# MilchRatchet/Luminary

Hardware: AMD Instinct MI355X
Metric: Mrays/s at 1920x1080, 8 bounces (higher is better)
Workload: dtype f32

## Files before the change

include/lum_core.h:

```cpp
#ifndef LUM_CORE_H
#define LUM_CORE_H

#include <stdint.h>

#ifdef __cplusplus
extern "C" {
#endif

typedef struct LumContext LumContext;

typedef struct LumDeviceSceneView {
  uint32_t num_meshes;
  uint32_t num_instances;
  uint32_t num_materials;
  uint32_t num_lights;
  const uint32_t* mesh_tri_offset;
  const float* vertices;
  const uint32_t* tri_tex;
  const uint32_t* instance_mesh_ids;
  const float* instance_transforms;
  const uint16_t* materials;
  const uint8_t* light_tree_root;
  const uint8_t* light_tree_nodes;
  const uint32_t* light_tri_handles;
// ... 135 lines not shown

int lumc_generate_result(LumContext* ctx, uint32_t mode, uint32_t local_error_minimization, uint32_t uniform_samples, float exposure,
                         const LumOutputParams* tone, float* d_result, void* stream);
int lumc_generate_result_host(LumContext* ctx, uint32_t mode, uint32_t local_error_minimization, uint32_t uniform_samples, float exposure,
                              const LumOutputParams* tone, float* result);
int lumc_render_undersampled(LumContext* ctx, uint32_t stage, uint32_t iteration, void* stream);
int lumc_generate_result_undersampled(LumContext* ctx, uint32_t stage, uint32_t iteration, float* d_result, void* stream);
int lumc_generate_result_undersampled_host(LumContext* ctx, uint32_t stage, uint32_t iteration, float* result);
int lumc_adaptive_note_first_sample(LumContext* ctx, void* stream);
int lumc_post_bloom(LumContext* ctx, float* d_image, uint32_t full_width, uint32_t full_height, uint32_t undersampling_stage, float blend, void* stream);
int lumc_post_bloom_host(LumContext* ctx, float* image, uint32_t full_width, uint32_t full_height, uint32_t undersampling_stage, float blend);
typedef struct LumDenoiseParams {
  uint32_t iterations;
  float sigma_luminance;
  float sigma_normal;
  float sigma_depth;
  uint32_t uniform_samples;
} LumDenoiseParams;
void lumc_denoise_default_params(LumDenoiseParams* params);
int lumc_render_guides(LumContext* ctx, uint32_t num_samples, void* stream);
int lumc_download_guides(LumContext* ctx, float* albedo, float* normal, float* depth);
int lumc_has_guides(const LumContext* ctx);
int lumc_denoise(LumContext* ctx, const LumDenoiseParams* params, float* d_image, void* stream);
int lumc_denoise_host(LumContext* ctx, const LumDenoiseParams* params, float* image);
int lumc_set_denoise_form(LumContext* ctx, int lds);
int lumc_download_result_image(LumContext* ctx, float* result);
const float* lumc_result_image(LumContext* ctx);

int lumc_trace_closest(LumContext* ctx, uint32_t num_rays, const float* d_origins, const float* d_dirs, const uint32_t* d_ignore, uint32_t* d_out, void* stream);
int lumc_pixel_query(LumContext* ctx, uint32_t x, uint32_t y, uint32_t sample_id, uint32_t out[6]);
int lumc_trace_closest_host(LumContext* ctx, uint32_t num_rays, const float* origins, const float* dirs, const uint32_t* ignore, uint32_t* out);

int lumc_trace_visibility(LumContext* ctx, uint32_t num_rays, const float* d_origins, const float* d_dirs, const float* d_dist, const uint32_t* d_ids, const uint32_t* d_order,
                          float* d_out, void* stream);
int lumc_trace_visibility_host(LumContext* ctx, uint32_t num_rays, const float* origins, const float* dirs, const float* dist, const uint32_t* ids, const uint32_t* order, float* out);
int lumc_light_query_host(LumContext* ctx, uint32_t num_rays, const float* origins, const float* dirs, const uint32_t* self, const float* randoms, uint32_t* out_ids,
                          uint32_t* out_num_hits);

#define LUMC_LENS_MAX_INTERFACES 24
typedef struct LumLensInterface { float radius, vertex, cylindrical_radius; } LumLensInterface;
typedef struct LumLensMedium { float design_ior, abbe, cylindrical_radius; } LumLensMedium;
typedef struct LumPhysicalCamera {
  float aperture_point, aperture_radius, exit_pupil_point, exit_pupil_radius, image_plane_distance, sensor_width;
  uint32_t allow_reflections;
  uint32_t num_interfaces;
  LumLensInterface interfaces[LUMC_LENS_MAX_INTERFACES];
  LumLensMedium media[LUMC_LENS_MAX_INTERFACES + 1];
} LumPhysicalCamera;
int lumc_set_physical_camera(LumContext* ctx, const LumPhysicalCamera* camera);
int lumc_camera_rays(LumContext* ctx, const uint32_t* pixels, uint32_t n, uint32_t first_sample, uint32_t samples, float* out_origin, float* out_dir, float* out_weight);

int lumc_set_bvh_builder(LumContext* ctx, int builder);

unsigned int lumc_lds_stack_bytes(void);

#define LUMC_COMM_ID_BYTES 128
int lumc_device_count(void);
uint32_t lumc_tile_lattice_step(uint32_t world);
uint32_t lumc_tile_owner(uint32_t tile_x, uint32_t tile_y, uint32_t tiles_x, uint32_t world);
int lumc_tile_pixels(uint32_t width, uint32_t height, uint32_t rank, uint32_t world, uint32_t tile, uint32_t* out, uint32_t* count);
int lumc_comm_unique_id(uint8_t id[LUMC_COMM_ID_BYTES]);
int lumc_comm_init_rank(LumContext* ctx, int world, int rank, const uint8_t id[LUMC_COMM_ID_BYTES]);
int lumc_comm_init_all(LumContext** ctxs, int n);
void lumc_comm_destroy(LumContext* ctx);
int lumc_frame_assemble(LumContext* ctx, uint32_t frame_pixels, int root, void* stream, float** d_frame_out);
int lumc_frame_assemble_all(LumContext** ctxs, int n, uint32_t frame_pixels, int root, float** d_frame_root);
int lumc_frame_gather(LumContext* ctx, uint32_t width, uint32_t height, int root, void* stream, float** d_frame_out);
int lumc_frame_gather_all(LumContext** ctxs, int n, uint32_t width, uint32_t height, int root, float** d_frame_root);
int lumc_frame_download(LumContext* ctx, uint32_t frame_pixels, float* first_moment, float* second_moment);
uint32_t lumc_frame_plane_stride(const LumContext* ctx);
int lumc_use_assembled_frame(LumContext* ctx, int on);
int lumc_accumulators_from_frame(LumContext* dst, LumContext* src);
int lumc_comm_count(const LumContext* ctx);
int lumc_device_name(int ordinal, char* out, size_t size);

int lumc_set_ray_sorting(LumContext* ctx, int mode);
int lumc_get_ray_sorting(const LumContext* ctx);

enum { LUMC_FLAVOUR_EXACT = 0, LUMC_FLAVOUR_FAST = 1 };
int lumc_set_flavour(LumContext* ctx, int flavour);
int lumc_get_flavour(const LumContext* ctx);
int lumc_set_ambient_reuse(LumContext* ctx, int mode);
int lumc_get_ambient_reuse(const LumContext* ctx);
int lumc_set_fused_resolve(LumContext* ctx, int on);
int lumc_set_sobol_table(LumContext* ctx, int on);
double lumc_bvh_build_seconds(const LumContext* ctx);
int lumc_bvh_meshes_by_builder(const LumContext* ctx, uint32_t out[2]);
int lumc_bvh_stats(LumContext* ctx, uint64_t out[4]);
uint32_t lumc_scene_view_sizeof(void);
int lumc_host_bvh_probe(const float* boxes, uint32_t count, uint32_t max_leaf, uint64_t out[6], double inner_area[3]);
uint32_t lumc_leaf_max_triangles(void);
typedef struct LumMeshRefitStats {
  uint64_t refits, rebuilds;
  uint32_t last_refits, last_rebuilds;
  double max_cost_growth;
  double seconds;
  double seconds_upload, seconds_refit, seconds_rebuild, seconds_assemble;
  double seconds_hash, seconds_download, seconds_lights;
} LumMeshRefitStats;
int lumc_set_mesh_refit(LumContext* ctx, uint32_t mode, float max_cost_growth);
int lumc_mesh_refit_stats(const LumContext* ctx, LumMeshRefitStats* out);
int lumc_bvh_refit_probe(const float* built_boxes, const float* refit_boxes, uint32_t count, uint32_t refit_count, int builder, int on_gpu, uint64_t sizes[3],
                         void* built_nodes, void* refit_nodes, void* host_refit_nodes, uint32_t* prims, double cost[3], uint64_t* valid);
int lumc_scene_tree_probe(const LumDeviceSceneView* scene, uint64_t sizes[4], void* nodes, void* tris, void* leaves, void* rows, uint32_t* mesh_root, float bounds[6]);
typedef struct LumInstanceUpdateStats {
  uint64_t device_updates, fallbacks, relayouts;
  uint32_t tlas_nodes, tlas_depth, tlas_capacity, hittable;
  double seconds;
  double seconds_relayout, seconds_upload, seconds_boxes, seconds_build, seconds_leaves;
} LumInstanceUpdateStats;
int lumc_set_instance_update(LumContext* ctx, uint32_t mode);
int lumc_instance_update_stats(const LumContext* ctx, LumInstanceUpdateStats* out);
int lumc_instance_boxes_probe(const LumDeviceSceneView* scene, const float* mesh_boxes, int on_gpu, void* rows, float* boxes, uint32_t* hittable);
int lumc_resident_tree_probe(LumContext* ctx, uint64_t sizes[5], void* top_nodes, void* leaves, uint32_t* mesh_root, uint64_t* mesh_hash);
int lumc_set_mesh_refit_in_place(LumContext* ctx, uint32_t on);
typedef struct LumResidentRefitStats {
  uint64_t updates, fallbacks;
  uint32_t last_meshes, last_launches;
  uint64_t last_bytes_downloaded;
  double seconds;
  double seconds_upload, seconds_hash, seconds_refit, seconds_cost, seconds_top_level;
} LumResidentRefitStats;
int lumc_resident_refit_stats(const LumContext* ctx, LumResidentRefitStats* out);
int lumc_resident_mesh_nodes_probe(LumContext* ctx, void* nodes);
int lumc_host_bvh_nodes_probe(const float* boxes, uint32_t count, uint32_t max_leaf, uint32_t max_depth, uint64_t sizes[3], void* nodes, uint32_t* prims);

#ifdef __cplusplus
}
#endif

#endif
```

luminary_amd/core.py:

```python
import ctypes as C

import numpy as np

from . import DeviceSceneView, _lib

DIRTY_CONSTANTS, DIRTY_MATERIALS, DIRTY_INSTANCES, DIRTY_LIGHTS, DIRTY_MESHES, DIRTY_TEXTURES, DIRTY_PARTICLES, DIRTY_ALL = 1, 2, 4, 8, 16, 32, 64, 127
DIRTY_MESH_POSITIONS = 128
DIRTY_INSTANCE_TRANSFORMS = 256
BVH_BUILDERS = {"sah": 0, "lbvh": 1, "ploc": 2, "sah_gpu": 3}
CNT_TRACE, CNT_SHADOW, CNT_LIGHT_BVH, CNT_VERTICES, CNT_NODES, CNT_TRIS, CNT_NODES_SHADOW, CNT_TRIS_SHADOW, CNT_NODES_LIGHT, CNT_TRIS_LIGHT, CNT_NODES_LDS, CNT_NODES_LDS_SHADOW, CNT_AMBIENT_DEFERRED, CNT_AMBIENT_FALLBACK = range(14)
CNT_COUNT = 16
KERNELS = ("generate", "trace", "shade", "shadow", "accumulate", "light_query", "resolve", "output", "sky", "sort", "volume")


class CoreError(RuntimeError):
    pass


class OutputParams(C.Structure):
    _fields_ = [("src_width", C.c_uint32), ("src_height", C.c_uint32), ("dst_width", C.c_uint32), ("dst_height", C.c_uint32),
                ("inv_sample_count", C.c_float), ("exposure", C.c_float), ("tonemap", C.c_uint32), ("filter", C.c_uint32), ("dithering", C.c_uint32),
                ("purkinje", C.c_uint32), ("use_color_correction", C.c_uint32), ("passthrough", C.c_uint32), ("purkinje_kappa1", C.c_float),
                ("purkinje_kappa2", C.c_float), ("cc_h", C.c_float), ("cc_s", C.c_float), ("cc_v", C.c_float), ("film_grain", C.c_float),
                ("agx_slope", C.c_float), ("agx_power", C.c_float), ("agx_saturation", C.c_float), ("supersampling", C.c_uint32),
# ... 127 lines not shown
        self._lib.lumc_context_create.restype = C.c_int
        rc = self._lib.lumc_context_create(C.c_int(device), C.byref(self._ctx))
        if rc != 0:
            msg = self._lib.lumc_last_error(self._ctx).decode() if self._ctx else "context allocation failed"
            if self._ctx:
                self._lib.lumc_context_destroy(self._ctx)
                self._ctx = C.c_void_p()
            raise CoreError("lumc_context_create failed (no CPU fallback exists): " + msg)
        self.num_pixels = 0

    @property
    def flavour(self):
        fn = getattr(self._lib, "lumc_get_flavour", None)
        if fn is None:
            return "exact"
        fn.restype = C.c_int
        return "fast" if fn(self._ctx) == 1 else "exact"

    @staticmethod
    def device_count():
        return int(_lib().lumc_device_count())

    @staticmethod
    def tile_pixels(width, height, rank, world, tile=32):
        lib = _lib()
        n = C.c_uint32()
        if lib.lumc_tile_pixels(C.c_uint32(width), C.c_uint32(height), C.c_uint32(rank), C.c_uint32(world), C.c_uint32(tile), C.c_void_p(0), C.byref(n)):
            raise CoreError("lumc_tile_pixels: bad arguments")
        out = np.zeros(max(n.value, 1), dtype=np.uint32)
        lib.lumc_tile_pixels(C.c_uint32(width), C.c_uint32(height), C.c_uint32(rank), C.c_uint32(world), C.c_uint32(tile), out.ctypes.data_as(C.c_void_p), C.byref(n))
        return out[:n.value]

    @staticmethod
    def comm_unique_id():
        buf = (C.c_uint8 * 128)()
        if _lib().lumc_comm_unique_id(buf):
            raise CoreError("lumc_comm_unique_id failed")
        return bytes(buf)

    def comm_init_rank(self, world, rank, unique_id):
        buf = (C.c_uint8 * 128).from_buffer_copy(unique_id)
        self._call("lumc_comm_init_rank", C.c_int(world), C.c_int(rank), buf)

    def frame_assemble(self, frame_pixels, root=0, stream=0):
        ptr = C.c_void_p()
        self._call("lumc_frame_assemble", C.c_uint32(frame_pixels), C.c_int(root), C.c_void_p(stream), C.byref(ptr))
        return ptr.value

    def frame_gather(self, width, height, root=0, stream=0):
        ptr = C.c_void_p()
        self._call("lumc_frame_gather", C.c_uint32(width), C.c_uint32(height), C.c_int(root), C.c_void_p(stream), C.byref(ptr))
        return ptr.value

    def frame_download(self, frame_pixels):
        fm = np.zeros(3 * frame_pixels, dtype=np.float32)
        sm = np.zeros(frame_pixels, dtype=np.float32)
        self._call("lumc_frame_download", C.c_uint32(frame_pixels), fm.ctypes.data_as(C.c_void_p), sm.ctypes.data_as(C.c_void_p))
        return fm.reshape(3, -1), sm

    @property
    def ray_sorting(self):
        fn = self._lib.lumc_get_ray_sorting
        fn.restype = C.c_int
        return int(fn(self._ctx))

    def set_ray_sorting(self, mode):
        self._call("lumc_set_ray_sorting", C.c_int(mode))

    def set_fused_resolve(self, on):
        self._call("lumc_set_fused_resolve", C.c_int(int(on)))

    def set_sobol_table(self, on):
        self._call("lumc_set_sobol_table", C.c_int(1 if on else 0))

    def set_ambient_reuse(self, mode):
        self._call("lumc_set_ambient_reuse", C.c_int(mode))

    @property
    def ambient_reuse(self):
        fn = self._lib.lumc_get_ambient_reuse
        fn.restype = C.c_int
        return bool(fn(self._ctx))

    def set_physical_camera(self, camera):
        self._call("lumc_set_physical_camera", C.byref(camera) if camera is not None else C.c_void_p(0))

    def camera_rays(self, pixels, first_sample, samples):
        px = np.ascontiguousarray(pixels, dtype=np.uint32)
        n = px.size * samples
        o = np.zeros((n, 3), dtype=np.float32)
        d = np.zeros((n, 3), dtype=np.float32)
        w = np.zeros(n, dtype=np.float32)
        self._call("lumc_camera_rays", px.ctypes.data_as(C.c_void_p), C.c_uint32(px.size), C.c_uint32(first_sample), C.c_uint32(samples),
                   o.ctypes.data_as(C.c_void_p), d.ctypes.data_as(C.c_void_p), w.ctypes.data_as(C.c_void_p))
        return o, d, w

    def pixel_query(self, x, y, sample_id=0):
        out = (C.c_uint32 * 6)()
        self._call("lumc_pixel_query", C.c_uint32(x), C.c_uint32(y), C.c_uint32(sample_id), out)
        a = np.array(list(out), dtype=np.uint32)
        return int(a[0]), int(a[1]), float(a[2:3].view(np.float32)[0]), a[3:6].view(np.float32).copy()

    def set_flavour(self, name):
        self._call("lumc_set_flavour", C.c_int({"exact": 0, "fast": 1}[name]))

    def _call(self, name, *args):
        fn = getattr(self._lib, name)
        fn.restype = C.c_int
        if fn(self._ctx, *args) != 0:
            raise CoreError("%s failed: %s" % (name, self._lib.lumc_last_error(self._ctx).decode()))

    def close(self):
        if self._ctx:
            self._lib.lumc_context_destroy(self._ctx)
            self._ctx = C.c_void_p()

    def __del__(self):
        try:
            self.close()
        except Exception:
            pass

    def upload(self, view):
        self._view_keepalive = view
        self._call("lumc_scene_upload", C.byref(view))
        self.width, self.height = view.width, view.height

    def update(self, view, dirty):
        self._view_keepalive = view
        self._call("lumc_scene_update", C.byref(view), C.c_uint(dirty))
        self.width, self.height = view.width, view.height

    def generate_output(self, params, first_moment=None, want_float=False):
        out = np.zeros((params.dst_height, params.dst_width), dtype=np.uint32)
        planes = np.zeros(params.output_planes_shape(), dtype=np.float32) if want_float else None
        pl = planes.ctypes.data_as(C.c_void_p) if want_float else C.c_void_p(0)
        if isinstance(first_moment, np.ndarray):
            fm = np.ascontiguousarray(first_moment, dtype=np.float32)
            self._call("lumc_generate_output_from_host", C.byref(params), fm.ctypes.data_as(C.c_void_p), out.ctypes.data_as(C.c_void_p), pl)
        else:
            ptr = C.c_void_p(0) if first_moment is None else C.c_void_p(int(first_moment))
            self._call("lumc_generate_output_host", C.byref(params), ptr, out.ctypes.data_as(C.c_void_p), pl)
        return (out, planes) if want_float else out

    def download_luts(self):
        out = {"conductor": np.zeros(1024, np.uint16), "glossy": np.zeros(1024, np.uint16), "dielectric": np.zeros(32768, np.uint16),
               "dielectric_inv": np.zeros(32768, np.uint16)}
        self._call("lumc_download_luts", *[out[k].ctypes.data_as(C.c_void_p) for k in ("conductor", "glossy", "dielectric", "dielectric_inv")])
        return out

    def download_sky_luts(self):
        tm = np.zeros(2 * 64 * 256 * 4, dtype=np.float32)
        ms = np.zeros(2 * 32 * 32 * 4, dtype=np.float32)
        self._call("lumc_download_sky_luts", tm.ctypes.data_as(C.c_void_p), ms.ctypes.data_as(C.c_void_p))
        return tm, ms

    def cloud_noise_generate(self, seed):
        shape, detail, weather = np.zeros(128 ** 3, np.uint32), np.zeros(32 ** 3, np.uint32), np.zeros(1024 ** 2, np.uint32)
        self._call("lumc_cloud_noise_generate", C.c_uint32(seed), shape.ctypes.data_as(C.c_void_p), detail.ctypes.data_as(C.c_void_p),
                   weather.ctypes.data_as(C.c_void_p))
        return shape, detail, weather

    def sky_hdri_build(self, origin, dim, samples):
        o = (C.c_float * 3)(*[float(x) for x in origin])
        self._call("lumc_sky_hdri_build", o, C.c_uint32(dim), C.c_uint32(samples))
        out = np.zeros((dim, dim, 4), dtype=np.float32)
# ... 278 lines not shown
```

luminary_amd/csrc/device/dev_trace.h:

```cpp
#pragma once

#include "dev_light.h"

LUM_NS_BEGIN

#ifndef LUM_TRACE_BLOCK
#define LUM_TRACE_BLOCK 1024
#endif
constexpr int kTraceBlock = LUM_TRACE_BLOCK;

constexpr uint32_t kHitSky        = 0xFFFFFFFEu;
constexpr uint32_t kLeaveInstance = 0xFFFFFFFDu;
constexpr uint32_t kTraversalDone = 0xFFFFFFFCu;
constexpr uint32_t kNoInstance    = 0xFFFFFFFFu;
constexpr int kStackSize = 128;
#ifndef LUM_CHUNK_MAX
#define LUM_CHUNK_MAX 256u
#endif
#ifndef LUM_VOTE_TRIS
#define LUM_VOTE_TRIS 1u
#define LUM_VOTE_NODES 2u
#endif
#ifndef LUM_REFILL
#define LUM_REFILL 40
// ... 87 lines not shown
  static LUM_DEV W pack(uint32_t e) { return e; }
  static LUM_DEV uint32_t unpack(W w) { return w; }
};
template <> struct StackWord<uint2> {
  typedef unsigned long long W;
  static LUM_DEV W pack(uint2 e) { return (W) e.x | ((W) e.y << 32); }
  static LUM_DEV uint2 unpack(W w) { return make_uint2((uint32_t) w, (uint32_t) (w >> 32)); }
};
template <typename E> struct TraversalStack {
  typedef typename StackWord<E>::W W;
  typedef __attribute__((address_space(5))) W* ScratchPtr;
  typedef __attribute__((address_space(3))) W* LdsPtr;
  ScratchPtr scratch; LdsPtr lds; int lds_entries;
  LUM_DEV void store(int i, E e) { if (i < lds_entries) lds[(uint32_t) i * (uint32_t) kTraceBlock] = StackWord<E>::pack(e); else scratch[i] = StackWord<E>::pack(e); }
  LUM_DEV E load(int i) const { if (i < lds_entries) return StackWord<E>::unpack(lds[(uint32_t) i * (uint32_t) kTraceBlock]); return StackWord<E>::unpack(scratch[i]); }
};
template <bool kOrdered, bool kCull, int kFarFirst = 0, typename S>
LUM_DEV uint32_t visit_node(const NodeSource& src, uint32_t cur, const TRay& r, float tmax, S& stk, int& sp,
                            typename StackEntry<kCull>::E& top, RayStats& st) {
  static_assert(!(kFarFirst && kCull), "the negated keys are not distances: only for queries that do not cull by them");
  using SE = StackEntry<kCull>;
  const uint32_t b = cur << 7;
  float4 nx, ny, nz, fx, fy, fz;
  uint4 ch;
  if (cur < src.lds_count) {
    const char* p = src.lds + b;
    nx = *reinterpret_cast<const float4*>(p + r.nx); ny = *reinterpret_cast<const float4*>(p + r.ny); nz = *reinterpret_cast<const float4*>(p + r.nz);
    fx = *reinterpret_cast<const float4*>(p + r.fx); fy = *reinterpret_cast<const float4*>(p + r.fy); fz = *reinterpret_cast<const float4*>(p + r.fz);
    ch = *reinterpret_cast<const uint4*>(p + 96u);
    st.lds_nodes++;
  }
  else {
    const Bvh4Node* __restrict__ nodes = src.global;
    nx = node_f4(nodes, b + r.nx); ny = node_f4(nodes, b + r.ny); nz = node_f4(nodes, b + r.nz);
    fx = node_f4(nodes, b + r.fx); fy = node_f4(nodes, b + r.fy); fz = node_f4(nodes, b + r.fz);
    ch = node_u4(nodes, b + 96u);
  }
  float k0 = child_entry<kFarFirst>(nx.x, ny.x, nz.x, fx.x, fy.x, fz.x, r, tmax);
  float k1 = child_entry<kFarFirst>(nx.y, ny.y, nz.y, fx.y, fy.y, fz.y, r, tmax);
  float k2 = child_entry<kFarFirst>(nx.z, ny.z, nz.z, fx.z, fy.z, fz.z, r, tmax);
  float k3 = child_entry<kFarFirst>(nx.w, ny.w, nz.w, fx.w, fy.w, fz.w, r, tmax);
  uint32_t c0 = ch.x, c1 = ch.y, c2 = ch.z, c3 = ch.w;
  if (kOrdered) {
    cswap(k0, c0, k1, c1); cswap(k2, c2, k3, c3); cswap(k0, c0, k2, c2); cswap(k1, c1, k3, c3); cswap(k1, c1, k2, c2);
  }
  const float inf = __builtin_inff();
  if (k1 < inf) {
    if (k2 < inf) {
      if (k3 < inf) { stk.store(sp, top); sp++; top = SE::make(c3, k3); }
      stk.store(sp, top); sp++; top = SE::make(c2, k2);
    }
    stk.store(sp, top); sp++; top = SE::make(c1, k1);
  }
  return (k0 < inf) ? c0 : kBvhEmpty;
}

template <typename S>
LUM_DEV uint2 stack_pop(const S& stk, int& sp, uint2& top) {
  const uint2 e = top;
  if (sp > 0) { sp--; top = stk.load(sp); }
  else top = make_uint2(kTraversalDone, 0u);
  return e;
}
template <typename S, typename E>
LUM_DEV void stack_push(S& stk, int& sp, E& top, E e) { stk.store(sp, top); sp++; top = e; }

LUM_DEV float4 tri_f4(const BvhTri* tris, uint32_t index, uint32_t word) { return reinterpret_cast<const float4*>(tris + index)[word]; }

struct LeafTris {
  float4 a[kBvhLeafMaxTri], b[kBvhLeafMaxTri], c[kBvhLeafMaxTri];
  template <bool kAllSlots>
  LUM_DEV void load(const BvhTri* __restrict__ tris, uint32_t first, uint32_t count) {
#pragma unroll
    for (uint32_t j = 0; j < kBvhLeafMaxTri; j++) {
      if (kAllSlots) {
        const uint32_t t = first + min(j, count - 1u);
        a[j] = tri_f4(tris, t, 0); b[j] = tri_f4(tris, t, 1); c[j] = tri_f4(tris, t, 2);
      }
      else if (j < count) { a[j] = tri_f4(tris, first + j, 0); b[j] = tri_f4(tris, first + j, 1); c[j] = tri_f4(tris, first + j, 2); }
    }
  }
};

template <class Q>
LUM_DEV void trace_items(const DeviceScene& sc, uint32_t n, uint32_t* __restrict__ cursor, Q& q, RayStats& st, uint32_t& rays, uint32_t lds_count) {
  if (n == 0u) return;
  using SE = StackEntry<Q::kCull>;
  using E = typename SE::E;
  E stack_in_scratch[kStackSize];
  int sp = 0;
  TRay r;
  V3 wo = v3(0.0f, 0.0f, 0.0f), wd = v3(0.0f, 0.0f, 1.0f);
  float tmax = 0.0f;
  uint32_t cur = kTraversalDone, inst = kNoInstance, idx = 0;
  r.set(wo, wd);
  bool more = true;
  const uint32_t lane = threadIdx.x & 63u;
  const unsigned long long below = (1ull << lane) - 1ull;
  extern __shared__ float4 lds_top[];
  {
    const float4* __restrict__ g = reinterpret_cast<const float4*>(sc.bvh_nodes);
    for (uint32_t i = threadIdx.x; i < lds_count * (kNodeBytes / 16u); i += blockDim.x) lds_top[i] = g[i];
    __syncthreads();
  }
  __shared__ float4 lds_leaves[4u * LUM_LDS_INSTANCES];
  const uint32_t staged_leaves = min(sc.tlas_num_leaves, (uint32_t) LUM_LDS_INSTANCES);
  for (uint32_t i = threadIdx.x; i < 4u * staged_leaves; i += blockDim.x) lds_leaves[i] = sc.tlas_leaves[i];
  __syncthreads();
  const NodeSource nodes{sc.bvh_nodes, reinterpret_cast<const char*>(lds_top), lds_count};
  typedef typename TraversalStack<E>::W StackW;
  static_assert(sizeof(StackW) == sizeof(E), "a stack entry is one machine word");
  TraversalStack<E> stk{(typename TraversalStack<E>::ScratchPtr) reinterpret_cast<StackW*>(stack_in_scratch),
                        (typename TraversalStack<E>::LdsPtr) (reinterpret_cast<StackW*>(reinterpret_cast<char*>(lds_top) + lds_count * kNodeBytes) + threadIdx.x),
                        (int) (LUM_LDS_STACK_BYTES / (kRayBlockMax * (uint32_t) sizeof(E)))};

  E top = SE::make(kTraversalDone, 0.0f);
#ifdef LUM_PHASE_STATS
  uint32_t phase_[8] = {0, 0, 0, 0, 0, 0, 0, 0};
  unsigned long long ptime_[12] = {0, 0, 0, 0, 0, 0, 0, 0, 0, 0, 0, 0};
  const unsigned long long t_kernel_ = __builtin_readcyclecounter();
#endif
  auto pop = [&]() {
    LUM_PHASE(6); LUM_PHASE_LANES(7);
    bool left_instance = false, again;
    E e;
    do {
      e = top;
      const bool done = SE::node(e) == kTraversalDone, leave = SE::node(e) == kLeaveInstance;
      if (!done) { sp--; top = stk.load(sp); }
      left_instance |= leave;
      again = !done && (leave || !SE::reachable(e, tmax));
    } while (again);
    cur = SE::node(e);
    if (left_instance) { inst = kNoInstance; r.set(wo, wd); }
  };

  const uint32_t waves = gridDim.x * (blockDim.x / 64u);
  uint32_t chunk = n / (waves * 2u);
  chunk = (min(max(chunk, 64u), LUM_CHUNK_MAX) + 63u) & ~63u;
  uint32_t chunk_next = 0, chunk_end = 0;

  while (true) {
    const unsigned long long idle = __ballot(cur == kTraversalDone);
#ifdef LUM_PHASE_STATS
    const unsigned long long t_refill_ = __builtin_readcyclecounter();
    const bool refilling_ = idle != 0ull && more;
#endif
    if (idle != 0ull && more) {
      if (chunk_next >= chunk_end) {
        uint32_t base = 0;
        if (lane == 0) base = atomicAdd(cursor, chunk);
        base = __builtin_amdgcn_readfirstlane(base);
        chunk_next = base;
        chunk_end = min(base + chunk, n);
        more = base < n;
      }
      if (more) {
        const uint32_t avail = chunk_end - chunk_next, want = (uint32_t) __popcll(idle);
        const uint32_t rank = (uint32_t) __popcll(idle & below);
        if (cur == kTraversalDone && rank < avail) {
          idx = chunk_next + rank;
          if (q.load(sc, idx, wo, wd, tmax)) {
            rays++;
            const uint32_t e = 0x7F800000u;
            const bool finite = (fbits(wo.x) & e) != e && (fbits(wo.y) & e) != e && (fbits(wo.z) & e) != e && (fbits(wd.x) & e) != e && (fbits(wd.y) & e) != e &&
                                (fbits(wd.z) & e) != e;
            if (finite) { r.set(wo, wd); cur = 0; sp = 0; top = SE::make(kTraversalDone, 0.0f); inst = kNoInstance; }
            else q.finish(sc, idx);
          }
        }
        chunk_next += min(want, avail);
      }
    }
#ifdef LUM_PHASE_STATS
    if (refilling_) { ptime_[8] += __builtin_readcyclecounter() - t_refill_; ptime_[9]++; }
#endif
    if (__ballot(cur != kTraversalDone) == 0ull) break;
    LUM_PHASE(5);

    while (true) {
      const bool live = cur != kTraversalDone;
      const bool at_leaf = live && (cur & kBvhLeafBit);
      const bool want_tris = at_leaf && inst != kNoInstance, want_enter = at_leaf && inst == kNoInstance;
      const uint32_t n_live = (uint32_t) __popcll(__ballot(live)), n_tris = (uint32_t) __popcll(__ballot(want_tris)), n_enter = (uint32_t) __popcll(__ballot(want_enter));
      if (n_live == 0u) break;
      const uint32_t n_nodes = n_live - n_tris - n_enter;
      const bool run_tris = n_tris * LUM_VOTE_TRIS >= max(n_nodes, n_enter) * LUM_VOTE_NODES;
      const bool run_enter = !run_tris && n_enter >= n_nodes;
      const bool do_tris = run_tris && want_tris, do_enter = run_enter && want_enter, do_node = !run_tris && !run_enter && live && !at_leaf;
      LUM_TIME_BEGIN();
#ifdef LUM_PHASE_STATS
      const bool memory_node_ = __ballot(do_node && cur >= lds_count) != 0ull;
#endif
      {
        if (do_tris) {
          LUM_PHASE(3); LUM_PHASE_LANES(4);
          if (q.on_tris(sc, inst, cur & 0x0FFFFFFFu, ((cur >> 28) & 0x7u) + 1u, r.o, r.d, tmax, st)) cur = kTraversalDone;
          else pop();
          if (cur == kTraversalDone) q.finish(sc, idx);
        }
      }
      {
        if (do_enter) {
          LUM_PHASE(1); LUM_PHASE_LANES(2);
          const uint32_t leaf_index = cur & 0x0FFFFFFFu;
          float4 r0, r1, r2, meta;
          if (leaf_index < staged_leaves) { const float4* leaf = lds_leaves + 4u * leaf_index; r0 = leaf[0]; r1 = leaf[1]; r2 = leaf[2]; meta = leaf[3]; }
          else { const float4* __restrict__ leaf = sc.tlas_leaves + 4u * leaf_index; r0 = leaf[0]; r1 = leaf[1]; r2 = leaf[2]; meta = leaf[3]; }
          inst = fbits(meta.x);
          const float px = wo.x - r0.w, py = wo.y - r1.w, pz = wo.z - r2.w;
          const V3 oo = v3(mat_row_apply(r0.x, r0.y, r0.z, px, py, pz), mat_row_apply(r1.x, r1.y, r1.z, px, py, pz), mat_row_apply(r2.x, r2.y, r2.z, px, py, pz));
          const V3 od = v3(mat_row_apply(r0.x, r0.y, r0.z, wd.x, wd.y, wd.z), mat_row_apply(r1.x, r1.y, r1.z, wd.x, wd.y, wd.z),
                           mat_row_apply(r2.x, r2.y, r2.z, wd.x, wd.y, wd.z));
          r.set(oo, od);
          stack_push(stk, sp, top, SE::make(kLeaveInstance, 0.0f));
          cur = fbits(meta.y);
        }
      }
      {
        if (do_node) {
          LUM_PHASE(0);
          st.nodes++;
          cur = visit_node<Q::kOrdered, Q::kCull, Q::kFarFirst>(nodes, cur, r, tmax, stk, sp, top, st);
          if (cur == kBvhEmpty) {
            pop();
            if (cur == kTraversalDone) q.finish(sc, idx);
          }
        }
      }
#ifdef LUM_PHASE_STATS
      {
        asm volatile("s_waitcnt vmcnt(0) lgkmcnt(0)" ::: "memory");
        const int kind = run_tris ? 4 : (run_enter ? 6 : (memory_node_ ? 0 : 2));
        LUM_TIME_END(kind);
      }
#endif
      if (more && n_live < LUM_REFILL) break;
    }
  }
#ifdef LUM_PHASE_STATS
  ptime_[10] = __builtin_readcyclecounter() - t_kernel_; ptime_[11] = 1;
  for (int k = 0; k < 8; k++) if (phase_[k]) atomicAdd(&g_phase[k], (unsigned long long) phase_[k]);
  if ((threadIdx.x & 63u) == 0u) for (int k = 0; k < 12; k++) if (ptime_[k]) atomicAdd(&g_phase_time[k], ptime_[k]);
#endif
}

struct Hit { uint32_t instance_id, tri_id; float t; uint32_t scene_tri; };

struct ClosestState {
  static constexpr bool kOrdered = true;
  static constexpr int kFarFirst = 0;
  static constexpr bool kCull = true;
  static constexpr uint32_t kOpaqueBit = 0x80000000u;
  bool use_ignore, cutout;
  uint32_t ign_inst, ign_tri;
  Hit best;
  LUM_DEV void begin(bool ignore, uint32_t inst, uint32_t tri) { use_ignore = ignore; cutout = false; ign_inst = inst; ign_tri = tri; best = Hit{kHitSky, 0u, kFltMax, 0u}; }
  LUM_DEV bool on_tris(const DeviceScene& sc, uint32_t inst, uint32_t first, uint32_t count, V3 o, V3 d, float& tmax, RayStats& st) {
    LeafTris lt;
    lt.load<false>(sc.blas_tris, first, count);
#pragma unroll
    for (uint32_t j = 0; j < kBvhLeafMaxTri; j++) {
      if (j >= count) break;
      const float4 a = lt.a[j], b = lt.b[j], c = lt.c[j];
      const uint32_t id = fbits(a.w);
      st.tris++;
      if (use_ignore && inst == ign_inst && id == ign_tri) continue;
      F2 uv;
      const float t = intersect_triangle(v3(a.x, a.y, a.z), v3(b.x, b.y, b.z), v3(c.x, c.y, c.z), o, d, uv);
      if (t < best.t || (t == best.t && t != kFltMax && (inst < best.instance_id || (inst == best.instance_id && id < best.tri_id)))) {
        if (fbits(c.w) < sc.num_textures &&
            texture_load(sc, fbits(c.w), triangle_uv(sc.tri_tex[fbits(b.w)], uv), true, make_float4(0.0f, 0.0f, 0.0f, 1.0f)).w == 0.0f) {
          cutout = true;
          continue;
        }
        best.instance_id = inst; best.tri_id = id; best.t = t; best.scene_tri = fbits(b.w) | (fbits(c.w) == kBvhTriOpaque ? kOpaqueBit : 0u); tmax = t;
      }
    }
    return false;
  }
  LUM_DEV Hit result() const { return (best.t == kFltMax) ? Hit{kHitSky, 0u, kFltMax, 0u} : Hit{best.instance_id, best.tri_id, best.t, best.scene_tri & ~kOpaqueBit}; }
};

struct ShadowState {
  static constexpr bool kOrdered = true;
// ... 140 lines not shown
```

luminary_amd/csrc/device/kernel_shadow.h:

```cpp
#pragma once

#include "dev_trace.h"

#ifndef LUM_SHADOW_KERNEL_EXTERN
#define LUM_SHADOW_KERNEL_EXTERN 0
#endif

LUM_NS_BEGIN

struct ShadowQuery : ShadowState {
  ShadowQueue sq;
  const uint32_t* order;
  uint32_t out;
  LUM_DEV bool load(const DeviceScene&, uint32_t slot, V3& o, V3& d, float& tmax) {
    const uint32_t j = order ? order[slot] : slot;
    const float4 o4 = ld_stream(&sq.origin_dist[j]), d4 = ld_stream(&sq.dir_out[j]);
    begin(ld_stream(&sq.ids[j]), o4.w);
    out = fbits(d4.w);
    o = v3(o4.x, o4.y, o4.z); d = v3(d4.x, d4.y, d4.z); tmax = o4.w;
    return true;
  }
  LUM_DEV void finish(const DeviceScene&, uint32_t) {
    const Col v = result();
#ifdef LUM_PHASE_STATS
    { const uint32_t kind = min(out / sq.capacity, 3u); atomicAdd(&g_vis_stat[2u * kind], 1ull); if (blocked) atomicAdd(&g_vis_stat[2u * kind + 1u], 1ull); }
#endif
    st_stream(&sq.vis[out], make_float4(v.r, v.g, v.b, 0.0f));
  }
};

#if LUM_SHADOW_KERNEL_EXTERN
__global__ LUM_TRACE_BOUNDS void k_shadow_rays(DeviceScene sc, ShadowQueue sq, const uint32_t* order, uint32_t* ctrl, uint64_t* counters, uint32_t lds_nodes);
#else
__global__ LUM_TRACE_BOUNDS void k_shadow_rays(DeviceScene sc, ShadowQueue sq, const uint32_t* order, uint32_t* ctrl, uint64_t* counters, uint32_t lds_nodes) {
  RayStats st{0, 0, 0};
  uint32_t rays = 0;
  ShadowQuery q;
  q.sq = sq;
  q.order = order;
  trace_items(sc, ctrl[kCtlShadowItems], ctrl + kCtlShadowCursor, q, st, rays, lds_nodes);
  flush_stats(counters, st, rays, kCntShadow, kCntNodesShadow, kCntTrisShadow, kCntNodesLdsShadow);
}
#endif

LUM_NS_END
```

luminary_amd/csrc/device/kernels.h:

```cpp
#pragma once

#include "kernel_shadow.h"
#include "dev_sky.h"
#include "dev_volume.h"
#include "dev_particle.h"
#include "dev_water.h"
#include "dev_cloud_march.h"
#include "dev_adaptive.h"
#include "dev_camera.h"
#include "dev_wave.h"

LUM_NS_BEGIN

#ifndef LUM_SHADE_WAVES
#define LUM_SHADE_WAVES 3
#endif
#ifndef LUM_CLOUD_WAVES
#define LUM_CLOUD_WAVES 4
#endif
#ifndef LUM_FEATURE_WAVES
#define LUM_FEATURE_WAVES 3
#endif
#ifndef LUM_VOLUME_WAVES
#define LUM_VOLUME_WAVES 4
// ... 94 lines not shown
  const uint32_t rounds = (pass_tasks + gridDim.x * 256u - 1u) / (gridDim.x * 256u);
  for (uint32_t round = 0; round < rounds; round++) {
    const uint32_t slot = (round * gridDim.x + blockIdx.x) * 256u + threadIdx.x;
    const uint32_t t = pass.task_begin + slot;
    bool valid = false;
    uint32_t x = 0, y = 0, sample_id = 0;
    if (slot < pass_tasks) {
      uint32_t lo = pass.block_begin, hi = pass.block_end - 1u;
      while (lo < hi) {
        const uint32_t mid = (lo + hi) >> 1;
        if (t < a.block_task_end[mid] * pass.executions) hi = mid; else lo = mid + 1u;
      }
      const uint32_t block = lo;
      const uint32_t base = block ? a.block_task_end[block - 1u] * pass.executions : 0u;
      const uint32_t packed = a.stage_counts[block];
      const uint32_t per_pixel = adaptive_stage_count(packed, a.stage_id) * pass.executions;
      const uint32_t local = t - base;
      const uint32_t local_pixel = local / per_pixel, local_sample = local - local_pixel * per_pixel;
      const uint32_t by = block / a.blocks_x, bx = block - by * a.blocks_x;
      x = (bx << kAdaptiveBlockLog) + (local_pixel & 3u);
      y = (by << kAdaptiveBlockLog) + (local_pixel >> kAdaptiveBlockLog);
      sample_id = adaptive_pixel_samples(a, packed) + local_sample;
      valid = x < sc.width && y < sc.height && sample_id < kMaxGlobalSamples;
      results[slot] = make_float4(0.0f, 0.0f, 0.0f, 0.0f);
    }
    generate_path<kCam>(sc, lens, q, count, valid, x, y, sample_id, slot);
  }
}

template <int kCam>
__global__ __launch_bounds__(kBlock) void k_camera_rays(DeviceScene sc, DeviceLens lens_arg, const uint32_t* pixels, uint32_t n, uint32_t first_sample, uint32_t samples,
                                                        float* out_origin, float* out_dir, float* out_weight) {
  __shared__ DeviceLens lds_lens;
  const DeviceLens& lens = stage_lens<kCam>(lens_arg, &lds_lens);
  const uint32_t total = n * samples;
  for (uint32_t i = blockIdx.x * kBlock + threadIdx.x; i < total; i += gridDim.x * kBlock) {
    const uint32_t b = i / n, index = pixels[i - b * n];
    const uint32_t y = index / sc.width, x = index - y * sc.width;
    const Sampler smp{sc.bluenoise_2d, x, y, first_sample + b, 0};
    V3 o, d;
    const float w = camera_sample<kCam>(sc, lens, smp, o, d);
    out_origin[3 * i] = o.x; out_origin[3 * i + 1] = o.y; out_origin[3 * i + 2] = o.z;
    out_dir[3 * i] = d.x; out_dir[3 * i + 1] = d.y; out_dir[3 * i + 2] = d.z;
    out_weight[i] = w;
  }
}

constexpr uint32_t kNoAmbientPath = 0xFFFFFFFFu;
constexpr bool kReuseProves = !LUM_FAST;
constexpr uint32_t kHitTriOpaque = 0x80000000u, kHitTriCutout = 0x40000000u, kHitTriBeyondEps = 0x20000000u, kHitTriHit = 0x10000000u, kHitTriMask = 0x0FFFFFFFu;

struct TraceQuery : ClosestState {
  PathQueue q;
  const uint32_t* order;
  uint32_t item;
  LUM_DEV bool load(const DeviceScene&, uint32_t j, V3& o, V3& d, float& tmax) {
    const uint32_t i = order ? order[j] : j;
    item = i;
    const float4 o4 = ld_stream(&q.origin_t[i]), d4 = ld_stream(&q.dir_slot[i]);
    const uint32_t state = q.aux[i].w;
    const uint2 ign = *reinterpret_cast<const uint2*>(&q.hit_id[i]);
    begin((state & kStUseIgnoreHandle) != 0, ign.x, ign.y);
    o = v3(o4.x, o4.y, o4.z); d = v3(d4.x, d4.y, d4.z); tmax = kFltMax;
    return true;
  }
  LUM_DEV void finish(const DeviceScene&, uint32_t) {
    const uint32_t i = item;
    const Hit h = result();
    reinterpret_cast<float*>(&q.origin_t[i])[3] = h.t;
    *reinterpret_cast<uint2*>(&q.hit_id[i]) = make_uint2(h.instance_id, h.tri_id);
    static_assert(kOpaqueBit == kHitTriOpaque, "the opaque bit is stored where ClosestState keeps it");
    q.hit_scene_tri[i] = ((best.t == kFltMax) ? 0u : (best.scene_tri | kHitTriHit | (best.t > kEps ? kHitTriBeyondEps : 0u))) | (cutout ? kHitTriCutout : 0u);
  }
};

__global__ LUM_TRACE_BOUNDS void k_trace(DeviceScene sc, PathQueue q, const uint32_t* order, uint32_t* ctrl, uint64_t* counters, uint32_t lds_nodes) {
  RayStats st{0, 0, 0};
  uint32_t rays = 0;
  TraceQuery tq;
  tq.q = q;
  tq.order = order;
  tq.item = 0;
  trace_items(sc, ctrl[kCtlPaths], ctrl + kCtlTraceCursor, tq, st, rays, lds_nodes);
  flush_stats(counters, st, rays, kCntTrace, kCntNodes, kCntTris, kCntNodesLds);
}

LUM_DEV GeoContext build_context(const DeviceScene& sc, V3 hit_origin, V3 ray_world, uint32_t state, uint32_t inst, uint32_t tri, uint32_t tbase, uint32_t medium) {
  const Transform tf = load_transform(sc, inst);
  const float4 a = sc.vertices[3 * tbase], b = sc.vertices[3 * tbase + 1], c = sc.vertices[3 * tbase + 2];
  const uint4 tt = sc.tri_tex[tbase];
  V3 position = xf_point_inv(tf, hit_origin);
  const V3 ray = xf_rot_inv(tf, ray_world);
  const V3 p0 = v3(a.x, a.y, a.z);
  const V3 e1 = v3(b.x, b.y, b.z) - p0, e2 = v3(c.x, c.y, c.z) - p0;
  V3 face = normalize(cross(e1, e2));
  const F2 co = barycentric_in_triangle(p0, e1, e2, position);
  position = p0 + (e1 * co.x + e2 * co.y);
  position = xf_point(tf, position);
  const Material mat = load_material(sc, tt.w & 0xFFFFu);
  const F2 tex_coords = triangle_uv(tt, co);
  const V3 n0 = normal_unpack(fbits(a.w)), n1 = normal_unpack(fbits(b.w)), n2 = normal_unpack(fbits(c.w));
  const bool inside = dot(face, ray) > 0.0f;
  if (inside) face = face * -1.0f;
  V3 normal = lerp_normals(n0, n1 - n0, n2 - n0, co, face);
  if (mat.normal_tex != kTextureNone) {
    const bool valid = mat.normal_tex < sc.num_textures;
    const float4 nf = texture_load(sc, mat.normal_tex, tex_coords, false, make_float4(0.0f, 0.0f, 1.0f, 0.0f));
    V3 mn = v3(nf.x, nf.y, nf.z);
    if ((mat.flags & kDMatNormalMapCompressed) && valid) mn = mn * 2.0f - v3(1.0f, 1.0f, 1.0f);
    mn = normalize(mn);
    normal = qapply(qinv(rotation_to_z(normal)), mn);
  }
  normal = adapt_normal(ray * -1.0f, normal, face);
  Col albedo = mat.albedo;
  float alpha = mat.alpha;
  if (mat.albedo_tex != kTextureNone) {
    const float4 af = texture_load(sc, mat.albedo_tex, tex_coords, true, make_float4(0.9f, 0.9f, 0.9f, 1.0f));
    albedo = col(af.x, af.y, af.z);
    alpha = af.w;
  }
  const bool emissive_side = !inside || (mat.flags & kDMatBidirectionalEmission);
  const bool emits = (mat.flags & kDMatEmission) && emissive_side && ((state & kStAllowEmission) != 0);
  Col emission = emits ? mat.emission : col(0.0f, 0.0f, 0.0f);
  if (emits && mat.luminance_tex != kTextureNone) {
    const float4 lf = texture_load(sc, mat.luminance_tex, tex_coords, true, make_float4(0.0f, 0.0f, 0.0f, 0.0f));
    emission = col(lf.x, lf.y, lf.z) * (alpha * mat.emission_scale);
  }
  float roughness = mat.roughness;
  if (mat.roughness_tex != kTextureNone) roughness = texture_load(sc, mat.roughness_tex, tex_coords, true, make_float4(0.5f, 0.0f, 0.0f, 0.0f)).x;
  if (mat.flags & kDMatRoughnessAsSmoothness) roughness = 1.0f - roughness;
  roughness = fmaxf(roughness, 2e-2f);
  if ((state & kStDeltaPath) == 0) roughness = fmaxf(roughness, mat.roughness_clamp);
  uint32_t flags = mat.flags & kDMatSubstrateMask;
  if (mat.metallic_tex == kTextureNone && (mat.flags & kDMatMetallic)) flags |= kMatMetallic;
  if (mat.flags & kDMatColoredTransparency) flags |= kMatColoredTransparency;
  if (inside) flags |= kMatRefractionInside;
  const float other_ior = medium_ior_peek(medium, inside);
  const float ior_in = inside ? mat.refraction_index : other_ior;
  const float ior_out = inside ? other_ior : mat.refraction_index;
  if (((flags & kMatSubstrateMask) == kMatTranslucent) && (fabsf(1.0f - ior_in / ior_out) < 1e-4f)) {
    if ((flags & kMatColoredTransparency) == 0) albedo = col(lerpf(1.0f, albedo.r, alpha), lerpf(1.0f, albedo.g, alpha), lerpf(1.0f, albedo.b, alpha));
    alpha = 0.0f;
    flags |= kMatColoredTransparency;
  }
  GeoContext g;
  g.instance_id = inst; g.tri_id = tri;
  g.normal = xf_rot(tf, normal);
  g.face_normal_packed = normal_pack(face);
  g.position = position;
  g.V = ray_world * -1.0f;
  g.state = state;
  g.params.flags = flags;
  g.params.set(albedo, alpha, roughness, emission, ior_in / ior_out);
  return g;
}

LUM_DEV void add_to_result(float4* results, uint32_t slot, Col v) {
  if (!any_positive(v)) return;
  float4 r = results[slot];
  r.x += v.r; r.y += v.g; r.z += v.b;
  results[slot] = r;
}

struct ResolveRecords { uint4 aux; uint32_t slot; float4 cl, lc; uint4 amb; };
LUM_DEV ResolveRecords load_resolve_records(const PathQueue& in, const NeeQueue& nee, uint32_t i) {
  ResolveRecords r;
// ... 1430 lines not shown
#pragma unroll
        for (uint32_t r = 0; r < kListRounds; r++) {
          if ((scattered_mask >> r) & 1u) vq.items[base + w.rank(b[r])] = ((group_start + r) * gridDim.x + blockIdx.x) * kBlock + threadIdx.x;
          base += Wave::count(b[r]);
        }
      }
      scattered_mask = 0;
    }
  }
}

__global__ __launch_bounds__(kBlock) void k_volume_bounce(DeviceScene sc, PathQueue in, PathQueue out, VolumeQueue vq, uint32_t* ctrl, uint32_t depth_const) {
  const uint32_t n = ctrl[kCtlVolumeItems];
  uint32_t* count_out = ctrl + kCtlStride + kCtlPaths;
  const uint32_t lane = threadIdx.x & 63;
  const unsigned long long below = (1ull << lane) - 1ull;
  const uint32_t rounds = (n + gridDim.x * kBlock - 1) / (gridDim.x * kBlock);
  constexpr uint32_t kReserveRounds = 8;
  uint32_t reserved_base = 0;
  for (uint32_t round = 0; round < rounds; round++) {
    const uint32_t k = (round * gridDim.x + blockIdx.x) * kBlock + threadIdx.x;
    const bool valid = k < n;
    if (round % kReserveRounds == 0) {
      uint32_t count = 0;
      const uint32_t first = (round * gridDim.x + blockIdx.x) * kBlock + (threadIdx.x & ~63u);
      for (uint32_t r = 0; r < kReserveRounds && round + r < rounds; r++) {
        const uint32_t lo = first + r * gridDim.x * kBlock;
        count += (lo < n) ? min(64u, n - lo) : 0u;
      }
      uint32_t base = 0;
      if (lane == 0 && count) base = atomicAdd(count_out, count);
      reserved_base = __builtin_amdgcn_readfirstlane(base);
    }
    float4 n_o, n_d; uint4 n_aux, n_hid;
    if (valid) {
      const uint32_t i = vq.items[k];
      const float4 o4 = in.origin_t[i], d4 = in.dir_slot[i];
      const uint4 aux = in.aux[i], hid = in.hit_id[i];
      const Sampler smp{sc.bluenoise_2d, hid.z & 0xFFFFu, hid.z >> 16, path_sample_id(hid.w), depth_const};
      const V3 ray = v3(d4.x, d4.y, d4.z);
      const V3 origin = v3(o4.x, o4.y, o4.z) + ray * o4.w;
      const VolContext ctx = volume_context(sc, volume_stack_peek(hid.w, false), origin, ray, aux.w, 0.0f);
      const V3 bounce = volume_bsdf_sample(sc, ctx, smp, kRndVolGiResampling, kRndVolGiDiffuse);
      uint32_t state = aux.w & ~(kStDeltaPath | kStCameraDirection | kStAllowEmission | kStUseIgnoreHandle);
      if (sc.sky_mode != kSkyDefault) state &= ~kStAllowAmbient; else state |= kStAllowAmbient;
      state |= kStVolumeScattered;
      n_o = make_float4(origin.x, origin.y, origin.z, kFltMax);
      n_d = make_float4(bounce.x, bounce.y, bounce.z, d4.w);
      n_aux = make_uint4(aux.x, aux.y, aux.z, state);
      n_hid = make_uint4(0u, 0u, hid.z, hid.w);
    }
    const unsigned long long b = __ballot(valid);
    if (valid) {
      const uint32_t j = reserved_base + (uint32_t) __popcll(b & below);
      out.origin_t[j] = n_o; out.dir_slot[j] = n_d; out.aux[j] = n_aux; out.hit_id[j] = n_hid;
    }
    reserved_base += (uint32_t) __popcll(b);
  }
}

struct RaysQuery : ClosestState {
  const float* origins; const float* dirs; const uint32_t* ignore; uint32_t* out;
  LUM_DEV bool load(const DeviceScene&, uint32_t i, V3& o, V3& d, float& tmax) {
    const bool ign = ignore != nullptr && ignore[2 * i] != 0xFFFFFFFFu;
    begin(ign, ign ? ignore[2 * i] : 0u, ign ? ignore[2 * i + 1] : 0u);
    o = v3(origins[3 * i], origins[3 * i + 1], origins[3 * i + 2]); d = v3(dirs[3 * i], dirs[3 * i + 1], dirs[3 * i + 2]); tmax = kFltMax;
    return true;
  }
  LUM_DEV void finish(const DeviceScene&, uint32_t i) {
    const Hit h = result();
    out[3 * i] = h.instance_id; out[3 * i + 1] = h.tri_id; out[3 * i + 2] = fbits(h.t);
  }
};

__global__ LUM_TRACE_BOUNDS void k_trace_rays(DeviceScene sc, uint32_t n, const float* origins, const float* dirs, const uint32_t* ignore,
                                                           uint32_t* out, uint32_t* cursor, uint64_t* counters, uint32_t lds_nodes) {
  RayStats st{0, 0, 0};
  uint32_t rays = 0;
  RaysQuery q;
  q.origins = origins; q.dirs = dirs; q.ignore = ignore; q.out = out;
  trace_items(sc, n, cursor, q, st, rays, lds_nodes);
  flush_stats(counters, st, rays, kCntTrace, kCntNodes, kCntTris, kCntNodesLds);
}

__global__ __launch_bounds__(kBlock) void k_light_query_probe(DeviceScene sc, uint32_t n, const float* origins, const float* dirs, const uint32_t* self, const float* randoms,
                                                              uint32_t* out_ids, uint32_t* out_num_hits) {
  const uint32_t i = blockIdx.x * kBlock + threadIdx.x;
  if (i >= n) return;
  RayStats st{0, 0, 0};
  uint32_t num_hits = 0;
  const uint32_t id = light_query(sc, v3(origins[3 * i], origins[3 * i + 1], origins[3 * i + 2]), v3(dirs[3 * i], dirs[3 * i + 1], dirs[3 * i + 2]), self[2 * i], self[2 * i + 1],
                                  randoms[i], num_hits, st);
  out_ids[i] = id; out_num_hits[i] = num_hits;
}

__global__ __launch_bounds__(256) void k_sobol_table(uint2* __restrict__ table, uint32_t first_sample, uint32_t count, uint32_t stride, uint32_t dims) {
  const uint32_t t = blockIdx.x * 256u + threadIdx.x;
  const uint32_t dim = t / stride, s = t - dim * stride;
  if (dim >= dims || s >= count) return;
  const U2 q = sobol_owen(first_sample + s, dim);
  table[t] = make_uint2(q.x, q.y);
}

LUM_NS_END
```

luminary_amd/csrc/device/wavefront_table.h:

```cpp
#pragma once

#include <hip/hip_runtime.h>

#include "dev_scene.h"

namespace lum {

struct WavefrontKernels {
  const char* flavour;
  uint32_t trace_block;
  int (*set_ray_kernel_lds)(size_t bytes);
  int (*init_sampler_seeds)();
  void (*sobol_table)(hipStream_t s, uint2* table, uint32_t first_sample, uint32_t count, uint32_t stride, uint32_t dims);
  void (*generate)(uint32_t grid, hipStream_t s, const DeviceScene& sc, const PassParams& pp, const PathQueue& q, float4* results, uint32_t* count, const DeviceLens& lens,
                   int cam);
  void (*generate_adaptive)(uint32_t grid, hipStream_t s, const DeviceScene& sc, const AdaptiveView& a, const AdaptivePass& pass, const PathQueue& q, float4* results,
                            uint32_t* count, const DeviceLens& lens, int cam);
  void (*trace)(uint32_t grid, size_t lds, hipStream_t s, const DeviceScene& sc, const PathQueue& q, const uint32_t* order, uint32_t* ctrl, uint64_t* counters,
                uint32_t lds_nodes);
  void (*sky_inscattering)(uint32_t grid, hipStream_t s, const DeviceScene& sc, const PathQueue& in, float4* results, const uint32_t* ctrl, uint32_t depth_const);
  void (*shade)(uint32_t grid, hipStream_t s, const DeviceScene& sc, const PathQueue& in, const PathQueue& out, const NeeQueue& nee, const ShadowQueue& sq, float4* results,
                uint32_t* ctrl, uint32_t depth_const, uint64_t* counters, uint32_t ambient_reuse, const FusedResolve* fused_dev, uint32_t fused_flags);
  void (*shade_debug)(uint32_t grid, hipStream_t s, const DeviceScene& sc, const PathQueue& in, float4* results, const uint32_t* ctrl);
  void (*sky)(uint32_t grid, hipStream_t s, const DeviceScene& sc, const PathQueue& in, const ShadowQueue& sq, float4* results, const uint32_t* ctrl, uint32_t depth_const);
  void (*light_query)(uint32_t grid, hipStream_t s, const DeviceScene& sc, const PathQueue& in, const NeeQueue& nee, const ShadowQueue& sq, uint32_t* ctrl, uint32_t depth_const,
                      uint64_t* counters);
  void (*shadow_rays)(uint32_t grid, size_t lds, hipStream_t s, const DeviceScene& sc, const ShadowQueue& sq, const uint32_t* order, uint32_t* ctrl, uint64_t* counters,
                      uint32_t lds_nodes);
  void (*resolve)(uint32_t grid, hipStream_t s, const DeviceScene& sc, const PathQueue& in, const NeeQueue& nee, const ShadowQueue& sq, float4* results, const uint32_t* ctrl);
  void (*resolve_reuse)(uint32_t grid, hipStream_t s, const DeviceScene& sc, const PathQueue& in, const PathQueue& next, const NeeQueue& nee, const ShadowQueue& sq, float4* results,
                        uint32_t* ctrl, uint64_t* counters);
  void (*resolve_listed)(uint32_t grid, hipStream_t s, const DeviceScene& sc, const PathQueue& in, const NeeQueue& nee, const ShadowQueue& sq, float4* results, const uint32_t* ctrl);
  void (*resolve_ended)(uint32_t grid, hipStream_t s, const DeviceScene& sc, const PathQueue& in, const NeeQueue& nee, const ShadowQueue& sq, float4* results, const uint32_t* ctrl,
                        const uint32_t* list);
  bool fused_resolve;
  void (*volume_inscatter)(uint32_t grid, hipStream_t s, const DeviceScene& sc, const PathQueue& in, const VolumeQueue& vq, const ShadowQueue& sq, uint32_t* ctrl,
                           uint32_t depth_const);
  void (*volume_resolve)(uint32_t grid, hipStream_t s, const DeviceScene& sc, const PathQueue& in, const VolumeQueue& vq, const ShadowQueue& sq, float4* results,
                         const uint32_t* ctrl);
  void (*volume_events)(uint32_t grid, hipStream_t s, const DeviceScene& sc, const PathQueue& in, const VolumeQueue& vq, float4* results, uint32_t* ctrl, uint32_t depth_const);
  void (*volume_bounce)(uint32_t grid, hipStream_t s, const DeviceScene& sc, const PathQueue& in, const PathQueue& out, const VolumeQueue& vq, uint32_t* ctrl,
                        uint32_t depth_const);
  void (*trace_particles)(uint32_t grid, size_t lds, hipStream_t s, const DeviceScene& particle_tree, const PathQueue& q, uint32_t* ctrl, uint32_t lds_nodes);
  void (*particle_shade)(uint32_t grid, hipStream_t s, const DeviceScene& sc, const PathQueue& in, const PathQueue& out, const NeeQueue& nee, const ShadowQueue& sq,
                         uint32_t* ctrl, uint32_t depth_const);
  void (*trace_ocean)(uint32_t grid, hipStream_t s, const DeviceScene& sc, const PathQueue& q, const uint32_t* ctrl);
  void (*ocean_shade)(uint32_t grid, hipStream_t s, const DeviceScene& sc, const PathQueue& in, const PathQueue& out, const NeeQueue& nee, const ShadowQueue& sq, uint32_t* ctrl,
                      uint32_t depth_const);
  void (*clouds_list)(uint32_t grid, hipStream_t s, const DeviceScene& sc, const PathQueue& in, const CloudQueue& cq, uint32_t* ctrl);
  void (*clouds_march)(uint32_t grid, hipStream_t s, const DeviceScene& sc, const PathQueue& in, const CloudQueue& cq, uint32_t* ctrl, uint32_t depth_const);
  void (*clouds)(uint32_t grid, hipStream_t s, const DeviceScene& sc, const PathQueue& in, const CloudQueue& cq, float4* results, const uint32_t* ctrl, uint32_t depth_const);
  void (*trace_rays)(uint32_t grid, size_t lds, hipStream_t s, const DeviceScene& sc, uint32_t n, const float* origins, const float* dirs, const uint32_t* ignore, uint32_t* out,
                     uint32_t* cursor, uint64_t* counters, uint32_t lds_nodes);
  void (*camera_rays)(uint32_t grid, hipStream_t s, const DeviceScene& sc, const DeviceLens& lens, int cam, const uint32_t* pixels, uint32_t n, uint32_t first_sample,
                      uint32_t samples, float* origin, float* dir, float* weight);
  void (*guide)(uint32_t grid, hipStream_t s, const DeviceScene& sc, const PathQueue& in, const uint32_t* ctrl, float* planes, uint32_t n);
  void (*guide_normalise)(uint32_t grid, hipStream_t s, float* planes, uint32_t n, uint32_t samples);
  void (*denoise_prepare)(uint32_t grid, hipStream_t s, const AdaptiveView& a, const DenoiseArgs& p, const float* fm, const float* sm, const float* image, const float* guides,
                          float4* rec_a, uint4* rec_b);
  void (*denoise_atrous)(hipStream_t s, const DenoiseArgs& p, const float4* a_in, const uint4* rec_b, float4* a_out, bool lds);
  void (*denoise_finish)(uint32_t grid, hipStream_t s, const DenoiseArgs& p, const float4* rec_a, const float* guides, float* image);
  void (*light_query_probe)(hipStream_t s, const DeviceScene& sc, uint32_t n, const float* origins, const float* dirs, const uint32_t* self, const float* randoms, uint32_t* out_ids,
                            uint32_t* out_num_hits);
};

const WavefrontKernels* wavefront_kernels_exact();
const WavefrontKernels* wavefront_kernels_fast();

}
```

luminary_amd/csrc/device/wavefront_table_impl.h:

```cpp
#pragma once

#include "dev_adaptive.h"
#include "dev_denoise.h"
#include "wavefront_table.h"

LUM_NS_BEGIN
namespace table {

static int set_ray_kernel_lds(size_t bytes) {
  hipError_t e = hipFuncSetAttribute((const void*) k_trace, hipFuncAttributeMaxDynamicSharedMemorySize, (int) bytes);
  if (e == hipSuccess) e = hipFuncSetAttribute((const void*) k_shadow_rays, hipFuncAttributeMaxDynamicSharedMemorySize, (int) bytes);
  if (e == hipSuccess) e = hipFuncSetAttribute((const void*) k_trace_rays, hipFuncAttributeMaxDynamicSharedMemorySize, (int) bytes);
  if (e == hipSuccess) e = hipFuncSetAttribute((const void*) k_trace_particles, hipFuncAttributeMaxDynamicSharedMemorySize, (int) bytes);
  return (int) e;
}
static int init_sampler_seeds() { return upload_sampler_seeds(); }
static void sobol_table(hipStream_t s, uint2* table, uint32_t first_sample, uint32_t count, uint32_t stride, uint32_t dims) {
  hipLaunchKernelGGL(k_sobol_table, dim3((dims * stride + 255u) / 256u), dim3(256), 0, s, table, first_sample, count, stride, dims);
}
static void generate(uint32_t grid, hipStream_t s, const DeviceScene& sc, const PassParams& pp, const PathQueue& q, float4* results, uint32_t* count, const DeviceLens& lens,
                     int cam) {
  auto* k = cam == kCamPhysical ? k_generate<kCamPhysical> : cam == kCamPhysicalReflections ? k_generate<kCamPhysicalReflections> : k_generate<kCamThinLens>;
  hipLaunchKernelGGL(k, dim3(grid), dim3(kBlock), 0, s, sc, pp, q, results, count, lens);
}
static void generate_adaptive(uint32_t grid, hipStream_t s, const DeviceScene& sc, const AdaptiveView& a, const AdaptivePass& pass, const PathQueue& q, float4* results,
                              uint32_t* count, const DeviceLens& lens, int cam) {
  auto* k = cam == kCamPhysical ? k_generate_adaptive<kCamPhysical> : cam == kCamPhysicalReflections ? k_generate_adaptive<kCamPhysicalReflections>
                                                                                                     : k_generate_adaptive<kCamThinLens>;
  hipLaunchKernelGGL(k, dim3(grid), dim3(kBlock), 0, s, sc, a, pass, q, results, count, lens);
}
static void camera_rays(uint32_t grid, hipStream_t s, const DeviceScene& sc, const DeviceLens& lens, int cam, const uint32_t* pixels, uint32_t n, uint32_t first_sample,
                        uint32_t samples, float* origin, float* dir, float* weight) {
  auto* k = cam == kCamPhysical ? k_camera_rays<kCamPhysical> : cam == kCamPhysicalReflections ? k_camera_rays<kCamPhysicalReflections> : k_camera_rays<kCamThinLens>;
  hipLaunchKernelGGL(k, dim3(grid), dim3(kBlock), 0, s, sc, lens, pixels, n, first_sample, samples, origin, dir, weight);
}
static void trace(uint32_t grid, size_t lds, hipStream_t s, const DeviceScene& sc, const PathQueue& q, const uint32_t* order, uint32_t* ctrl, uint64_t* counters,
                  uint32_t lds_nodes) {
  hipLaunchKernelGGL(k_trace, dim3(grid), dim3(kTraceBlock), lds, s, sc, q, order, ctrl, counters, lds_nodes);
}
static void sky_inscattering(uint32_t grid, hipStream_t s, const DeviceScene& sc, const PathQueue& in, float4* results, const uint32_t* ctrl, uint32_t depth_const) {
  hipLaunchKernelGGL(k_sky_inscattering, dim3(grid), dim3(kBlock), 0, s, sc, in, results, ctrl, depth_const);
}
static void shade(uint32_t grid, hipStream_t s, const DeviceScene& sc, const PathQueue& in, const PathQueue& out, const NeeQueue& nee, const ShadowQueue& sq, float4* results,
                  uint32_t* ctrl, uint32_t depth_const, uint64_t* counters, uint32_t ambient_reuse, const FusedResolve* fused_dev, uint32_t fused_flags) {
  auto* k = sc.sky_mode == kSkyDefault ? k_shade<kSkyDefault, false> : sc.sky_mode == kSkyHdri ? k_shade<kSkyHdri, false> : k_shade<kSkyConstantColor, false>;
  if (sc.ocean_active) k = sc.sky_mode == kSkyDefault ? k_shade<kSkyDefault, true> : sc.sky_mode == kSkyHdri ? k_shade<kSkyHdri, true> : k_shade<kSkyConstantColor, true>;
  if (sc.sobol_table) {
    k = sc.sky_mode == kSkyDefault ? k_shade<kSkyDefault, false, true> : sc.sky_mode == kSkyHdri ? k_shade<kSkyHdri, false, true> : k_shade<kSkyConstantColor, false, true>;
    if (sc.ocean_active) k = sc.sky_mode == kSkyDefault ? k_shade<kSkyDefault, true, true> : sc.sky_mode == kSkyHdri ? k_shade<kSkyHdri, true, true> : k_shade<kSkyConstantColor, true, true>;
  }
  hipLaunchKernelGGL(k, dim3(grid), dim3(kBlock), 0, s, sc, in, out, nee, sq, results, ctrl, depth_const, counters, ambient_reuse, fused_dev, fused_flags);
}
static void shade_debug(uint32_t grid, hipStream_t s, const DeviceScene& sc, const PathQueue& in, float4* results, const uint32_t* ctrl) {
  hipLaunchKernelGGL(k_shade_debug, dim3(grid), dim3(kBlock), 0, s, sc, in, results, ctrl);
}
static void sky(uint32_t grid, hipStream_t s, const DeviceScene& sc, const PathQueue& in, const ShadowQueue& sq, float4* results, const uint32_t* ctrl, uint32_t depth_const) {
  hipLaunchKernelGGL(k_sky, dim3(grid), dim3(kBlock), 0, s, sc, in, sq, results, ctrl, depth_const);
}
static void light_query(uint32_t grid, hipStream_t s, const DeviceScene& sc, const PathQueue& in, const NeeQueue& nee, const ShadowQueue& sq, uint32_t* ctrl, uint32_t depth_const,
                        uint64_t* counters) {
  hipLaunchKernelGGL(k_light_query, dim3(grid), dim3(kBlock), 0, s, sc, in, nee, sq, ctrl, depth_const, counters);
}
static void shadow_rays(uint32_t grid, size_t lds, hipStream_t s, const DeviceScene& sc, const ShadowQueue& sq, const uint32_t* order, uint32_t* ctrl, uint64_t* counters,
                        uint32_t lds_nodes) {
  hipLaunchKernelGGL(k_shadow_rays, dim3(grid), dim3(kTraceBlock), lds, s, sc, sq, order, ctrl, counters, lds_nodes);
}
static void resolve(uint32_t grid, hipStream_t s, const DeviceScene& sc, const PathQueue& in, const NeeQueue& nee, const ShadowQueue& sq, float4* results, const uint32_t* ctrl) {
  hipLaunchKernelGGL(k_resolve, dim3(grid), dim3(kBlock), 0, s, sc, in, nee, sq, results, ctrl);
}
static void resolve_reuse(uint32_t grid, hipStream_t s, const DeviceScene& sc, const PathQueue& in, const PathQueue& next, const NeeQueue& nee, const ShadowQueue& sq, float4* results,
                          uint32_t* ctrl, uint64_t* counters) {
  hipLaunchKernelGGL(k_resolve_reuse, dim3(grid), dim3(kBlock), 0, s, sc, in, next, nee, sq, results, ctrl, counters);
}
static void resolve_listed(uint32_t grid, hipStream_t s, const DeviceScene& sc, const PathQueue& in, const NeeQueue& nee, const ShadowQueue& sq, float4* results, const uint32_t* ctrl) {
  hipLaunchKernelGGL(k_resolve_listed, dim3(grid), dim3(kBlock), 0, s, sc, in, nee, sq, results, ctrl);
}
static void resolve_ended(uint32_t grid, hipStream_t s, const DeviceScene& sc, const PathQueue& in, const NeeQueue& nee, const ShadowQueue& sq, float4* results, const uint32_t* ctrl,
                          const uint32_t* list) {
  hipLaunchKernelGGL(k_resolve_ended, dim3(grid), dim3(kBlock), 0, s, sc, in, nee, sq, results, ctrl, list);
}
static void volume_inscatter(uint32_t grid, hipStream_t s, const DeviceScene& sc, const PathQueue& in, const VolumeQueue& vq, const ShadowQueue& sq, uint32_t* ctrl,
                             uint32_t depth_const) {
  hipLaunchKernelGGL(k_volume_inscatter, dim3(grid), dim3(kBlock), 0, s, sc, in, vq, sq, ctrl, depth_const);
}
static void volume_resolve(uint32_t grid, hipStream_t s, const DeviceScene& sc, const PathQueue& in, const VolumeQueue& vq, const ShadowQueue& sq, float4* results,
                           const uint32_t* ctrl) {
  hipLaunchKernelGGL(k_volume_resolve, dim3(grid), dim3(kBlock), 0, s, sc, in, vq, sq, results, ctrl);
}
static void volume_events(uint32_t grid, hipStream_t s, const DeviceScene& sc, const PathQueue& in, const VolumeQueue& vq, float4* results, uint32_t* ctrl,
                          uint32_t depth_const) {
  hipLaunchKernelGGL(k_volume_events, dim3(grid), dim3(kBlock), 0, s, sc, in, vq, results, ctrl, depth_const);
}
static void volume_bounce(uint32_t grid, hipStream_t s, const DeviceScene& sc, const PathQueue& in, const PathQueue& out, const VolumeQueue& vq, uint32_t* ctrl,
                          uint32_t depth_const) {
  hipLaunchKernelGGL(k_volume_bounce, dim3(grid), dim3(kBlock), 0, s, sc, in, out, vq, ctrl, depth_const);
}
static void trace_particles(uint32_t grid, size_t lds, hipStream_t s, const DeviceScene& particle_tree, const PathQueue& q, uint32_t* ctrl, uint32_t lds_nodes) {
  hipLaunchKernelGGL(k_trace_particles, dim3(grid), dim3(kTraceBlock), lds, s, particle_tree, q, ctrl, lds_nodes);
}
static void particle_shade(uint32_t grid, hipStream_t s, const DeviceScene& sc, const PathQueue& in, const PathQueue& out, const NeeQueue& nee, const ShadowQueue& sq,
                           uint32_t* ctrl, uint32_t depth_const) {
  hipLaunchKernelGGL(k_particle_shade, dim3(grid), dim3(kBlock), 0, s, sc, in, out, nee, sq, ctrl, depth_const);
}
static void trace_ocean(uint32_t grid, hipStream_t s, const DeviceScene& sc, const PathQueue& q, const uint32_t* ctrl) {
  hipLaunchKernelGGL(k_trace_ocean, dim3(grid), dim3(kBlock), 0, s, sc, q, ctrl);
}
static void ocean_shade(uint32_t grid, hipStream_t s, const DeviceScene& sc, const PathQueue& in, const PathQueue& out, const NeeQueue& nee, const ShadowQueue& sq,
                        uint32_t* ctrl, uint32_t depth_const) {
  hipLaunchKernelGGL(k_ocean_shade, dim3(grid), dim3(kBlock), 0, s, sc, in, out, nee, sq, ctrl, depth_const);
}
static void clouds_list(uint32_t grid, hipStream_t s, const DeviceScene& sc, const PathQueue& in, const CloudQueue& cq, uint32_t* ctrl) {
  hipLaunchKernelGGL(k_clouds_list, dim3(grid), dim3(kBlock), 0, s, sc, in, cq, ctrl);
}
static void clouds_march(uint32_t grid, hipStream_t s, const DeviceScene& sc, const PathQueue& in, const CloudQueue& cq, uint32_t* ctrl, uint32_t depth_const) {
  hipLaunchKernelGGL(k_clouds_march, dim3(grid), dim3(kBlock), 0, s, sc, in, cq, ctrl, depth_const);
}
static void clouds(uint32_t grid, hipStream_t s, const DeviceScene& sc, const PathQueue& in, const CloudQueue& cq, float4* results, const uint32_t* ctrl, uint32_t depth_const) {
  hipLaunchKernelGGL(k_clouds, dim3(grid), dim3(kBlock), 0, s, sc, in, cq, results, ctrl, depth_const);
}
static void trace_rays(uint32_t grid, size_t lds, hipStream_t s, const DeviceScene& sc, uint32_t n, const float* origins, const float* dirs, const uint32_t* ignore, uint32_t* out,
                       uint32_t* cursor, uint64_t* counters, uint32_t lds_nodes) {
  hipLaunchKernelGGL(k_trace_rays, dim3(grid), dim3(kTraceBlock), lds, s, sc, n, origins, dirs, ignore, out, cursor, counters, lds_nodes);
}
static void guide(uint32_t grid, hipStream_t s, const DeviceScene& sc, const PathQueue& in, const uint32_t* ctrl, float* planes, uint32_t n) {
  hipLaunchKernelGGL(k_guide, dim3(grid), dim3(kBlock), 0, s, sc, in, ctrl, planes, n);
}
static void guide_normalise(uint32_t grid, hipStream_t s, float* planes, uint32_t n, uint32_t samples) {
  hipLaunchKernelGGL(k_guide_normalise, dim3(grid), dim3(256), 0, s, planes, n, samples);
}
static void denoise_prepare(uint32_t grid, hipStream_t s, const AdaptiveView& a, const DenoiseArgs& p, const float* fm, const float* sm, const float* image, const float* guides,
                            float4* rec_a, uint4* rec_b) {
  hipLaunchKernelGGL(k_denoise_prepare, dim3(grid), dim3(256), 0, s, a, p, fm, sm, image, guides, rec_a, rec_b);
}
static void denoise_atrous(hipStream_t s, const DenoiseArgs& p, const float4* a_in, const uint4* rec_b, float4* a_out, bool lds) {
  const dim3 grid((p.width + kDenoiseTileX - 1u) / kDenoiseTileX, (p.height + kDenoiseTileY - 1u) / kDenoiseTileY);
  if (lds && p.step <= kDenoiseMaxLdsStep) hipLaunchKernelGGL(k_denoise_atrous<true>, grid, dim3(256), 0, s, p, a_in, rec_b, a_out);
  else hipLaunchKernelGGL(k_denoise_atrous<false>, grid, dim3(256), 0, s, p, a_in, rec_b, a_out);
}
static void denoise_finish(uint32_t grid, hipStream_t s, const DenoiseArgs& p, const float4* rec_a, const float* guides, float* image) {
  hipLaunchKernelGGL(k_denoise_finish, dim3(grid), dim3(256), 0, s, p, rec_a, guides, image);
}
static void light_query_probe(hipStream_t s, const DeviceScene& sc, uint32_t n, const float* origins, const float* dirs, const uint32_t* self, const float* randoms, uint32_t* out_ids,
                              uint32_t* out_num_hits) {
  hipLaunchKernelGGL(k_light_query_probe, dim3((n + kBlock - 1) / kBlock), dim3(kBlock), 0, s, sc, n, origins, dirs, self, randoms, out_ids, out_num_hits);
}

static constexpr WavefrontKernels make_table() {
  WavefrontKernels t{};
  t.flavour = LUM_FLAVOUR_NAME; t.trace_block = (uint32_t) kTraceBlock; t.set_ray_kernel_lds = set_ray_kernel_lds; t.init_sampler_seeds = init_sampler_seeds;
  t.sobol_table = sobol_table; t.generate = generate; t.generate_adaptive = generate_adaptive; t.trace = trace; t.sky_inscattering = sky_inscattering;
  t.shade = shade; t.shade_debug = shade_debug; t.sky = sky; t.light_query = light_query;
  t.shadow_rays = shadow_rays; t.resolve = resolve; t.resolve_reuse = resolve_reuse; t.resolve_listed = resolve_listed; t.resolve_ended = resolve_ended; t.fused_resolve = LUM_FAST != 0;
  t.volume_inscatter = volume_inscatter; t.volume_resolve = volume_resolve; t.volume_events = volume_events; t.volume_bounce = volume_bounce;
  t.trace_particles = trace_particles; t.particle_shade = particle_shade; t.trace_ocean = trace_ocean; t.ocean_shade = ocean_shade;
  t.clouds_list = clouds_list; t.clouds_march = clouds_march; t.clouds = clouds; t.trace_rays = trace_rays;
  t.camera_rays = camera_rays; t.guide = guide;
  t.guide_normalise = guide_normalise; t.denoise_prepare = denoise_prepare; t.denoise_atrous = denoise_atrous; t.denoise_finish = denoise_finish; t.light_query_probe = light_query_probe;
  return t;
}
static constexpr WavefrontKernels kTable = make_table();

}
LUM_NS_END

#ifdef LUM_PHASE_STATS
#if LUM_FAST
extern "C" int lumc_debug_phase_stats_fast(uint64_t out[16], int reset) {
  if (hipMemcpyFromSymbol(out, HIP_SYMBOL(g_phase), sizeof(uint64_t) * 16) != hipSuccess) return 1;
  if (reset) { const uint64_t zero[16] = {0}; if (hipMemcpyToSymbol(HIP_SYMBOL(g_phase), zero, sizeof(zero)) != hipSuccess) return 1; }
  return 0;
}
extern "C" int lumc_debug_phase_times_fast(uint64_t out[16], int reset) {
  if (hipMemcpyFromSymbol(out, HIP_SYMBOL(g_phase_time), sizeof(uint64_t) * 16) != hipSuccess) return 1;
  if (reset) { const uint64_t zero[16] = {0}; if (hipMemcpyToSymbol(HIP_SYMBOL(g_phase_time), zero, sizeof(zero)) != hipSuccess) return 1; }
  return 0;
}
extern "C" int lumc_debug_vis_stats_fast(uint64_t out[8], int reset) {
  if (hipMemcpyFromSymbol(out, HIP_SYMBOL(g_vis_stat), sizeof(uint64_t) * 8) != hipSuccess) return 1;
  if (reset) { const uint64_t zero[8] = {0}; if (hipMemcpyToSymbol(HIP_SYMBOL(g_vis_stat), zero, sizeof(zero)) != hipSuccess) return 1; }
  return 0;
}
extern "C" int lumc_debug_shade_times_fast(uint64_t out[16], int reset) {
  if (hipMemcpyFromSymbol(out, HIP_SYMBOL(g_shade_time), sizeof(uint64_t) * 16) != hipSuccess) return 1;
  if (reset) { const uint64_t zero[16] = {0}; if (hipMemcpyToSymbol(HIP_SYMBOL(g_shade_time), zero, sizeof(zero)) != hipSuccess) return 1; }
  return 0;
}
#else
extern "C" int lumc_debug_phase_stats(uint64_t out[16], int reset) {
  if (hipMemcpyFromSymbol(out, HIP_SYMBOL(g_phase), sizeof(uint64_t) * 16) != hipSuccess) return 1;
  if (reset) { const uint64_t zero[16] = {0}; if (hipMemcpyToSymbol(HIP_SYMBOL(g_phase), zero, sizeof(zero)) != hipSuccess) return 1; }
  return 0;
}
#endif
#endif

namespace lum {
#if LUM_FAST
const WavefrontKernels* wavefront_kernels_fast() { return &fast::table::kTable; }
#else
const WavefrontKernels* wavefront_kernels_exact() { return &exact::table::kTable; }
#endif
}
```

luminary_amd/csrc/host/context.h:

```cpp
#pragma once

#include <hip/hip_runtime.h>

#include <cstdio>
#include <memory>
#include <string>
#include <vector>

#include "../../../include/lum_core.h"
#include "../device/dev_scene.h"
#include "../device/wavefront_table.h"
#include "bvh_build.h"
#include "bvh_refit.h"
#include "device_buffer.h"
#include "instance_update.h"
#include "scene_arrays.h"
#include "work_layout.h"

using namespace lum;

typedef struct ncclComm* ncclComm_t;

struct MeshTree { Bvh4 bvh; bool built_on_gpu = false; };

struct MeshRefit {
  RefitPlan plan;
  std::shared_ptr<MeshTree> own;
  uint64_t fit_hash[2] = {0, 0};
  double built_cost = 0.0;
  bool stale = false;
};

struct LumContext {
  int device = 0;
  std::string error;
  const WavefrontKernels* wf = wavefront_kernels_fast();
  int camera = kCamThinLens;
  DeviceLens lens{};
  SceneArrays arrays;
  std::vector<std::shared_ptr<const MeshTree>> mesh_bvh;
  std::vector<Aabb> mesh_box;
  std::vector<MeshRefit> mesh_refit;
  std::vector<uint32_t> mesh_tri_offset;
  uint32_t refit_mode = 0;
  float refit_max_cost_growth = 0.0f;
  LumMeshRefitStats refit_stats{};
  InstanceUpdate instance_update;
  std::vector<uint32_t> instance_mesh_ids;
  uint32_t instance_update_mode = 0;
  LumInstanceUpdateStats instance_stats{};
  uint32_t refit_in_place = 0;
  ResidentRefit resident_refit;
  uint32_t stale_meshes = 0;
  LumResidentRefitStats resident_stats{};
  std::vector<uint32_t> sky_lut_key;
  DeviceBuffer<float> d_bridge_lut;
  std::vector<float> bridge_lut_host;
  DeviceBuffer<float4> d_sky_lut[2];
  DeviceScene scene{};
  bool has_scene = false;
  uint64_t bvh_stats[4] = {0, 0, 0, 0};
  int ambient_reuse = -1;
  uint32_t shade_grid_rounds = 2;
  int fused_resolve = 1;
  struct Fused : FusedBuffers {
    DeviceBuffer<char> block;
    bool records_stale = false;
    uint32_t refused_capacity = 0;
  } fused;
  DeviceBuffer<uint2> d_sobol;
  int sobol_table = 1;
  int fused_ended = 1;
  int fused_ended_default = 1;
  int bvh_builder = 3;
  double bvh_build_seconds = 0.0;
  uint32_t bvh_meshes_by_builder[2] = {0, 0};
  uint32_t lds_nodes = 0;
  uint32_t trace_blocks = 256;
  DeviceBuffer<uint16_t> d_luts[4];
  DeviceBuffer<uint32_t> d_pixels;
  uint32_t num_pixels = 0;
  uint64_t pixels_hash = 0;
  DeviceBuffer<float> d_first_moment, d_second_moment;
  struct Work : WorkBuffers { DeviceBuffer<char> block; } work;
  uint32_t particle_lds_nodes = 0;
  DeviceBuffer<float> d_frame_output;
  DeviceBuffer<uint16_t> d_bluenoise_1d;
  DeviceBuffer<uint32_t> d_argb8;
  struct Adaptive {
    bool active = false;
    LumAdaptiveParams params{};
    uint32_t blocks_x = 0, blocks_y = 0, num_blocks = 0;
    uint32_t stage_id = 0;
    uint32_t executions[kAdaptiveStages + 1] = {0, 0, 0, 0, 0};
    DeviceBuffer<uint32_t> d_stage_counts, d_block_tasks, d_block_task_end;
    DeviceBuffer<float> d_block_variance;
    DeviceBuffer<float> d_partial;
    DeviceBuffer<char> d_scan_temp;
    size_t scan_temp_bytes = 0;
    std::vector<uint32_t> task_end;
    float variance_total = 0.0f;
    DeviceBuffer<uint8_t> d_block_mask;
    bool build_pending = false;
  } adaptive;
  DeviceBuffer<uint32_t> d_cloud_noise[3];
  bool cloud_noise_static = false;
  uint32_t cloud_noise_seed = 0;
  bool cloud_noise_weather_valid = false;
  DeviceBuffer<float4> d_sky_hdri;
  uint32_t sky_hdri_dim = 0;
  std::vector<DeviceBuffer<float>> bloom_mips;
  uint32_t bloom_width = 0, bloom_height = 0;
  DeviceBuffer<uint32_t> d_undersampling_pixels;
  std::vector<uint32_t> sky_hdri_key;
  DeviceBuffer<float> d_frame_result;
  DeviceBuffer<float> d_guides;
  bool guides_valid = false;
  DeviceBuffer<float4> d_denoise_rec[3];
  int denoise_lds = 1;
  struct RaySort {
    int mode = 0;
    PathQueue queue{};
    DeviceBuffer<float4> planes[4];
    int key = 0;
    DeviceBuffer<uint32_t> d_keys[2], d_vals[2];
    DeviceBuffer<char> d_temp;
    size_t temp_bytes = 0;
    float world_lo[3] = {0, 0, 0}, world_hi[3] = {1, 1, 1};
  } sort;
  bool sync_debug = false;
  struct Exchange {
    ncclComm_t comm = nullptr;
    int comm_rank = 0, comm_world = 1;
    DeviceBuffer<float> d_frame;
    uint32_t frame_pixels() const { return (uint32_t) (d_frame.count() / 4); }
    DeviceBuffer<float> d_gather_send, d_gather_recv;
    DeviceBuffer<uint32_t> d_gather_pixels;
    uint32_t gather_stride = 0, gather_key[3] = {0, 0, 0};
    bool use_frame = false;
  } exchange;
  DeviceBuffer<uint32_t> d_ctrl;
  DeviceBuffer<uint64_t> d_counters;
  bool profiling = false;
  struct Stamp { hipEvent_t a, b; int kernel; };
  std::vector<Stamp> stamps;
  double kernel_ms[LUMC_KERNEL_COUNT] = {};
  uint32_t kernel_launches[LUMC_KERNEL_COUNT] = {};
};

#define HIP_TRY(ctx, expr)                                                                                          \
  do {                                                                                                              \
    const hipError_t e__ = (expr);                                                                                  \
    if (e__ != hipSuccess) {                                                                                        \
      (ctx)->error = std::string(#expr) + " failed: " + hipGetErrorString(e__);                                     \
      return 1;                                                                                                     \
    }                                                                                                               \
  } while (0)

#pragma GCC visibility push(hidden)

constexpr uint32_t kLaunchBlock = 256;
inline uint32_t grid_for(uint32_t n) {
  const uint32_t blocks = (n + kLaunchBlock - 1) / kLaunchBlock;
  return blocks < 1 ? 1 : (blocks > 2048 ? 2048 : blocks);
}

inline uint32_t grid_persistent(const LumContext* ctx, uint32_t n) {
  const uint32_t tb = ctx->wf->trace_block;
  const uint32_t blocks = (n + tb - 1) / tb;
  return blocks < 1 ? 1 : (blocks > ctx->trace_blocks ? ctx->trace_blocks : blocks);
}

struct Launch {
  LumContext* ctx;
  hipStream_t stream;
  int kernel;
  size_t idx = (size_t) -1;
  Launch(LumContext* c, hipStream_t s, int k) : ctx(c), stream(s), kernel(k) {
    if (!ctx->profiling) return;
    LumContext::Stamp st;
    st.kernel = k;
    if (hipEventCreate(&st.a) != hipSuccess || hipEventCreate(&st.b) != hipSuccess) return;
    (void) hipEventRecord(st.a, stream);
    ctx->stamps.push_back(st);
    idx = ctx->stamps.size() - 1;
  }
  ~Launch() {
    if (idx != (size_t) -1) (void) hipEventRecord(ctx->stamps[idx].b, stream);
    if (ctx->sync_debug) {
      const hipError_t e = hipStreamSynchronize(stream);
      std::fprintf(stderr, "[lum] launch group %d: %s\n", kernel, hipGetErrorString(e));
    }
  }
};

const uint32_t* sort_rays(LumContext* ctx, hipStream_t stream, const float4* origin, const float4* dir, const uint32_t* count, uint32_t capacity);
int sort_closest_rays(LumContext* ctx, hipStream_t stream, PathQueue& queue, uint32_t* ctrl, uint32_t N, const uint32_t** order);
void free_sort(LumContext* ctx);
void free_exchange(LumContext* ctx);
int scene_device_init();
extern "C" uint64_t pixel_list_hash(const uint32_t* pixels, uint32_t n);

#pragma GCC visibility pop
extern "C" int adaptive_compute_variance(LumContext* ctx, hipStream_t stream);
extern "C" int adaptive_finish_build(LumContext* ctx, hipStream_t stream);
```

luminary_amd/csrc/host/core.hip:

```cpp
#include <hip/hip_runtime.h>

#include <algorithm>
#include <cmath>
#include <cstdio>
#include <cstdlib>
#include <cstring>
#include <string>
#include <vector>

#include "../../../include/lum_core.h"
#include "../device/kernels_shared.h"
#include <hipcub/hipcub.hpp>
#include "context.h"
#include "tiles.h"

static_assert(kLaunchBlock == (uint32_t) kBlock, "grid_for (context.h) counts the kernels' workgroups");

namespace {

void free_work(LumContext* ctx) {
  ctx->work = LumContext::Work{};
  ctx->fused = LumContext::Fused{};
  free_sort(ctx);
  ctx->d_sobol.reset();
// ... 4 lines not shown
  const uint32_t kinds = volumes ? kVolumeShadowKinds : 4u;
  const bool clouds = ctx->scene.cloud_active && ctx->scene.sky_mode == kSkyDefault;
  if (clouds && paths >= (1u << 30)) { ctx->error = "pass too large for the cloud march list (2^30 paths)"; return 1; }
  if (paths <= ctx->work.capacity && kinds <= ctx->work.shadow_kinds && (!clouds || ctx->work.cloud.items)) return 0;
  if (paths < ctx->work.capacity) paths = ctx->work.capacity;
  free_work(ctx);
  WorkBuffers sized;
  ArenaCarver size(nullptr);
  lay_out_work(size, paths, kinds, clouds, sized);
  HIP_TRY(ctx, ctx->work.block.resize(size.used));
  ArenaCarver arena(ctx->work.block.get());
  lay_out_work(arena, paths, kinds, clouds, ctx->work);
  return 0;
}

int upload_fused_records(LumContext* ctx, hipStream_t stream) {
  FusedResolve by_depth[6];
  for (int d = 0; d < 6; d++) {
    by_depth[d].prev = ctx->work.queue[(d + 2) % 3];
    by_depth[d].nee_prev = (d & 1) ? ctx->work.nee : ctx->fused.nee;
    by_depth[d].fallback = ctx->fused.fallback;
    by_depth[d].ended = ctx->fused.ended[d & 1];
    by_depth[d].ended_prev = ctx->fused.ended[(d & 1) ^ 1];
  }
  HIP_TRY(ctx, hipStreamSynchronize(stream));
  HIP_TRY(ctx, hipMemcpy(ctx->fused.records, by_depth, sizeof(by_depth), hipMemcpyHostToDevice));
  ctx->fused.records_stale = false;
  return 0;
}
int ensure_fused(LumContext* ctx, hipStream_t stream) {
  LumContext::Fused& f = ctx->fused;
  const uint32_t paths = ctx->work.capacity;
  if (f.block && f.capacity == paths) return f.records_stale ? upload_fused_records(ctx, stream) : 0;
  if (f.refused_capacity == paths) return 1;
  FusedBuffers sized;
  ArenaCarver size(nullptr);
  lay_out_fused(size, paths, ctx->work, sized);
  if (f.block.resize(size.used) != hipSuccess) { f.refused_capacity = paths; return 1; }
  ArenaCarver arena(f.block.get());
  lay_out_fused(arena, paths, ctx->work, f);
  ctx->work.queue[2] = f.queue;
  for (int k = 0; k < 3; k++) ctx->work.queue[k].parent = f.parent[k];
  return upload_fused_records(ctx, stream);
}

constexpr uint32_t kCtrlRows = 68;

inline uint32_t shade_grid(const LumContext* ctx, uint32_t n) {
  const uint32_t blocks = (n + kBlock - 1) / kBlock;
  const uint32_t resident = ctx->trace_blocks * 3u;
  const uint32_t rounds = ctx->shade_grid_rounds;
  const uint32_t cap = resident * (rounds ? rounds : 1u);
  return blocks < 1 ? 1 : std::min(blocks, cap);
}

int resolve_stamps(LumContext* ctx) {
  for (auto& st : ctx->stamps) {
    float ms = 0.0f;
    if (hipEventSynchronize(st.b) == hipSuccess && hipEventElapsedTime(&ms, st.a, st.b) == hipSuccess) {
      ctx->kernel_ms[st.kernel] += ms;
      ctx->kernel_launches[st.kernel]++;
    }
    (void) hipEventDestroy(st.a);
    (void) hipEventDestroy(st.b);
  }
  ctx->stamps.clear();
  return 0;
}

}

extern "C" {

int lumc_context_create(int device_ordinal, LumContext** out) {
  if (!out) return 1;
  *out = nullptr;
  LumContext* ctx = new LumContext();
  ctx->device = device_ordinal;
  if (const char* b = getenv("LUM_BVH_BUILDER")) ctx->bvh_builder = (std::strcmp(b, "lbvh") == 0) ? 1 : (std::strcmp(b, "ploc") == 0) ? 2 : (std::strcmp(b, "sah") == 0 || std::strcmp(b, "host") == 0) ? 0 : 3;
  if (const char* e = getenv("LUM_SORT")) ctx->sort.mode = atoi(e);
  if (const char* e = getenv("LUM_SYNC_DEBUG")) ctx->sync_debug = atoi(e) != 0;
  if (const char* e = getenv("LUM_SORT_KEY")) ctx->sort.key = atoi(e);
  if (const char* e = getenv("LUM_AMBIENT_REUSE")) ctx->ambient_reuse = atoi(e) != 0 ? 1 : 0;
  if (const char* e = getenv("LUM_FUSED_RESOLVE")) ctx->fused_resolve = atoi(e) != 0 ? 1 : 0;
  if (const char* e = getenv("LUM_SHADE_GRID")) ctx->shade_grid_rounds = (uint32_t) atoi(e);
  if (const char* e = getenv("LUM_SOBOL_TABLE_RT")) ctx->sobol_table = atoi(e) != 0 ? 1 : 0;
  if (const char* e = getenv("LUM_FUSED_ENDED")) ctx->fused_ended = ctx->fused_ended_default = atoi(e) != 0 ? 1 : 0;
  if (const char* e = getenv("LUM_DENOISE_LDS")) ctx->denoise_lds = atoi(e) != 0 ? 1 : 0;
  if (const char* f = getenv("LUM_FLAVOUR")) ctx->wf = (std::strcmp(f, "exact") == 0) ? wavefront_kernels_exact() : wavefront_kernels_fast();
  *out = ctx;
  int count = 0;
  HIP_TRY(ctx, hipGetDeviceCount(&count));
  if (device_ordinal < 0 || device_ordinal >= count) { ctx->error = "no such HIP device"; return 1; }
  HIP_TRY(ctx, hipSetDevice(device_ordinal));
  HIP_TRY(ctx, (hipError_t) wavefront_kernels_exact()->init_sampler_seeds());
  HIP_TRY(ctx, (hipError_t) wavefront_kernels_fast()->init_sampler_seeds());
  HIP_TRY(ctx, (hipError_t) exact::upload_sampler_seeds());
  HIP_TRY(ctx, (hipError_t) scene_device_init());
  HIP_TRY(ctx, ctx->d_ctrl.resize(kCtlStride * kCtrlRows));
  HIP_TRY(ctx, hipMemset(ctx->d_ctrl.get(), 0, sizeof(uint32_t) * kCtlStride * kCtrlRows));
  HIP_TRY(ctx, ctx->d_counters.resize(LUMC_CNT_COUNT));
  HIP_TRY(ctx, hipMemset(ctx->d_counters.get(), 0, sizeof(uint64_t) * LUMC_CNT_COUNT));
  return 0;
}

void lumc_context_destroy(LumContext* ctx) {
  if (!ctx) return;
  (void) hipSetDevice(ctx->device);
  (void) hipDeviceSynchronize();
  resolve_stamps(ctx);
  free_exchange(ctx);
  delete ctx;
}

const char* lumc_last_error(const LumContext* ctx) { return ctx ? ctx->error.c_str() : "null context"; }
uint32_t lumc_scene_view_sizeof(void) { return (uint32_t) sizeof(LumDeviceSceneView); }

uint64_t pixel_list_hash(const uint32_t* pixels, uint32_t n) {
  uint64_t h = 1469598103934665603ull;
  for (uint32_t i = 0; i < n; i++) { h ^= pixels ? pixels[i] : i; h *= 1099511628211ull; }
  return h;
}

int lumc_set_pixels(LumContext* ctx, const uint32_t* pixels, uint32_t num_pixels) {
  if (!ctx || !ctx->has_scene) { if (ctx) ctx->error = "lumc_set_pixels: no scene"; return 1; }
  HIP_TRY(ctx, hipSetDevice(ctx->device));
  if (!pixels) num_pixels = ctx->scene.width * ctx->scene.height;
  ctx->adaptive = LumContext::Adaptive();
  ctx->d_pixels.reset(); ctx->d_first_moment.reset(); ctx->d_second_moment.reset();
  ctx->num_pixels = num_pixels;
  ctx->pixels_hash = pixel_list_hash(pixels, num_pixels);
  if (num_pixels == 0) return 0;
  HIP_TRY(ctx, ctx->d_pixels.assign(pixels, num_pixels));
  HIP_TRY(ctx, ctx->d_first_moment.resize(3 * (size_t) num_pixels));
  HIP_TRY(ctx, ctx->d_second_moment.resize(num_pixels));
  return lumc_clear_accumulators(ctx);
}

int lumc_clear_accumulators(LumContext* ctx) {
  if (!ctx || !ctx->d_first_moment) return 1;
  HIP_TRY(ctx, hipMemset(ctx->d_first_moment.get(), 0, sizeof(float) * 3 * (size_t) ctx->num_pixels));
  HIP_TRY(ctx, hipMemset(ctx->d_second_moment.get(), 0, sizeof(float) * (size_t) ctx->num_pixels));
  return 0;
}

static void trace_particles(LumContext* ctx, hipStream_t stream, const PathQueue& q, uint32_t* ctrl, uint32_t N) {
  DeviceScene tree = ctx->scene;
  tree.bvh_nodes = tree.particle_bvh_nodes; tree.blas_tris = tree.particle_tris; tree.tlas_leaves = tree.particle_leaves; tree.tlas_num_nodes = tree.particle_tlas_num_nodes; tree.tlas_num_leaves = tree.particle_num_leaves;
  Launch l(ctx, stream, LUMC_KERNEL_TRACE);
  ctx->wf->trace_particles(grid_persistent(ctx, N), (size_t) ctx->particle_lds_nodes * kNodeBytes + LUM_LDS_STACK_BYTES, stream, tree, q, ctrl, ctx->particle_lds_nodes);
}

static bool ambient_reuse_active(const LumContext* ctx) {
  const DeviceScene& sc = ctx->scene;
  const bool wanted = ctx->ambient_reuse < 0 ? (ctx->wf == wavefront_kernels_fast()) : ctx->ambient_reuse != 0;
  return wanted && ctx->has_scene && sc.sky_mode != kSkyDefault && !sc.fog_active && !sc.ocean_active && !sc.particles_active && !sc.cloud_active &&
         !sc.sky_aerial_perspective && ctx->sort.mode == 0 && sc.shading_mode == 0u;
}

static void prepare_sobol_table(LumContext* ctx, hipStream_t stream, DeviceScene& sc, uint32_t first_sample, uint32_t sample_count) {
  sc.sobol_table = nullptr;
  if (!(ctx->sobol_table && sample_count > 0 && sample_count <= kSobolTableMaxSamples && sc.shading_mode == 0u)) return;
  const uint32_t stride = (sample_count + 15u) & ~15u, dims = (sc.max_ray_depth + 1u) * kRndTargetCount;
  const size_t entries = (size_t) stride * dims;
  if (ctx->d_sobol.count() < entries && ctx->d_sobol.resize(entries) != hipSuccess) (void) hipGetLastError();
  if (ctx->d_sobol) {
    ctx->wf->sobol_table(stream, ctx->d_sobol.get(), first_sample, sample_count, stride, dims);
    sc.sobol_table = ctx->d_sobol.get(); sc.sobol_first = first_sample; sc.sobol_count = sample_count; sc.sobol_stride = stride;
  }
}

static size_t ray_kernel_lds(const LumContext* ctx) { return (size_t) ctx->lds_nodes * kNodeBytes + LUM_LDS_STACK_BYTES; }
static bool render_volumes(const DeviceScene& sc) { return sc.fog_active || sc.ocean_active; }

static void first_hits(LumContext* ctx, hipStream_t stream, const DeviceScene& sc, uint32_t N) {
  const WavefrontKernels& wf = *ctx->wf;
  {
    Launch l(ctx, stream, LUMC_KERNEL_TRACE);
    wf.trace(grid_persistent(ctx, N), ray_kernel_lds(ctx), stream, sc, ctx->work.queue[0], nullptr, ctx->d_ctrl.get(), ctx->d_counters.get(), ctx->lds_nodes);
  }
  if (sc.particles_active) trace_particles(ctx, stream, ctx->work.queue[0], ctx->d_ctrl.get(), N);
  if (sc.ocean_active) {
    Launch l(ctx, stream, LUMC_KERNEL_TRACE);
    wf.trace_ocean(grid_for(N), stream, sc, ctx->work.queue[0], (const uint32_t*) ctx->d_ctrl.get());
  }
}

static void debug_pass(LumContext* ctx, hipStream_t stream, const DeviceScene& sc, uint32_t N) {
  const WavefrontKernels& wf = *ctx->wf;
  first_hits(ctx, stream, sc, N);
  if (render_volumes(sc)) {
    Launch l(ctx, stream, LUMC_KERNEL_VOLUME);
    wf.volume_events(grid_for(N), stream, sc, ctx->work.queue[0], ctx->work.volume, ctx->work.results, ctx->d_ctrl.get(), 0u);
  }
  if (sc.sky_aerial_perspective && sc.sky_mode != kSkyConstantColor) {
    Launch l(ctx, stream, LUMC_KERNEL_SKY);
    wf.sky_inscattering(grid_for(N), stream, sc, ctx->work.queue[0], ctx->work.results, (const uint32_t*) ctx->d_ctrl.get(), 0u);
  }
  Launch l(ctx, stream, LUMC_KERNEL_SHADE);
  wf.shade_debug(grid_for(N), stream, sc, ctx->work.queue[0], ctx->work.results, (const uint32_t*) ctx->d_ctrl.get());
}

enum ResolveScheme { kResolvePlain, kResolveReuse, kResolveFused };

struct DepthBuffers {
  PathQueue& cur;
  PathQueue& next;
  PathQueue& prev;
  NeeQueue& nee;
  NeeQueue& nee_before;
  uint32_t* ctrl;
  const FusedResolve* fused_records;
  uint32_t* ended;
  uint32_t depth, depth_const;
  bool last;
};

static DepthBuffers depth_buffers(LumContext* ctx, ResolveScheme scheme, uint32_t depth, uint32_t max_depth) {
  const bool fused = scheme == kResolveFused;
  const int cur = fused ? (int) (depth % 3u) : (int) (depth & 1u);
  const int next_q = fused ? (cur + 1) % 3 : (cur ^ 1), prev_q = fused ? (cur + 2) % 3 : (cur ^ 1);
  const bool second_set = fused && (depth & 1u);
  const uint32_t depth_const = (depth == max_depth && depth > 0) ? depth - 1 : depth;
  return DepthBuffers{ctx->work.queue[cur], ctx->work.queue[next_q], ctx->work.queue[prev_q], second_set ? ctx->fused.nee : ctx->work.nee, second_set ? ctx->work.nee : ctx->fused.nee,
                      ctx->d_ctrl.get() + kCtlStride * depth, fused ? ctx->fused.records + depth % 6u : nullptr, fused ? ctx->fused.ended[depth & 1u] : nullptr, depth, depth_const,
                      depth == max_depth};
}

static int closest_hits(LumContext* ctx, hipStream_t stream, const DeviceScene& sc, ResolveScheme scheme, const DepthBuffers& d, uint32_t N) {
  const WavefrontKernels& wf = *ctx->wf;
  const uint32_t* order = nullptr;
  if (ctx->sort.mode >= 1 && d.depth >= 1 && sort_closest_rays(ctx, stream, d.cur, d.ctrl, N, &order)) return 1;
  {
    Launch l(ctx, stream, LUMC_KERNEL_TRACE);
    wf.trace(grid_persistent(ctx, N), ray_kernel_lds(ctx), stream, sc, d.cur, order, d.ctrl, ctx->d_counters.get(), ctx->lds_nodes);
  }
  if (scheme == kResolveReuse && d.depth > 0) {
    uint32_t* prev = d.ctrl - kCtlStride;
    {
      Launch l(ctx, stream, LUMC_KERNEL_RESOLVE);
      wf.resolve_reuse(grid_for(N), stream, sc, d.prev, d.cur, d.nee, ctx->work.shadow, ctx->work.results, prev, ctx->d_counters.get());
    }
    {
      Launch l(ctx, stream, LUMC_KERNEL_SHADOW);
      wf.shadow_rays(ctx->trace_blocks, ray_kernel_lds(ctx), stream, sc, ctx->work.shadow, nullptr, prev + kCtlVolumeShift, ctx->d_counters.get(), ctx->lds_nodes);
    }
    Launch l(ctx, stream, LUMC_KERNEL_RESOLVE);
    wf.resolve_listed(std::min<uint32_t>(grid_for(N), 1024u), stream, sc, d.prev, d.nee, ctx->work.shadow, ctx->work.results, (const uint32_t*) prev);
  }
  return 0;
}

static void media_passes(LumContext* ctx, hipStream_t stream, const DeviceScene& sc, const DepthBuffers& d, uint32_t N) {
  const WavefrontKernels& wf = *ctx->wf;
  if (sc.particles_active) trace_particles(ctx, stream, d.cur, d.ctrl, N);
  if (sc.ocean_active) {
    Launch l(ctx, stream, LUMC_KERNEL_TRACE);
    wf.trace_ocean(grid_for(N), stream, sc, d.cur, (const uint32_t*) d.ctrl);
  }
  if (render_volumes(sc)) {
    {
      Launch l(ctx, stream, LUMC_KERNEL_VOLUME);
      wf.volume_inscatter(grid_for(N), stream, sc, d.cur, ctx->work.volume, ctx->work.shadow, d.ctrl, d.depth_const);
    }
    {
      Launch l(ctx, stream, LUMC_KERNEL_SHADOW);
      wf.shadow_rays(grid_persistent(ctx, N), ray_kernel_lds(ctx), stream, sc, ctx->work.shadow, nullptr, d.ctrl + kCtlVolumeShift, ctx->d_counters.get(), ctx->lds_nodes);
    }
    Launch l(ctx, stream, LUMC_KERNEL_VOLUME);
    wf.volume_resolve(grid_for(N), stream, sc, d.cur, ctx->work.volume, ctx->work.shadow, ctx->work.results, (const uint32_t*) d.ctrl);
    wf.volume_events(grid_for(N), stream, sc, d.cur, ctx->work.volume, ctx->work.results, d.ctrl, d.depth_const);
  }
  if (sc.cloud_active && sc.sky_mode == kSkyDefault && sc.cloud_noise_shape) {
    Launch l(ctx, stream, LUMC_KERNEL_SKY);
    wf.clouds_list(grid_for(N), stream, sc, d.cur, ctx->work.cloud, d.ctrl);
    wf.clouds_march(ctx->trace_blocks * 4u, stream, sc, d.cur, ctx->work.cloud, d.ctrl, d.depth_const);
    wf.clouds(grid_for(N), stream, sc, d.cur, ctx->work.cloud, ctx->work.results, (const uint32_t*) d.ctrl, d.depth_const);
  }
  if (sc.sky_aerial_perspective && sc.sky_mode != kSkyConstantColor) {
    Launch l(ctx, stream, LUMC_KERNEL_SKY);
    wf.sky_inscattering(grid_for(N), stream, sc, d.cur, ctx->work.results, (const uint32_t*) d.ctrl, d.depth_const);
  }
}

static void shade_depth(LumContext* ctx, hipStream_t stream, const DeviceScene& sc, ResolveScheme scheme, const DepthBuffers& d, uint32_t N) {
  const WavefrontKernels& wf = *ctx->wf;
  const bool fused = scheme == kResolveFused;
  {
    Launch l(ctx, stream, LUMC_KERNEL_SHADE);
    wf.shade(shade_grid(ctx, N), stream, sc, d.cur, d.next, d.nee, ctx->work.shadow, ctx->work.results, d.ctrl, d.depth_const, ctx->d_counters.get(),
             (scheme != kResolvePlain && !d.last) ? 1u : 0u, d.fused_records,
             fused ? ((d.depth > 0 ? 1u : 0u) | (!d.last ? 2u : 0u) | (ctx->fused_ended ? 4u : 0u)) : 0u);
  }
  if (fused && d.depth > 0) {
    {
      Launch l(ctx, stream, LUMC_KERNEL_SHADOW);
      wf.shadow_rays(ctx->trace_blocks, ray_kernel_lds(ctx), stream, sc, ctx->fused.fallback, nullptr, d.ctrl + kCtlVolumeShift, ctx->d_counters.get(), ctx->lds_nodes);
    }
    Launch l(ctx, stream, LUMC_KERNEL_RESOLVE);
    wf.resolve_listed(std::min<uint32_t>(grid_for(N), 1024u), stream, sc, d.prev, d.nee_before, ctx->fused.fallback, ctx->work.results, (const uint32_t*) d.ctrl);
  }
}

static void feature_shading(LumContext* ctx, hipStream_t stream, const DeviceScene& sc, const DepthBuffers& d, uint32_t N) {
  const WavefrontKernels& wf = *ctx->wf;
  if (sc.particles_active) {
    Launch l(ctx, stream, LUMC_KERNEL_SHADE);
    wf.particle_shade(grid_for(N), stream, sc, d.cur, d.next, d.nee, ctx->work.shadow, d.ctrl, d.depth_const);
  }
  if (sc.ocean_active) {
    Launch l(ctx, stream, LUMC_KERNEL_SHADE);
    wf.ocean_shade(grid_for(N), stream, sc, d.cur, d.next, d.nee, ctx->work.shadow, d.ctrl, d.depth_const);
  }
  if (sc.sky_mode == kSkyDefault) {
    Launch l(ctx, stream, LUMC_KERNEL_SKY);
    wf.sky(grid_for(N), stream, sc, d.cur, ctx->work.shadow, ctx->work.results, (const uint32_t*) d.ctrl, d.depth_const);
  }
}

static int visibility_and_resolve(LumContext* ctx, hipStream_t stream, const DeviceScene& sc, ResolveScheme scheme, const DepthBuffers& d, uint32_t N) {
  const WavefrontKernels& wf = *ctx->wf;
  {
    Launch l(ctx, stream, LUMC_KERNEL_LIGHT_QUERY);
    wf.light_query(std::min<uint32_t>(grid_for(N), ctx->trace_blocks * 4u), stream, sc, d.cur, d.nee, ctx->work.shadow, d.ctrl, d.depth_const, ctx->d_counters.get());
  }
  const uint32_t* shadow_order = nullptr;
  if (ctx->sort.mode == 2) {
    shadow_order = sort_rays(ctx, stream, ctx->work.shadow.origin_dist, ctx->work.shadow.dir_out, d.ctrl + kCtlShadowItems,
                             (sc.ocean_active ? kSurfaceShadowKindsWater : 4u) * (ctx->work.shadow.capacity < N ? ctx->work.shadow.capacity : N));
    if (!shadow_order) { ctx->error = "ray sorting failed"; return 1; }
  }
  {
    Launch l(ctx, stream, LUMC_KERNEL_SHADOW);
    wf.shadow_rays(grid_persistent(ctx, N), ray_kernel_lds(ctx), stream, sc, ctx->work.shadow, shadow_order, d.ctrl, ctx->d_counters.get(), ctx->lds_nodes);
  }
  if (d.last || scheme == kResolvePlain) {
    Launch l(ctx, stream, LUMC_KERNEL_RESOLVE);
    wf.resolve(grid_for(N), stream, sc, d.cur, d.nee, ctx->work.shadow, ctx->work.results, (const uint32_t*) d.ctrl);
  }
  else if (scheme == kResolveFused) {
    if (!ctx->fused_ended) {
      Launch l(ctx, stream, LUMC_KERNEL_RESOLVE);
      wf.resolve_ended(std::min<uint32_t>(grid_for(N), 4096u), stream, sc, d.cur, d.nee, ctx->work.shadow, ctx->work.results, (const uint32_t*) d.ctrl, d.ended);
    }
  }
  return 0;
}

static void volume_bounce(LumContext* ctx, hipStream_t stream, const DeviceScene& sc, const DepthBuffers& d, uint32_t N) {
  if (render_volumes(sc) && !d.last) {
    Launch l(ctx, stream, LUMC_KERNEL_VOLUME);
    ctx->wf->volume_bounce(grid_for(N), stream, sc, d.cur, d.next, ctx->work.volume, d.ctrl, d.depth_const);
  }
}

static int wavefront_depths(LumContext* ctx, hipStream_t stream, uint32_t N, uint32_t first_sample = 0, uint32_t sample_count = 0) {
  DeviceScene sc = ctx->scene;
  const uint32_t max_depth = sc.max_ray_depth;
  prepare_sobol_table(ctx, stream, sc, first_sample, sample_count);
  if (sc.shading_mode != 0u) { debug_pass(ctx, stream, sc, N); return 0; }
  ResolveScheme scheme = ambient_reuse_active(ctx) ? kResolveReuse : kResolvePlain;
  if (scheme == kResolveReuse && ctx->wf->fused_resolve && ctx->fused_resolve != 0 && ctx->wf == wavefront_kernels_fast() && max_depth > 0) {
    if (ensure_fused(ctx, stream) == 0) scheme = kResolveFused;
    else {
      (void) hipGetLastError();
      ctx->error.clear();
    }
  }
  for (uint32_t depth = 0; depth <= max_depth; depth++) {
    const DepthBuffers d = depth_buffers(ctx, scheme, depth, max_depth);
    if (closest_hits(ctx, stream, sc, scheme, d, N)) return 1;
    media_passes(ctx, stream, sc, d, N);
    shade_depth(ctx, stream, sc, scheme, d, N);
    feature_shading(ctx, stream, sc, d, N);
    if (visibility_and_resolve(ctx, stream, sc, scheme, d, N)) return 1;
    volume_bounce(ctx, stream, sc, d, N);
  }
  return 0;
}

int lumc_render(LumContext* ctx, uint32_t first_sample, uint32_t num_samples, uint32_t samples_per_pass, float* d_fm, float* d_sm, void* stream_) {
  if (!ctx || !ctx->has_scene) { if (ctx) ctx->error = "lumc_render: no scene"; return 1; }
  if (ctx->num_pixels == 0) return 0;
  hipStream_t stream = (hipStream_t) stream_;
  HIP_TRY(ctx, hipSetDevice(ctx->device));
  if (!d_fm) { d_fm = ctx->d_first_moment.get(); d_sm = ctx->d_second_moment.get(); }
  if (samples_per_pass == 0) samples_per_pass = 1;
  if (first_sample >= kMaxGlobalSamples) return 0;
  if (first_sample + (uint64_t) num_samples > kMaxGlobalSamples) num_samples = kMaxGlobalSamples - first_sample;
  const uint32_t P = ctx->num_pixels;
  const uint64_t want = (uint64_t) P * samples_per_pass;
  if (want > 0x7FFFFFFFull) { ctx->error = "pass too large"; return 1; }
  if (ensure_work(ctx, (uint32_t) want)) return 1;
  const DeviceScene& sc = ctx->scene;
  const uint32_t max_depth = sc.max_ray_depth;

  for (uint32_t done = 0; done < num_samples; done += samples_per_pass) {
    const uint32_t batch = std::min(samples_per_pass, num_samples - done);
    const uint32_t N = P * batch;
    PassParams pp{ctx->d_pixels.get(), P, batch, first_sample + done};
    HIP_TRY(ctx, hipMemsetAsync(ctx->d_ctrl.get(), 0, sizeof(uint32_t) * kCtlStride * (max_depth + 2), stream));
    {
      Launch l(ctx, stream, LUMC_KERNEL_GENERATE);
      ctx->wf->generate(grid_for(N), stream, sc, pp, ctx->work.queue[0], ctx->work.results, ctx->d_ctrl.get() + kCtlPaths, ctx->lens, ctx->camera);
    }
    if (wavefront_depths(ctx, stream, N, first_sample + done, batch)) return 1;
    {
      Launch l(ctx, stream, LUMC_KERNEL_ACCUMULATE);
      hipLaunchKernelGGL(k_accumulate, dim3(grid_for(P)), dim3(kBlock), 0, stream, (const float4*) ctx->work.results, P, batch, d_fm, d_sm);
    }
    HIP_TRY(ctx, hipGetLastError());
  }
  return 0;
}

int lumc_render_undersampled(LumContext* ctx, uint32_t stage, uint32_t iteration, void* stream_) {
  if (!ctx || !ctx->has_scene || !ctx->d_first_moment || ctx->d_pixels || ctx->num_pixels != ctx->scene.width * ctx->scene.height) {
// ... 537 lines not shown
  return 0;
}
int lumc_set_profiling(LumContext* ctx, int enabled) {
  if (!ctx) return 1;
  ctx->profiling = enabled != 0;
  for (int k = 0; k < LUMC_KERNEL_COUNT; k++) { ctx->kernel_ms[k] = 0.0; ctx->kernel_launches[k] = 0; }
  return 0;
}
int lumc_kernel_times(LumContext* ctx, double total_ms[LUMC_KERNEL_COUNT], uint32_t launches[LUMC_KERNEL_COUNT]) {
  if (!ctx) return 1;
  if (lumc_synchronize(ctx)) return 1;
  for (int k = 0; k < LUMC_KERNEL_COUNT; k++) { total_ms[k] = ctx->kernel_ms[k]; launches[k] = ctx->kernel_launches[k]; }
  return 0;
}

extern "C" const unsigned char lum_embedded_bluenoise_1d[];
extern "C" const unsigned char lum_embedded_bluenoise_1d_end[];

int lumc_generate_output(LumContext* ctx, const LumOutputParams* params, const float* d_first_moment, uint32_t* d_argb8, void* stream_) {
  if (!ctx || !params || !d_argb8) { if (ctx) ctx->error = "lumc_generate_output: null argument"; return 1; }
  static_assert(sizeof(LumOutputParams) == sizeof(OutputParams), "output parameter structs must match");
  HIP_TRY(ctx, hipSetDevice(ctx->device));
  hipStream_t stream = (hipStream_t) stream_;
  OutputParams p;
  std::memcpy(&p, params, sizeof(p));
  if (p.src_width == 0 || p.src_height == 0 || p.dst_width < 2 || p.dst_height < 2) { ctx->error = "lumc_generate_output: image sizes must be at least 2x2"; return 1; }
  if (p.supersampling > 3 || p.undersampling_stage > 15) { ctx->error = "lumc_generate_output: supersampling at most 3, undersampling stage at most 15"; return 1; }
  const uint32_t ns = p.src_width * p.src_height;
  const uint32_t uo = std::max(p.undersampling_stage, p.supersampling);
  const uint32_t n_out = (p.src_width >> uo) * (p.src_height >> uo);
  if (n_out == 0) { ctx->error = "lumc_generate_output: the frame is smaller than one output pixel"; return 1; }
  if (!d_first_moment) {
    if (p.undersampling_stage) { ctx->error = "lumc_generate_output: an undersampled image must be passed explicitly (lumc_result_image)"; return 1; }
    if (!ctx->d_first_moment || ctx->d_pixels || ctx->num_pixels != ns) { ctx->error = "lumc_generate_output: the context does not hold a full frame of this size"; return 1; }
    d_first_moment = ctx->d_first_moment.get();
  }
  if (!ctx->d_bluenoise_1d) {
    const size_t bytes = (size_t) (lum_embedded_bluenoise_1d_end - lum_embedded_bluenoise_1d);
    if (bytes != 65536 * sizeof(uint16_t)) { ctx->error = "embedded 1D blue-noise mask has the wrong size"; return 1; }
    HIP_TRY(ctx, ctx->d_bluenoise_1d.assign((const uint16_t*) lum_embedded_bluenoise_1d, 65536));
  }
  if (ctx->d_frame_output.count() < 3 * (size_t) ns) HIP_TRY(ctx, ctx->d_frame_output.resize(3 * (size_t) ns));
  {
    Launch l(ctx, stream, LUMC_KERNEL_OUTPUT);
    hipLaunchKernelGGL(k_final_image, dim3(grid_for(n_out)), dim3(256), 0, stream, p, d_first_moment, ctx->d_frame_output.get());
    hipLaunchKernelGGL(k_to_argb8, dim3(grid_for(p.dst_width * p.dst_height)), dim3(256), 0, stream, p, (const float*) ctx->d_frame_output.get(),
                       (const uint16_t*) ctx->d_bluenoise_1d.get(), d_argb8);
  }
  HIP_TRY(ctx, hipGetLastError());
  return 0;
}

int lumc_generate_output_host(LumContext* ctx, const LumOutputParams* params, const float* d_first_moment, uint32_t* argb8, float* frame_output) {
  if (!ctx || !params || !argb8) { if (ctx) ctx->error = "lumc_generate_output_host: null argument"; return 1; }
  HIP_TRY(ctx, hipSetDevice(ctx->device));
  const uint32_t n = params->dst_width * params->dst_height;
  if (ctx->d_argb8.count() < n) HIP_TRY(ctx, ctx->d_argb8.resize(n));
  if (lumc_generate_output(ctx, params, d_first_moment, ctx->d_argb8.get(), nullptr)) return 1;
  HIP_TRY(ctx, hipDeviceSynchronize());
  HIP_TRY(ctx, hipMemcpy(argb8, ctx->d_argb8.get(), sizeof(uint32_t) * (size_t) n, hipMemcpyDeviceToHost));
  if (frame_output) {
    const uint32_t uo = std::max(params->undersampling_stage, params->supersampling);
    HIP_TRY(ctx, hipMemcpy(frame_output, ctx->d_frame_output.get(), sizeof(float) * 3 * (size_t) (params->src_width >> uo) * (params->src_height >> uo), hipMemcpyDeviceToHost));
  }
  return 0;
}

int lumc_generate_output_from_host(LumContext* ctx, const LumOutputParams* params, const float* first_moment, uint32_t* argb8, float* frame_output) {
  if (!ctx || !params || !first_moment || !argb8) { if (ctx) ctx->error = "lumc_generate_output_from_host: null argument"; return 1; }
  HIP_TRY(ctx, hipSetDevice(ctx->device));
  DeviceBuffer<float> d;
  HIP_TRY(ctx, d.assign(first_moment, 3 * (size_t) (params->src_width >> params->undersampling_stage) * (params->src_height >> params->undersampling_stage)));
  return lumc_generate_output_host(ctx, params, d.get(), argb8, frame_output);
}

int lumc_trace_closest(LumContext* ctx, uint32_t n, const float* d_origins, const float* d_dirs, const uint32_t* d_ignore, uint32_t* d_out, void* stream_) {
  if (!ctx || !ctx->has_scene) { if (ctx) ctx->error = "lumc_trace_closest: no scene"; return 1; }
  if (n == 0) return 0;
  hipStream_t stream = (hipStream_t) stream_;
  uint32_t* cursor = ctx->d_ctrl.get() + kCtlStride * (kCtrlRows - 1);
  HIP_TRY(ctx, hipMemsetAsync(cursor, 0, sizeof(uint32_t), stream));
  Launch l(ctx, stream, LUMC_KERNEL_TRACE);
  ctx->wf->trace_rays(grid_persistent(ctx, n), ray_kernel_lds(ctx), stream, ctx->scene, n, d_origins, d_dirs, d_ignore, d_out, cursor, ctx->d_counters.get(),
                      ctx->lds_nodes);
  HIP_TRY(ctx, hipGetLastError());
  return 0;
}

int lumc_trace_closest_host(LumContext* ctx, uint32_t n, const float* origins, const float* dirs, const uint32_t* ignore, uint32_t* out) {
  if (!ctx || !ctx->has_scene) { if (ctx) ctx->error = "lumc_trace_closest_host: no scene"; return 1; }
  if (n == 0) return 0;
  DeviceBuffer<float> d_o, d_d;
  DeviceBuffer<uint32_t> d_i, d_out;
  HIP_TRY(ctx, d_o.assign(origins, 3 * (size_t) n));
  HIP_TRY(ctx, d_d.assign(dirs, 3 * (size_t) n));
  HIP_TRY(ctx, d_out.resize(3 * (size_t) n));
  HIP_TRY(ctx, d_i.assign(ignore, 2 * (size_t) n));
  if (lumc_trace_closest(ctx, n, d_o.get(), d_d.get(), d_i.get(), d_out.get(), nullptr)) return 1;
  HIP_TRY(ctx, hipMemcpy(out, d_out.get(), sizeof(uint32_t) * 3 * (size_t) n, hipMemcpyDeviceToHost));
  return 0;
}

int lumc_trace_visibility(LumContext* ctx, uint32_t n, const float* d_origins, const float* d_dirs, const float* d_dist, const uint32_t* d_ids, const uint32_t* d_order, float* d_out,
                          void* stream_) {
  if (!ctx || !ctx->has_scene) { if (ctx) ctx->error = "lumc_trace_visibility: no scene"; return 1; }
  if (n == 0) return 0;
  if (!d_origins || !d_dirs || !d_dist || !d_ids || !d_out) { ctx->error = "lumc_trace_visibility: null argument"; return 1; }
  hipStream_t stream = (hipStream_t) stream_;
  HIP_TRY(ctx, hipSetDevice(ctx->device));
  DeviceBuffer<float4> buffer;
  HIP_TRY(ctx, buffer.resize(4 * (size_t) n));
  float4* items = buffer.get();
  ShadowQueue sq{};
  sq.origin_dist = items; sq.dir_out = items + n; sq.ids = reinterpret_cast<uint4*>(items + 2 * (size_t) n); sq.vis = items + 3 * (size_t) n;
  sq.capacity = n;
  uint32_t* ctrl = ctx->d_ctrl.get() + kCtlStride * (kCtrlRows - 2);
  const uint32_t blocks = (n + 255u) / 256u;
  HIP_TRY(ctx, hipMemsetAsync(sq.vis, 0xFF, sizeof(float4) * (size_t) n, stream));
  HIP_TRY(ctx, hipMemsetD32Async((hipDeviceptr_t) (ctrl + kCtlShadowItems), (int) n, 1, stream));
  HIP_TRY(ctx, hipMemsetAsync(ctrl + kCtlShadowCursor, 0, sizeof(uint32_t), stream));
  hipLaunchKernelGGL(k_visibility_pack, dim3(blocks), dim3(256), 0, stream, n, d_origins, d_dirs, d_dist, d_ids, sq);
  {
    Launch l(ctx, stream, LUMC_KERNEL_SHADOW);
    ctx->wf->shadow_rays(grid_persistent(ctx, n), ray_kernel_lds(ctx), stream, ctx->scene, sq, d_order, ctrl, ctx->d_counters.get(), ctx->lds_nodes);
  }
  hipLaunchKernelGGL(k_visibility_unpack, dim3(blocks), dim3(256), 0, stream, n, sq.vis, d_out);
  HIP_TRY(ctx, hipGetLastError());
  HIP_TRY(ctx, hipStreamSynchronize(stream));
  return 0;
}

int lumc_trace_visibility_host(LumContext* ctx, uint32_t n, const float* origins, const float* dirs, const float* dist, const uint32_t* ids, const uint32_t* order, float* out) {
  if (!ctx || !ctx->has_scene) { if (ctx) ctx->error = "lumc_trace_visibility_host: no scene"; return 1; }
  if (n == 0) return 0;
  if (!origins || !dirs || !dist || !ids || !out) { ctx->error = "lumc_trace_visibility_host: null argument"; return 1; }
  if (order) {
    for (uint32_t i = 0; i < n; i++) if (order[i] >= n) { ctx->error = "lumc_trace_visibility_host: order entry out of range"; return 1; }
  }
  HIP_TRY(ctx, hipSetDevice(ctx->device));
  DeviceBuffer<float> d_o, d_d, d_t, d_out;
  DeviceBuffer<uint32_t> d_i, d_ord;
  HIP_TRY(ctx, d_o.assign(origins, 3 * (size_t) n));
  HIP_TRY(ctx, d_d.assign(dirs, 3 * (size_t) n));
  HIP_TRY(ctx, d_t.assign(dist, n));
  HIP_TRY(ctx, d_i.assign(ids, 4 * (size_t) n));
  HIP_TRY(ctx, d_ord.assign(order, n));
  HIP_TRY(ctx, d_out.resize(3 * (size_t) n));
  if (lumc_trace_visibility(ctx, n, d_o.get(), d_d.get(), d_t.get(), d_i.get(), d_ord.get(), d_out.get(), nullptr)) return 1;
  HIP_TRY(ctx, hipMemcpy(out, d_out.get(), sizeof(float) * 3 * (size_t) n, hipMemcpyDeviceToHost));
  return 0;
}

int lumc_light_query_host(LumContext* ctx, uint32_t n, const float* origins, const float* dirs, const uint32_t* self, const float* randoms, uint32_t* out_ids, uint32_t* out_num_hits) {
  if (!ctx || !ctx->has_scene) { if (ctx) ctx->error = "lumc_light_query_host: no scene"; return 1; }
  if (n == 0) return 0;
  if (!origins || !dirs || !self || !randoms || !out_ids || !out_num_hits) { ctx->error = "lumc_light_query_host: null argument"; return 1; }
  const DeviceScene& sc = ctx->scene;
  if (!sc.num_lights || !sc.light_nodes || !sc.light_tris || !sc.light_tri_handles) {
    for (uint32_t i = 0; i < n; i++) { out_ids[i] = 0xFFFFFFFFu; out_num_hits[i] = 0u; }
    return 0;
  }
  HIP_TRY(ctx, hipSetDevice(ctx->device));
  DeviceBuffer<float> d_o, d_d, d_r;
  DeviceBuffer<uint32_t> d_s, d_out;
  HIP_TRY(ctx, d_o.assign(origins, 3 * (size_t) n));
  HIP_TRY(ctx, d_d.assign(dirs, 3 * (size_t) n));
  HIP_TRY(ctx, d_s.assign(self, 2 * (size_t) n));
  HIP_TRY(ctx, d_r.assign(randoms, n));
  HIP_TRY(ctx, d_out.resize(2 * (size_t) n));
  HIP_TRY(ctx, hipMemset(d_out.get(), 0xFF, sizeof(uint32_t) * 2 * (size_t) n));
  ctx->wf->light_query_probe(nullptr, sc, n, d_o.get(), d_d.get(), d_s.get(), d_r.get(), d_out.get(), d_out.get() + n);
  HIP_TRY(ctx, hipGetLastError());
  HIP_TRY(ctx, hipDeviceSynchronize());
  HIP_TRY(ctx, hipMemcpy(out_ids, d_out.get(), sizeof(uint32_t) * (size_t) n, hipMemcpyDeviceToHost));
  HIP_TRY(ctx, hipMemcpy(out_num_hits, d_out.get() + n, sizeof(uint32_t) * (size_t) n, hipMemcpyDeviceToHost));
  return 0;
}

int lumc_pixel_query(LumContext* ctx, uint32_t x, uint32_t y, uint32_t sample_id, uint32_t out[6]) {
  if (!ctx || !ctx->has_scene || !out) { if (ctx) ctx->error = "lumc_pixel_query: no scene"; return 1; }
  if (x >= ctx->scene.width || y >= ctx->scene.height) { ctx->error = "lumc_pixel_query: pixel outside the frame"; return 1; }
  HIP_TRY(ctx, hipSetDevice(ctx->device));
  DeviceBuffer<float> buffer;
  HIP_TRY(ctx, buffer.resize(10));
  float* d = buffer.get();
  hipLaunchKernelGGL(k_pixel_ray, dim3(1), dim3(64), 0, 0, ctx->scene, ctx->lens, ctx->camera, x, y, sample_id, d, d + 3, (uint32_t*) (d + 9));
  uint32_t valid = 0;
  HIP_TRY(ctx, hipMemcpy(&valid, d + 9, 4, hipMemcpyDeviceToHost));
  if (valid && lumc_trace_closest(ctx, 1, d, d + 3, nullptr, (uint32_t*) (d + 6), nullptr)) return 1;
  HIP_TRY(ctx, hipDeviceSynchronize());
  if (valid) HIP_TRY(ctx, hipMemcpy(out, d + 6, 12, hipMemcpyDeviceToHost));
  else { out[0] = 0xFFFFFFFFu; out[1] = 0u; std::memcpy(&out[2], &kFltMax, 4); }
  HIP_TRY(ctx, hipMemcpy(out + 3, d + 3, 12, hipMemcpyDeviceToHost));
  return 0;
}

int lumc_set_physical_camera(LumContext* ctx, const LumPhysicalCamera* c) {
  if (!ctx) return 1;
  ctx->guides_valid = false;
  if (!c) { ctx->camera = kCamThinLens; return 0; }
  if (c->num_interfaces == 0 || c->num_interfaces > LUMC_LENS_MAX_INTERFACES) { ctx->error = "lumc_set_physical_camera: 1 ... 24 interfaces"; return 1; }
  const uint32_t n = c->num_interfaces;
  bool finite = std::isfinite(c->aperture_point) && std::isfinite(c->aperture_radius) && std::isfinite(c->exit_pupil_point) && std::isfinite(c->exit_pupil_radius) &&
                std::isfinite(c->image_plane_distance) && std::isfinite(c->sensor_width);
  bool ior_ok = true;
  for (uint32_t i = 0; i < n; i++) {
    const LumLensInterface& f = c->interfaces[i];
    finite = finite && std::isfinite(f.radius) && std::isfinite(f.vertex) && std::isfinite(f.cylindrical_radius);
  }
  for (uint32_t i = 0; i <= n; i++) {
    const LumLensMedium& m = c->media[i];
    finite = finite && std::isfinite(m.design_ior) && std::isfinite(m.abbe) && std::isfinite(m.cylindrical_radius);
    ior_ok = ior_ok && m.design_ior > 0.0f;
  }
  if (!finite) { ctx->error = "lumc_set_physical_camera: non-finite parameter"; return 1; }
  if (!(c->exit_pupil_radius > 0.0f) || !(c->aperture_radius > 0.0f)) { ctx->error = "lumc_set_physical_camera: exit pupil and aperture must be larger than 0"; return 1; }
  if (!ior_ok) { ctx->error = "lumc_set_physical_camera: index of refraction <= 0"; return 1; }
  static_assert(sizeof(LumLensInterface) == sizeof(LensInterface) && sizeof(LumLensMedium) == sizeof(LensMedium), "lens tables: one layout");
  DeviceLens l{};
  l.aperture_point = c->aperture_point; l.aperture_radius = c->aperture_radius; l.exit_pupil_point = c->exit_pupil_point; l.exit_pupil_radius = c->exit_pupil_radius;
  l.image_plane_distance = c->image_plane_distance; l.sensor_width = c->sensor_width; l.num_interfaces = n;
  std::memcpy(l.iface, c->interfaces, sizeof(LensInterface) * n);
  std::memcpy(l.medium, c->media, sizeof(LensMedium) * (n + 1));
  ctx->lens = l;
  ctx->camera = c->allow_reflections ? kCamPhysicalReflections : kCamPhysical;
  return 0;
}

int lumc_camera_rays(LumContext* ctx, const uint32_t* pixels, uint32_t n, uint32_t first_sample, uint32_t samples, float* out_origin, float* out_dir, float* out_weight) {
  if (!ctx || !ctx->has_scene || !pixels || !out_origin || !out_dir || !out_weight) { if (ctx) ctx->error = "lumc_camera_rays: no scene or null argument"; return 1; }
  const uint64_t total = (uint64_t) n * samples;
  if (total == 0) return 0;
  if (total > 0x7FFFFFFFull) { ctx->error = "lumc_camera_rays: too many rays"; return 1; }
  for (uint32_t p = 0; p < n; p++)
    if (pixels[p] >= ctx->scene.width * ctx->scene.height) { ctx->error = "lumc_camera_rays: pixel outside the frame"; return 1; }
  HIP_TRY(ctx, hipSetDevice(ctx->device));
  DeviceBuffer<uint32_t> d_px;
  DeviceBuffer<float> rays;
  HIP_TRY(ctx, d_px.resize(n));
  HIP_TRY(ctx, rays.resize(7 * (size_t) total));
  HIP_TRY(ctx, hipMemcpy(d_px.get(), pixels, sizeof(uint32_t) * (size_t) n, hipMemcpyHostToDevice));
  float* d = rays.get();
  ctx->wf->camera_rays(grid_for((uint32_t) total), 0, ctx->scene, ctx->lens, ctx->camera, d_px.get(), n, first_sample, samples, d, d + 3 * total, d + 6 * total);
  HIP_TRY(ctx, hipGetLastError());
  HIP_TRY(ctx, hipDeviceSynchronize());
  HIP_TRY(ctx, hipMemcpy(out_origin, d, sizeof(float) * 3 * total, hipMemcpyDeviceToHost));
  HIP_TRY(ctx, hipMemcpy(out_dir, d + 3 * total, sizeof(float) * 3 * total, hipMemcpyDeviceToHost));
  HIP_TRY(ctx, hipMemcpy(out_weight, d + 6 * total, sizeof(float) * total, hipMemcpyDeviceToHost));
  return 0;
}

int lumc_device_name(int ordinal, char* out, size_t size) {
  if (!out || size == 0) return 1;
  hipDeviceProp_t prop;
  if (hipGetDeviceProperties(&prop, ordinal) != hipSuccess) { out[0] = 0; return 1; }
  std::snprintf(out, size, "%s", prop.name);
  return 0;
}

int lumc_set_flavour(LumContext* ctx, int flavour) {
  if (!ctx || flavour < 0 || flavour > 1) { if (ctx) ctx->error = "lumc_set_flavour: 0 (exact) or 1 (fast)"; return 1; }
  ctx->wf = flavour == LUMC_FLAVOUR_FAST ? wavefront_kernels_fast() : wavefront_kernels_exact();
  return 0;
}
int lumc_set_fused_resolve(LumContext* ctx, int on) {
  if (!ctx) return 1;
  ctx->fused_resolve = on != 0 ? 1 : 0;
  ctx->fused_ended = on == 2 ? 0 : ctx->fused_ended_default;
  return 0;
}
int lumc_set_sobol_table(LumContext* ctx, int on) {
  if (!ctx) return 1;
  ctx->sobol_table = on != 0 ? 1 : 0;
  return 0;
}
int lumc_set_ambient_reuse(LumContext* ctx, int mode) {
  if (!ctx || mode < -1 || mode > 1) { if (ctx) ctx->error = "lumc_set_ambient_reuse: -1 (by flavour), 0 (off) or 1 (on)"; return 1; }
  ctx->ambient_reuse = mode;
  return 0;
}
int lumc_get_ambient_reuse(const LumContext* ctx) { return (ctx && ambient_reuse_active(ctx)) ? 1 : 0; }
int lumc_get_flavour(const LumContext* ctx) { return (ctx && ctx->wf == wavefront_kernels_exact()) ? LUMC_FLAVOUR_EXACT : LUMC_FLAVOUR_FAST; }

unsigned int lumc_lds_stack_bytes(void) { return LUM_LDS_STACK_BYTES; }

}
```

luminary_amd/csrc/host/scene_device.hip:

```cpp
#include <hip/hip_runtime.h>

#include <algorithm>
#include <chrono>
#include <cmath>
#include <cfloat>
#include <cstring>
#include <map>
#include <mutex>
#include <tuple>

#include "../../../include/lum_core.h"
#include "../device/kernels_scene.h"
#include "context.h"

namespace {

struct MeshTreeKey {
  uint64_t h0, h1, env;
  uint32_t tris; int builder;
  bool operator<(const MeshTreeKey& o) const { return std::tie(h0, h1, env, tris, builder) < std::tie(o.h0, o.h1, o.env, o.tris, o.builder); }
};
static std::mutex g_mesh_tree_mutex;
static std::map<MeshTreeKey, std::weak_ptr<const MeshTree>> g_mesh_trees;
extern "C" char** environ;
// ... 337 lines not shown
  const auto t_all = clock::now();
  BvhTri* d_tris = ctx->arrays.mesh.blas_tris.get();
  if (!d_tris) { ctx->error = "lumc_scene_update: the scene on the device has no traversal triangles"; return 1; }
  if (!arrays_uploaded && update_mesh_arrays(ctx, v)) return 1;
  HIP_TRY(ctx, hipDeviceSynchronize());
  st.seconds_upload = since(t_all);
  for (uint32_t m = 0; m < v->num_meshes; m++) {
    const uint32_t t0 = v->mesh_tri_offset[m], nt = v->mesh_tri_offset[m + 1] - t0;
    if (nt == 0) continue;
    const float* vertices = v->vertices + (size_t) t0 * 12;
    MeshRefit& mr = ctx->mesh_refit[m];
    const auto t_hash = clock::now();
    const MeshTreeKey key = mesh_tree_key(vertices, nt, ctx->bvh_builder);
    st.seconds_hash += since(t_hash);
    if (key.h0 == mr.fit_hash[0] && key.h1 == mr.fit_hash[1]) continue;
    bool build = ctx->refit_mode == 1;
    if (!build) {
      const auto t_refit = clock::now();
      if (mr.built_cost == 0.0) mr.built_cost = bvh4_cost(ctx->mesh_bvh[m]->bvh);
      if (!mr.plan.nodes) {
        const hipError_t e = refit_plan_create(mr.plan, ctx->mesh_bvh[m]->bvh, nt);
        if (e == hipErrorInvalidValue) build = true;
        else HIP_TRY(ctx, e);
      }
      if (!build) {
        if (!mr.own) {
          mr.own = std::make_shared<MeshTree>();
          mr.own->bvh.prims = ctx->mesh_bvh[m]->bvh.prims; mr.own->bvh.max_depth = ctx->mesh_bvh[m]->bvh.max_depth; mr.own->built_on_gpu = ctx->mesh_bvh[m]->built_on_gpu;
          mr.own->bvh.nodes.resize(mr.plan.num_nodes);
        }
        Aabb box;
        double download = 0.0;
        HIP_TRY(ctx, refit_run(mr.plan, sc.vertices + 3 * (size_t) t0, d_tris + t0, nullptr, mr.own->bvh.nodes.data(), &box, &download));
        st.seconds_download += download;
        const double growth = mr.built_cost > 0.0 ? bvh4_cost(mr.own->bvh) / mr.built_cost : 1.0;
        st.max_cost_growth = std::max(st.max_cost_growth, growth);
        if (ctx->refit_max_cost_growth > 0.0f && growth > (double) ctx->refit_max_cost_growth) build = true;
        else { ctx->mesh_bvh[m] = mr.own; ctx->mesh_box[m] = box; mesh_boxes_changed(ctx); st.refits++; st.last_refits++; }
      }
      st.seconds_refit += since(t_refit);
    }
    if (build) {
      const auto t_build = clock::now();
      std::vector<Aabb> tri_boxes(nt);
      ctx->mesh_box[m] = mesh_triangle_boxes(vertices, nt, tri_boxes.data());
      mesh_boxes_changed(ctx);
      std::shared_ptr<const MeshTree> tree = cached_or_built_mesh_tree(ctx, key, tri_boxes.data(), nt);
      if (!tree) return 1;
      std::vector<BvhTri> tris(nt);
      fill_mesh_tris(vertices, t0, tree->bvh.prims.data(), nt, tris.data());
      HIP_TRY(ctx, hipMemcpy(d_tris + t0, tris.data(), sizeof(BvhTri) * nt, hipMemcpyHostToDevice));
      mr.plan.reset(); mr.own.reset();
      mr.built_cost = bvh4_cost(tree->bvh);
      ctx->mesh_bvh[m] = std::move(tree);
      *rebuilt = true;
      st.rebuilds++; st.last_rebuilds++;
      st.seconds_rebuild += since(t_build);
    }
    mr.fit_hash[0] = key.h0; mr.fit_hash[1] = key.h1;
  }
  st.seconds = since(t_all);
  return 0;
}

static int update_scene_tree(LumContext* ctx, const LumDeviceSceneView* v, bool dirty_meshes, size_t* num_nodes) {
  DeviceScene& sc = ctx->scene;
  std::vector<BvhTri> blas_tris;
  if (!dirty_meshes && restore_stale_meshes(ctx)) return 1;
  if (dirty_meshes && build_mesh_trees(ctx, v, blas_tris)) return 1;
  if (ctx->mesh_box.size() != v->num_meshes || ctx->mesh_bvh.size() != v->num_meshes) { ctx->error = "lumc_scene_update: the meshes changed but LUMC_DIRTY_MESHES is not set"; return 1; }
  std::vector<const Bvh4*> mesh_bvh(v->num_meshes);
  for (uint32_t m = 0; m < v->num_meshes; m++) mesh_bvh[m] = &ctx->mesh_bvh[m]->bvh;
  const SceneTree tree = assemble_scene_tree(*v, mesh_bvh.data(), ctx->mesh_box.data());
  if (tree.nodes.empty()) { ctx->error = "top-level BVH exceeds 16 levels"; return 1; }
  if (total_triangles(v) >= (1u << 28) || tree.nodes.size() >= (1u << 25)) { ctx->error = "scene too large for 28-bit leaf ranges / 32-bit node offsets"; return 1; }
  if (upload(ctx, ctx->arrays.inst.rows, tree.inv_rows.data(), tree.inv_rows.size(), &sc.instance_rows)) return 1;
  ctx->instance_update.resident = false;
  ctx->resident_refit.drop_layout();
  if (upload(ctx, ctx->arrays.inst.nodes, tree.nodes.data(), tree.nodes.size(), &sc.bvh_nodes)) return 1;
  if (dirty_meshes && upload(ctx, ctx->arrays.mesh.blas_tris, blas_tris.data(), blas_tris.size(), &sc.blas_tris)) return 1;
  if (upload(ctx, ctx->arrays.inst.tlas_leaves, tree.tlas_leaves.data(), tree.tlas_leaves.size(), &sc.tlas_leaves)) return 1;
  sc.tlas_num_nodes = tree.tlas_num_nodes;
  sc.tlas_num_leaves = (uint32_t) (tree.tlas_leaves.size() / 4);
  std::memcpy(ctx->sort.world_lo, tree.world.lo, sizeof(ctx->sort.world_lo)); std::memcpy(ctx->sort.world_hi, tree.world.hi, sizeof(ctx->sort.world_hi));
  ctx->bvh_stats[0] = tree.nodes.size() - tree.tlas_num_nodes;
  ctx->bvh_stats[2] = tree.tlas_num_nodes;
  *num_nodes = tree.nodes.size();
  return 0;
}

static int update_ray_kernel_lds(LumContext* ctx, size_t num_nodes) {
  hipDeviceProp_t prop;
  HIP_TRY(ctx, hipGetDeviceProperties(&prop, ctx->device));
  size_t lds_bytes = prop.maxSharedMemoryPerMultiProcessor ? prop.maxSharedMemoryPerMultiProcessor : prop.sharedMemPerBlock;
  lds_bytes = std::min<size_t>(lds_bytes, 160 * 1024);
  lds_bytes = lds_bytes > 16384 ? lds_bytes - 8192 : 0;
  lds_bytes = lds_bytes > LUM_LDS_STACK_BYTES ? lds_bytes - LUM_LDS_STACK_BYTES : 0;
  ctx->lds_nodes = (uint32_t) std::min<size_t>(lds_bytes / kNodeBytes, num_nodes);
  if (const char* e = getenv("LUM_LDS_NODES")) ctx->lds_nodes = std::min<uint32_t>((uint32_t) atoi(e), ctx->lds_nodes);
  ctx->trace_blocks = (uint32_t) prop.multiProcessorCount;
  const size_t dyn = lds_bytes + LUM_LDS_STACK_BYTES;
  HIP_TRY(ctx, (hipError_t) wavefront_kernels_exact()->set_ray_kernel_lds(dyn));
  HIP_TRY(ctx, (hipError_t) wavefront_kernels_fast()->set_ray_kernel_lds(dyn));
  return 0;
}

static int relayout_resident(LumContext* ctx, const LumDeviceSceneView* v) {
  DeviceScene& sc = ctx->scene;
  InstanceUpdate& u = ctx->instance_update;
  SceneArrays::Inst& a = ctx->arrays.inst;
  const uint32_t n = v->num_instances, capacity = std::max<uint32_t>(1u, n > 0 ? n - 1u : 0u);
  if (restore_stale_meshes(ctx)) return 1;
  ResidentRefit& rr = ctx->resident_refit;
  rr.drop_layout();
  std::vector<const Bvh4*> mesh_bvh(v->num_meshes);
  for (uint32_t m = 0; m < v->num_meshes; m++) mesh_bvh[m] = &ctx->mesh_bvh[m]->bvh;
  std::vector<Bvh4Node> nodes;
  std::vector<uint32_t> mesh_root;
  layout_resident_nodes(*v, mesh_bvh.data(), capacity, nodes, mesh_root, ctx->refit_in_place ? &rr.mesh_slots : nullptr);
  if (total_triangles(v) >= (1u << 28) || nodes.size() >= (1u << 25)) { ctx->error = "scene too large for 28-bit leaf ranges / 32-bit node offsets"; return 1; }
  a.nodes.reset(); a.tlas_leaves.reset(); point_views(sc, a);
  if (upload(ctx, a.nodes, nodes.data(), nodes.size(), &sc.bvh_nodes)) return 1;
  HIP_TRY(ctx, a.tlas_leaves.resize(4 * ((size_t) n + 1)));
  sc.tlas_leaves = a.tlas_leaves.get();
  HIP_TRY(ctx, hipMemset(a.tlas_leaves.get(), 0, sizeof(float4) * 4 * ((size_t) n + 1)));
  HIP_TRY(ctx, u.mesh_root.assign(mesh_root.data(), v->num_meshes));
  u.capacity = capacity; u.mesh_nodes = (uint32_t) (nodes.size() - capacity); u.tlas_nodes = 0;
  rr.capacity = u.capacity; rr.mesh_nodes = u.mesh_nodes;
  if (update_ray_kernel_lds(ctx, nodes.size())) return 1;
  u.resident = true;
  return 0;
}

static int update_instance_transforms(LumContext* ctx, const LumDeviceSceneView* v, bool* fell_back, bool layout_only = false, bool upload = true) {
  using clock = std::chrono::steady_clock;
  auto since = [](clock::time_point t) { return std::chrono::duration<double>(clock::now() - t).count(); };
  DeviceScene& sc = ctx->scene;
  InstanceUpdate& u = ctx->instance_update;
  SceneArrays::Inst& a = ctx->arrays.inst;
  LumInstanceUpdateStats& st = ctx->instance_stats;
  st.seconds = st.seconds_relayout = st.seconds_upload = st.seconds_boxes = st.seconds_build = st.seconds_leaves = 0.0;
  *fell_back = false;
  const uint32_t n = v->num_instances;
  if (n != sc.num_instances || ctx->instance_mesh_ids.size() != n || ctx->mesh_bvh.size() != v->num_meshes || ctx->mesh_box.size() != v->num_meshes ||
      (n && std::memcmp(ctx->instance_mesh_ids.data(), v->instance_mesh_ids, sizeof(uint32_t) * n) != 0)) {
    ctx->error = "lumc_scene_update: LUMC_DIRTY_INSTANCE_TRANSFORMS with another instance count or other mesh ids than the scene on the device";
    return 1;
  }
  const auto t_all = clock::now();
  if (!u.prepared || u.num_instances != n || u.num_meshes != v->num_meshes) {
    u.reset();
    if (instance_update_prepare(u, n, v->num_meshes, ctx->mesh_box.data()) != hipSuccess) { (void) hipGetLastError(); u.reset(); *fell_back = true; return 0; }
  }
  auto t = clock::now();
  if (n && upload) HIP_TRY(ctx, hipMemcpy(a.transforms.get(), v->instance_transforms, sizeof(float4) * 2 * (size_t) n, hipMemcpyHostToDevice));
  HIP_TRY(ctx, hipDeviceSynchronize());
  st.seconds_upload = since(t);
  t = clock::now();
  uint32_t hittable = 0;
  Aabb world;
  HIP_TRY(ctx, instance_update_boxes(u, sc.instance_transforms, sc.instance_mesh_ids, sc.mesh_tri_offset, a.rows.get(), &hittable, &world));
  st.seconds_boxes = since(t);
  if (hittable < 2) { *fell_back = true; return 0; }
  if (!u.resident) {
    t = clock::now();
    if (relayout_resident(ctx, v)) { (void) hipGetLastError(); ctx->error.clear(); *fell_back = true; return 0; }
    HIP_TRY(ctx, hipDeviceSynchronize());
    st.relayouts++;
    st.seconds_relayout = since(t);
  }
  if (layout_only) return 0;
  t = clock::now();
  uint32_t num_nodes = 0, depth = 0;
  Bvh4Node* d_nodes = a.nodes.get();
  if (!build_bvh4_sah_device(u.dense_boxes.get(), hittable, 1, 16, d_nodes, u.capacity, u.prims.get(), &num_nodes, &depth)) {
    (void) hipGetLastError();
    *fell_back = true;
    return 0;
  }
  st.seconds_build = since(t);
  t = clock::now();
  HIP_TRY(ctx, instance_update_leaves(u, hittable, sc.instance_rows, sc.instance_mesh_ids, a.tlas_leaves.get(), d_nodes, num_nodes, std::max(num_nodes, u.tlas_nodes)));
  HIP_TRY(ctx, hipDeviceSynchronize());
  st.seconds_leaves = since(t);
  u.tlas_nodes = num_nodes;
  sc.tlas_num_nodes = num_nodes;
  sc.tlas_num_leaves = hittable + 1u;
  std::memcpy(ctx->sort.world_lo, world.lo, sizeof(ctx->sort.world_lo)); std::memcpy(ctx->sort.world_hi, world.hi, sizeof(ctx->sort.world_hi));
  ctx->bvh_stats[0] = u.mesh_nodes;
  ctx->bvh_stats[2] = num_nodes;
  st.device_updates++;
  st.tlas_nodes = num_nodes; st.tlas_depth = depth; st.tlas_capacity = u.capacity; st.hittable = hittable;
  st.seconds = since(t_all);
  return 0;
}

static int refit_in_place(LumContext* ctx, const LumDeviceSceneView* v, bool* fell_back) {
  using clock = std::chrono::steady_clock;
  auto since = [](clock::time_point t) { return std::chrono::duration<double>(clock::now() - t).count(); };
  DeviceScene& sc = ctx->scene;
  InstanceUpdate& u = ctx->instance_update;
  ResidentRefit& rr = ctx->resident_refit;
  LumMeshRefitStats& st = ctx->refit_stats;
  LumResidentRefitStats& rs = ctx->resident_stats;
  st.last_refits = st.last_rebuilds = 0; st.max_cost_growth = st.seconds = st.seconds_upload = st.seconds_refit = st.seconds_rebuild = st.seconds_assemble = 0.0;
  st.seconds_hash = st.seconds_download = st.seconds_lights = 0.0;
  rs.last_meshes = rs.last_launches = 0; rs.last_bytes_downloaded = 0;
  rs.seconds = rs.seconds_upload = rs.seconds_hash = rs.seconds_refit = rs.seconds_cost = rs.seconds_top_level = 0.0;
  *fell_back = false;
  if (ctx->mesh_bvh.size() != v->num_meshes || ctx->mesh_refit.size() != v->num_meshes || ctx->mesh_tri_offset.size() != (size_t) v->num_meshes + 1 ||
      std::memcmp(ctx->mesh_tri_offset.data(), v->mesh_tri_offset, sizeof(uint32_t) * ((size_t) v->num_meshes + 1)) != 0) {
    ctx->error = "lumc_scene_update: LUMC_DIRTY_MESH_POSITIONS with other meshes or triangle counts than the scene on the device";
    return 1;
  }
  const auto t_all = clock::now();
  BvhTri* d_tris = ctx->arrays.mesh.blas_tris.get();
  if (!d_tris) { ctx->error = "lumc_scene_update: the scene on the device has no traversal triangles"; return 1; }
  if (update_mesh_arrays(ctx, v)) return 1;
  HIP_TRY(ctx, hipDeviceSynchronize());
  rs.seconds_upload = st.seconds_upload = since(t_all);
  auto t = clock::now();
  std::vector<uint32_t> moved;
  std::vector<MeshTreeKey> keys;
  for (uint32_t m = 0; m < v->num_meshes; m++) {
    const uint32_t t0 = v->mesh_tri_offset[m], nt = v->mesh_tri_offset[m + 1] - t0;
    if (nt == 0) continue;
    const MeshTreeKey key = mesh_tree_key(v->vertices + (size_t) t0 * 12, nt, ctx->bvh_builder);
    if (key.h0 == ctx->mesh_refit[m].fit_hash[0] && key.h1 == ctx->mesh_refit[m].fit_hash[1]) continue;
    if (ctx->mesh_bvh[m]->bvh.prims.size() != nt) { *fell_back = true; return 0; }
    moved.push_back(m); keys.push_back(key);
  }
  rs.seconds_hash = st.seconds_hash = since(t);
  t = clock::now();
  if (!u.resident || !u.prepared || u.num_instances != v->num_instances || u.num_meshes != v->num_meshes || rr.mesh_slots.size() != v->num_meshes) {
    if (u.resident && rr.mesh_slots.size() != v->num_meshes) {
      if (restore_stale_meshes(ctx)) return 1;
      u.resident = false;
    }
    if (update_instance_transforms(ctx, v, fell_back, true)) return 1;
    if (*fell_back) return 0;
    if (!u.resident || !u.prepared || rr.mesh_slots.size() != v->num_meshes) { *fell_back = true; return 0; }
  }
  if (moved.empty()) { rs.seconds = since(t_all); st.seconds = rs.seconds; return 0; }
  if (rr.mesh.size() != v->num_meshes) { rr.mesh.clear(); rr.mesh.resize(v->num_meshes); rr.batch.clear(); }
  for (uint32_t m : moved) {
    MeshRefit& mr = ctx->mesh_refit[m];
    if (mr.built_cost == 0.0) mr.built_cost = bvh4_cost(ctx->mesh_bvh[m]->bvh);
    if (rr.mesh[m].slots) continue;
    const hipError_t e = resident_mesh_create(rr.mesh[m], ctx->mesh_bvh[m]->bvh, v->mesh_tri_offset[m + 1] - v->mesh_tri_offset[m], rr.mesh_slots[m]);
    if (e != hipSuccess) { (void) hipGetLastError(); *fell_back = true; return 0; }
  }
  if (resident_refit_prepare(rr, moved, v->mesh_tri_offset, u.mesh_nodes) != hipSuccess) { (void) hipGetLastError(); *fell_back = true; return 0; }
  std::vector<ResidentResult> results(moved.size());
  uint32_t launches = 0;
  double seconds[2] = {0.0, 0.0};
  HIP_TRY(ctx, resident_refit_run(rr, sc.vertices, d_tris, ctx->arrays.inst.nodes.get(), u.capacity, u.mesh_nodes, u.mesh_box.get(), u.num_meshes, results.data(), &launches, seconds));
  for (uint32_t m : moved) if (!ctx->mesh_refit[m].stale) { ctx->mesh_refit[m].stale = true; ctx->stale_meshes++; }
  rs.seconds_cost = seconds[1];
  rs.seconds_refit = since(t) - seconds[1];
  double max_growth = 0.0;
  bool grown = false;
  for (size_t j = 0; j < moved.size(); j++) {
    const MeshRefit& mr = ctx->mesh_refit[moved[j]];
    const double growth = mr.built_cost > 0.0 ? results[j].cost / mr.built_cost : 1.0;
    max_growth = std::max(max_growth, growth);
    if (ctx->refit_max_cost_growth > 0.0f && growth > (double) ctx->refit_max_cost_growth) grown = true;
  }
  if (grown) {
    *fell_back = true;
    return 0;
// ... 499 lines not shown
```

Baseline: 3828.

## Add single-level traversal kernels for scenes with one instance

Adds templated trace, shadow and trace_rays kernels that skip the two-level TLAS/instance logic when the scene has exactly one instance. These kernels pre-transform rays into the single instance's space and start traversal at its BLAS root. They also drop the enter-instance vote, the leave-instance handling and the LDS staging of TLAS leaves. The intent is to remove per-ray instance-enter overhead and divergence. The cost is extra kernel variants, and the fast flavour only allows this path when the first leaf transform is the identity.

```diff
diff --git a/include/lum_core.h b/include/lum_core.h
--- a/include/lum_core.h
+++ b/include/lum_core.h
@@ -241,6 +241,8 @@
 int lumc_get_flavour(const LumContext* ctx);
 int lumc_set_ambient_reuse(LumContext* ctx, int mode);
 int lumc_get_ambient_reuse(const LumContext* ctx);
+int lumc_set_single_level(LumContext* ctx, int mode);
+int lumc_get_single_level(const LumContext* ctx);
 int lumc_set_fused_resolve(LumContext* ctx, int on);
 int lumc_set_sobol_table(LumContext* ctx, int on);
 double lumc_bvh_build_seconds(const LumContext* ctx);
diff --git a/luminary_amd/core.py b/luminary_amd/core.py
--- a/luminary_amd/core.py
+++ b/luminary_amd/core.py
@@ -233,6 +233,14 @@
         fn.restype = C.c_int
         return bool(fn(self._ctx))
 
+    def set_single_level(self, mode):
+        self._call("lumc_set_single_level", C.c_int(mode))
+
+    def get_single_level(self):
+        fn = self._lib.lumc_get_single_level
+        fn.restype = C.c_int
+        return int(fn(self._ctx))
+
     def set_physical_camera(self, camera):
         self._call("lumc_set_physical_camera", C.byref(camera) if camera is not None else C.c_void_p(0))
 
diff --git a/luminary_amd/csrc/device/dev_trace.h b/luminary_amd/csrc/device/dev_trace.h
--- a/luminary_amd/csrc/device/dev_trace.h
+++ b/luminary_amd/csrc/device/dev_trace.h
@@ -193,7 +193,12 @@
   }
 };
 
-template <class Q>
+template <bool kSingleLevel> struct OneInstance {};
+template <> struct OneInstance<true> { float4 r0, r1, r2; uint32_t inst, root; };
+LUM_DEV uint32_t instance_of(const OneInstance<false>&, uint32_t entered) { return entered; }
+LUM_DEV uint32_t instance_of(const OneInstance<true>& one, uint32_t) { return one.inst; }
+
+template <class Q, bool kSingleLevel = false>
 LUM_DEV void trace_items(const DeviceScene& sc, uint32_t n, uint32_t* __restrict__ cursor, Q& q, RayStats& st, uint32_t& rays, uint32_t lds_count) {
   if (n == 0u) return;
   using SE = StackEntry<Q::kCull>;
@@ -214,10 +219,18 @@
     for (uint32_t i = threadIdx.x; i < lds_count * (kNodeBytes / 16u); i += blockDim.x) lds_top[i] = g[i];
     __syncthreads();
   }
-  __shared__ float4 lds_leaves[4u * LUM_LDS_INSTANCES];
-  const uint32_t staged_leaves = min(sc.tlas_num_leaves, (uint32_t) LUM_LDS_INSTANCES);
-  for (uint32_t i = threadIdx.x; i < 4u * staged_leaves; i += blockDim.x) lds_leaves[i] = sc.tlas_leaves[i];
-  __syncthreads();
+  __shared__ float4 lds_leaves[kSingleLevel ? 1u : 4u * LUM_LDS_INSTANCES];
+  const uint32_t staged_leaves = kSingleLevel ? 0u : min(sc.tlas_num_leaves, (uint32_t) LUM_LDS_INSTANCES);
+  if constexpr (!kSingleLevel) {
+    for (uint32_t i = threadIdx.x; i < 4u * staged_leaves; i += blockDim.x) lds_leaves[i] = sc.tlas_leaves[i];
+    __syncthreads();
+  }
+  [[maybe_unused]] OneInstance<kSingleLevel> one;
+  if constexpr (kSingleLevel) {
+    const float4* __restrict__ leaf = sc.tlas_leaves;
+    const float4 meta = leaf[3];
+    one.r0 = leaf[0]; one.r1 = leaf[1]; one.r2 = leaf[2]; one.inst = fbits(meta.x); one.root = fbits(meta.y);
+  }
   const NodeSource nodes{sc.bvh_nodes, reinterpret_cast<const char*>(lds_top), lds_count};
   typedef typename TraversalStack<E>::W StackW;
   static_assert(sizeof(StackW) == sizeof(E), "a stack entry is one machine word");
@@ -235,6 +248,17 @@
     LUM_PHASE(6); LUM_PHASE_LANES(7);
     bool left_instance = false, again;
     E e;
+    if constexpr (kSingleLevel) {
+      do {
+        e = top;
+        const bool done = SE::node(e) == kTraversalDone;
+        if (!done) { sp--; top = stk.load(sp); }
+        again = !done && !SE::reachable(e, tmax);
+      } while (again);
+      cur = SE::node(e);
+      (void) left_instance;
+      return;
+    }
     do {
       e = top;
       const bool done = SE::node(e) == kTraversalDone, leave = SE::node(e) == kLeaveInstance;
@@ -276,8 +300,21 @@
             const uint32_t e = 0x7F800000u;
             const bool finite = (fbits(wo.x) & e) != e && (fbits(wo.y) & e) != e && (fbits(wo.z) & e) != e && (fbits(wd.x) & e) != e && (fbits(wd.y) & e) != e &&
                                 (fbits(wd.z) & e) != e;
-            if (finite) { r.set(wo, wd); cur = 0; sp = 0; top = SE::make(kTraversalDone, 0.0f); inst = kNoInstance; }
-            else q.finish(sc, idx);
+            if constexpr (kSingleLevel) {
+              if (finite) {
+                const float4 r0 = one.r0, r1 = one.r1, r2 = one.r2;
+                const float px = wo.x - r0.w, py = wo.y - r1.w, pz = wo.z - r2.w;
+                const V3 oo = v3(mat_row_apply(r0.x, r0.y, r0.z, px, py, pz), mat_row_apply(r1.x, r1.y, r1.z, px, py, pz), mat_row_apply(r2.x, r2.y, r2.z, px, py, pz));
+                const V3 od = v3(mat_row_apply(r0.x, r0.y, r0.z, wd.x, wd.y, wd.z), mat_row_apply(r1.x, r1.y, r1.z, wd.x, wd.y, wd.z),
+                                 mat_row_apply(r2.x, r2.y, r2.z, wd.x, wd.y, wd.z));
+                r.set(oo, od); cur = one.root; sp = 0; top = SE::make(kTraversalDone, 0.0f);
+              }
+              else q.finish(sc, idx);
+            }
+            else {
+              if (finite) { r.set(wo, wd); cur = 0; sp = 0; top = SE::make(kTraversalDone, 0.0f); inst = kNoInstance; }
+              else q.finish(sc, idx);
+            }
           }
         }
         chunk_next += min(want, avail);
@@ -292,12 +329,13 @@
     while (true) {
       const bool live = cur != kTraversalDone;
       const bool at_leaf = live && (cur & kBvhLeafBit);
-      const bool want_tris = at_leaf && inst != kNoInstance, want_enter = at_leaf && inst == kNoInstance;
-      const uint32_t n_live = (uint32_t) __popcll(__ballot(live)), n_tris = (uint32_t) __popcll(__ballot(want_tris)), n_enter = (uint32_t) __popcll(__ballot(want_enter));
+      const bool want_tris = at_leaf && (kSingleLevel || inst != kNoInstance), want_enter = !kSingleLevel && at_leaf && inst == kNoInstance;
+      const uint32_t n_live = (uint32_t) __popcll(__ballot(live)), n_tris = (uint32_t) __popcll(__ballot(want_tris)),
+                     n_enter = kSingleLevel ? 0u : (uint32_t) __popcll(__ballot(want_enter));
       if (n_live == 0u) break;
       const uint32_t n_nodes = n_live - n_tris - n_enter;
       const bool run_tris = n_tris * LUM_VOTE_TRIS >= max(n_nodes, n_enter) * LUM_VOTE_NODES;
-      const bool run_enter = !run_tris && n_enter >= n_nodes;
+      const bool run_enter = !kSingleLevel && !run_tris && n_enter >= n_nodes;
       const bool do_tris = run_tris && want_tris, do_enter = run_enter && want_enter, do_node = !run_tris && !run_enter && live && !at_leaf;
       LUM_TIME_BEGIN();
 #ifdef LUM_PHASE_STATS
@@ -306,12 +344,12 @@
       {
         if (do_tris) {
           LUM_PHASE(3); LUM_PHASE_LANES(4);
-          if (q.on_tris(sc, inst, cur & 0x0FFFFFFFu, ((cur >> 28) & 0x7u) + 1u, r.o, r.d, tmax, st)) cur = kTraversalDone;
+          if (q.on_tris(sc, instance_of(one, inst), cur & 0x0FFFFFFFu, ((cur >> 28) & 0x7u) + 1u, r.o, r.d, tmax, st)) cur = kTraversalDone;
           else pop();
           if (cur == kTraversalDone) q.finish(sc, idx);
         }
       }
-      {
+      if constexpr (!kSingleLevel) {
         if (do_enter) {
           LUM_PHASE(1); LUM_PHASE_LANES(2);
           const uint32_t leaf_index = cur & 0x0FFFFFFFu;
diff --git a/luminary_amd/csrc/device/kernel_shadow.h b/luminary_amd/csrc/device/kernel_shadow.h
--- a/luminary_amd/csrc/device/kernel_shadow.h
+++ b/luminary_amd/csrc/device/kernel_shadow.h
@@ -29,8 +29,11 @@
   }
 };
 
+template <bool kSingleLevel>
+__global__ LUM_TRACE_BOUNDS void k_shadow_rays(DeviceScene sc, ShadowQueue sq, const uint32_t* order, uint32_t* ctrl, uint64_t* counters, uint32_t lds_nodes);
 #if LUM_SHADOW_KERNEL_EXTERN
 __global__ LUM_TRACE_BOUNDS void k_shadow_rays(DeviceScene sc, ShadowQueue sq, const uint32_t* order, uint32_t* ctrl, uint64_t* counters, uint32_t lds_nodes);
+extern template __global__ void k_shadow_rays<true>(DeviceScene sc, ShadowQueue sq, const uint32_t* order, uint32_t* ctrl, uint64_t* counters, uint32_t lds_nodes);
 #else
 __global__ LUM_TRACE_BOUNDS void k_shadow_rays(DeviceScene sc, ShadowQueue sq, const uint32_t* order, uint32_t* ctrl, uint64_t* counters, uint32_t lds_nodes) {
   RayStats st{0, 0, 0};
@@ -41,6 +44,18 @@
   trace_items(sc, ctrl[kCtlShadowItems], ctrl + kCtlShadowCursor, q, st, rays, lds_nodes);
   flush_stats(counters, st, rays, kCntShadow, kCntNodesShadow, kCntTrisShadow, kCntNodesLdsShadow);
 }
+template <bool kSingleLevel>
+__global__ LUM_TRACE_BOUNDS void k_shadow_rays(DeviceScene sc, ShadowQueue sq, const uint32_t* order, uint32_t* ctrl, uint64_t* counters, uint32_t lds_nodes) {
+  static_assert(kSingleLevel, "the two-level form is the plain kernel of this name");
+  RayStats st{0, 0, 0};
+  uint32_t rays = 0;
+  ShadowQuery q;
+  q.sq = sq;
+  q.order = order;
+  trace_items<ShadowQuery, true>(sc, ctrl[kCtlShadowItems], ctrl + kCtlShadowCursor, q, st, rays, lds_nodes);
+  flush_stats(counters, st, rays, kCntShadow, kCntNodesShadow, kCntTrisShadow, kCntNodesLdsShadow);
+}
+template __global__ void k_shadow_rays<true>(DeviceScene sc, ShadowQueue sq, const uint32_t* order, uint32_t* ctrl, uint64_t* counters, uint32_t lds_nodes);
 #endif
 
 LUM_NS_END
diff --git a/luminary_amd/csrc/device/kernels.h b/luminary_amd/csrc/device/kernels.h
--- a/luminary_amd/csrc/device/kernels.h
+++ b/luminary_amd/csrc/device/kernels.h
@@ -200,6 +200,18 @@
   tq.order = order;
   tq.item = 0;
   trace_items(sc, ctrl[kCtlPaths], ctrl + kCtlTraceCursor, tq, st, rays, lds_nodes);
+  flush_stats(counters, st, rays, kCntTrace, kCntNodes, kCntTris, kCntNodesLds);
+}
+template <bool kSingleLevel>
+__global__ LUM_TRACE_BOUNDS void k_trace(DeviceScene sc, PathQueue q, const uint32_t* order, uint32_t* ctrl, uint64_t* counters, uint32_t lds_nodes) {
+  static_assert(kSingleLevel, "the two-level form is the plain kernel of this name");
+  RayStats st{0, 0, 0};
+  uint32_t rays = 0;
+  TraceQuery tq;
+  tq.q = q;
+  tq.order = order;
+  tq.item = 0;
+  trace_items<TraceQuery, true>(sc, ctrl[kCtlPaths], ctrl + kCtlTraceCursor, tq, st, rays, lds_nodes);
   flush_stats(counters, st, rays, kCntTrace, kCntNodes, kCntTris, kCntNodesLds);
 }
 
@@ -1796,6 +1808,17 @@
   trace_items(sc, n, cursor, q, st, rays, lds_nodes);
   flush_stats(counters, st, rays, kCntTrace, kCntNodes, kCntTris, kCntNodesLds);
 }
+template <bool kSingleLevel>
+__global__ LUM_TRACE_BOUNDS void k_trace_rays(DeviceScene sc, uint32_t n, const float* origins, const float* dirs, const uint32_t* ignore,
+                                                           uint32_t* out, uint32_t* cursor, uint64_t* counters, uint32_t lds_nodes) {
+  static_assert(kSingleLevel, "the two-level form is the plain kernel of this name");
+  RayStats st{0, 0, 0};
+  uint32_t rays = 0;
+  RaysQuery q;
+  q.origins = origins; q.dirs = dirs; q.ignore = ignore; q.out = out;
+  trace_items<RaysQuery, true>(sc, n, cursor, q, st, rays, lds_nodes);
+  flush_stats(counters, st, rays, kCntTrace, kCntNodes, kCntTris, kCntNodesLds);
+}
 
 __global__ __launch_bounds__(kBlock) void k_light_query_probe(DeviceScene sc, uint32_t n, const float* origins, const float* dirs, const uint32_t* self, const float* randoms,
                                                               uint32_t* out_ids, uint32_t* out_num_hits) {
diff --git a/luminary_amd/csrc/device/wavefront_table.h b/luminary_amd/csrc/device/wavefront_table.h
--- a/luminary_amd/csrc/device/wavefront_table.h
+++ b/luminary_amd/csrc/device/wavefront_table.h
@@ -5,6 +5,8 @@
 #include "dev_scene.h"
 
 namespace lum {
+
+inline bool single_level_scene(const DeviceScene& sc) { return sc.tlas_num_nodes == 1u && sc.tlas_num_leaves == 2u; }
 
 struct WavefrontKernels {
   const char* flavour;
@@ -17,7 +19,7 @@
   void (*generate_adaptive)(uint32_t grid, hipStream_t s, const DeviceScene& sc, const AdaptiveView& a, const AdaptivePass& pass, const PathQueue& q, float4* results,
                             uint32_t* count, const DeviceLens& lens, int cam);
   void (*trace)(uint32_t grid, size_t lds, hipStream_t s, const DeviceScene& sc, const PathQueue& q, const uint32_t* order, uint32_t* ctrl, uint64_t* counters,
-                uint32_t lds_nodes);
+                uint32_t lds_nodes, bool single_level);
   void (*sky_inscattering)(uint32_t grid, hipStream_t s, const DeviceScene& sc, const PathQueue& in, float4* results, const uint32_t* ctrl, uint32_t depth_const);
   void (*shade)(uint32_t grid, hipStream_t s, const DeviceScene& sc, const PathQueue& in, const PathQueue& out, const NeeQueue& nee, const ShadowQueue& sq, float4* results,
                 uint32_t* ctrl, uint32_t depth_const, uint64_t* counters, uint32_t ambient_reuse, const FusedResolve* fused_dev, uint32_t fused_flags);
@@ -26,7 +28,7 @@
   void (*light_query)(uint32_t grid, hipStream_t s, const DeviceScene& sc, const PathQueue& in, const NeeQueue& nee, const ShadowQueue& sq, uint32_t* ctrl, uint32_t depth_const,
                       uint64_t* counters);
   void (*shadow_rays)(uint32_t grid, size_t lds, hipStream_t s, const DeviceScene& sc, const ShadowQueue& sq, const uint32_t* order, uint32_t* ctrl, uint64_t* counters,
-                      uint32_t lds_nodes);
+                      uint32_t lds_nodes, bool single_level);
   void (*resolve)(uint32_t grid, hipStream_t s, const DeviceScene& sc, const PathQueue& in, const NeeQueue& nee, const ShadowQueue& sq, float4* results, const uint32_t* ctrl);
   void (*resolve_reuse)(uint32_t grid, hipStream_t s, const DeviceScene& sc, const PathQueue& in, const PathQueue& next, const NeeQueue& nee, const ShadowQueue& sq, float4* results,
                         uint32_t* ctrl, uint64_t* counters);
@@ -51,7 +53,7 @@
   void (*clouds_march)(uint32_t grid, hipStream_t s, const DeviceScene& sc, const PathQueue& in, const CloudQueue& cq, uint32_t* ctrl, uint32_t depth_const);
   void (*clouds)(uint32_t grid, hipStream_t s, const DeviceScene& sc, const PathQueue& in, const CloudQueue& cq, float4* results, const uint32_t* ctrl, uint32_t depth_const);
   void (*trace_rays)(uint32_t grid, size_t lds, hipStream_t s, const DeviceScene& sc, uint32_t n, const float* origins, const float* dirs, const uint32_t* ignore, uint32_t* out,
-                     uint32_t* cursor, uint64_t* counters, uint32_t lds_nodes);
+                     uint32_t* cursor, uint64_t* counters, uint32_t lds_nodes, bool single_level);
   void (*camera_rays)(uint32_t grid, hipStream_t s, const DeviceScene& sc, const DeviceLens& lens, int cam, const uint32_t* pixels, uint32_t n, uint32_t first_sample,
                       uint32_t samples, float* origin, float* dir, float* weight);
   void (*guide)(uint32_t grid, hipStream_t s, const DeviceScene& sc, const PathQueue& in, const uint32_t* ctrl, float* planes, uint32_t n);
diff --git a/luminary_amd/csrc/device/wavefront_table_impl.h b/luminary_amd/csrc/device/wavefront_table_impl.h
--- a/luminary_amd/csrc/device/wavefront_table_impl.h
+++ b/luminary_amd/csrc/device/wavefront_table_impl.h
@@ -7,10 +7,20 @@
 LUM_NS_BEGIN
 namespace table {
 
+typedef void (*TraceKernel)(DeviceScene, PathQueue, const uint32_t*, uint32_t*, uint64_t*, uint32_t);
+typedef void (*ShadowKernel)(DeviceScene, ShadowQueue, const uint32_t*, uint32_t*, uint64_t*, uint32_t);
+typedef void (*TraceRaysKernel)(DeviceScene, uint32_t, const float*, const float*, const uint32_t*, uint32_t*, uint32_t*, uint64_t*, uint32_t);
+static TraceKernel trace_kernel(bool single) { return single ? k_trace<true> : static_cast<TraceKernel>(k_trace); }
+static ShadowKernel shadow_kernel(bool single) { return single ? k_shadow_rays<true> : static_cast<ShadowKernel>(k_shadow_rays); }
+static TraceRaysKernel trace_rays_kernel(bool single) { return single ? k_trace_rays<true> : static_cast<TraceRaysKernel>(k_trace_rays); }
+
 static int set_ray_kernel_lds(size_t bytes) {
-  hipError_t e = hipFuncSetAttribute((const void*) k_trace, hipFuncAttributeMaxDynamicSharedMemorySize, (int) bytes);
-  if (e == hipSuccess) e = hipFuncSetAttribute((const void*) k_shadow_rays, hipFuncAttributeMaxDynamicSharedMemorySize, (int) bytes);
-  if (e == hipSuccess) e = hipFuncSetAttribute((const void*) k_trace_rays, hipFuncAttributeMaxDynamicSharedMemorySize, (int) bytes);
+  hipError_t e = hipSuccess;
+  for (int single = 0; single < 2 && e == hipSuccess; single++) {
+    e = hipFuncSetAttribute((const void*) trace_kernel(single != 0), hipFuncAttributeMaxDynamicSharedMemorySize, (int) bytes);
+    if (e == hipSuccess) e = hipFuncSetAttribute((const void*) shadow_kernel(single != 0), hipFuncAttributeMaxDynamicSharedMemorySize, (int) bytes);
+    if (e == hipSuccess) e = hipFuncSetAttribute((const void*) trace_rays_kernel(single != 0), hipFuncAttributeMaxDynamicSharedMemorySize, (int) bytes);
+  }
   if (e == hipSuccess) e = hipFuncSetAttribute((const void*) k_trace_particles, hipFuncAttributeMaxDynamicSharedMemorySize, (int) bytes);
   return (int) e;
 }
@@ -35,8 +45,8 @@
   hipLaunchKernelGGL(k, dim3(grid), dim3(kBlock), 0, s, sc, lens, pixels, n, first_sample, samples, origin, dir, weight);
 }
 static void trace(uint32_t grid, size_t lds, hipStream_t s, const DeviceScene& sc, const PathQueue& q, const uint32_t* order, uint32_t* ctrl, uint64_t* counters,
-                  uint32_t lds_nodes) {
-  hipLaunchKernelGGL(k_trace, dim3(grid), dim3(kTraceBlock), lds, s, sc, q, order, ctrl, counters, lds_nodes);
+                  uint32_t lds_nodes, bool single_level) {
+  hipLaunchKernelGGL(trace_kernel(single_level && single_level_scene(sc)), dim3(grid), dim3(kTraceBlock), lds, s, sc, q, order, ctrl, counters, lds_nodes);
 }
 static void sky_inscattering(uint32_t grid, hipStream_t s, const DeviceScene& sc, const PathQueue& in, float4* results, const uint32_t* ctrl, uint32_t depth_const) {
   hipLaunchKernelGGL(k_sky_inscattering, dim3(grid), dim3(kBlock), 0, s, sc, in, results, ctrl, depth_const);
@@ -62,8 +72,8 @@
   hipLaunchKernelGGL(k_light_query, dim3(grid), dim3(kBlock), 0, s, sc, in, nee, sq, ctrl, depth_const, counters);
 }
 static void shadow_rays(uint32_t grid, size_t lds, hipStream_t s, const DeviceScene& sc, const ShadowQueue& sq, const uint32_t* order, uint32_t* ctrl, uint64_t* counters,
-                        uint32_t lds_nodes) {
-  hipLaunchKernelGGL(k_shadow_rays, dim3(grid), dim3(kTraceBlock), lds, s, sc, sq, order, ctrl, counters, lds_nodes);
+                        uint32_t lds_nodes, bool single_level) {
+  hipLaunchKernelGGL(shadow_kernel(single_level && single_level_scene(sc)), dim3(grid), dim3(kTraceBlock), lds, s, sc, sq, order, ctrl, counters, lds_nodes);
 }
 static void resolve(uint32_t grid, hipStream_t s, const DeviceScene& sc, const PathQueue& in, const NeeQueue& nee, const ShadowQueue& sq, float4* results, const uint32_t* ctrl) {
   hipLaunchKernelGGL(k_resolve, dim3(grid), dim3(kBlock), 0, s, sc, in, nee, sq, results, ctrl);
@@ -119,8 +129,9 @@
   hipLaunchKernelGGL(k_clouds, dim3(grid), dim3(kBlock), 0, s, sc, in, cq, results, ctrl, depth_const);
 }
 static void trace_rays(uint32_t grid, size_t lds, hipStream_t s, const DeviceScene& sc, uint32_t n, const float* origins, const float* dirs, const uint32_t* ignore, uint32_t* out,
-                       uint32_t* cursor, uint64_t* counters, uint32_t lds_nodes) {
-  hipLaunchKernelGGL(k_trace_rays, dim3(grid), dim3(kTraceBlock), lds, s, sc, n, origins, dirs, ignore, out, cursor, counters, lds_nodes);
+                       uint32_t* cursor, uint64_t* counters, uint32_t lds_nodes, bool single_level) {
+  hipLaunchKernelGGL(trace_rays_kernel(single_level && single_level_scene(sc)), dim3(grid), dim3(kTraceBlock), lds, s, sc, n, origins, dirs, ignore, out, cursor, counters,
+                     lds_nodes);
 }
 static void guide(uint32_t grid, hipStream_t s, const DeviceScene& sc, const PathQueue& in, const uint32_t* ctrl, float* planes, uint32_t n) {
   hipLaunchKernelGGL(k_guide, dim3(grid), dim3(kBlock), 0, s, sc, in, ctrl, planes, n);
diff --git a/luminary_amd/csrc/host/context.h b/luminary_amd/csrc/host/context.h
--- a/luminary_amd/csrc/host/context.h
+++ b/luminary_amd/csrc/host/context.h
@@ -61,6 +61,8 @@
   bool has_scene = false;
   uint64_t bvh_stats[4] = {0, 0, 0, 0};
   int ambient_reuse = -1;
+  int single_level = -1;
+  bool first_leaf_identity = false;
   uint32_t shade_grid_rounds = 2;
   int fused_resolve = 1;
   struct Fused : FusedBuffers {
@@ -165,6 +167,10 @@
   return blocks < 1 ? 1 : (blocks > 2048 ? 2048 : blocks);
 }
 
+inline bool single_level_allowed(const LumContext* ctx) {
+  return ctx->single_level != 0 && (ctx->wf != wavefront_kernels_fast() || ctx->first_leaf_identity);
+}
+
 inline uint32_t grid_persistent(const LumContext* ctx, uint32_t n) {
   const uint32_t tb = ctx->wf->trace_block;
   const uint32_t blocks = (n + tb - 1) / tb;
diff --git a/luminary_amd/csrc/host/core.hip b/luminary_amd/csrc/host/core.hip
--- a/luminary_amd/csrc/host/core.hip
+++ b/luminary_amd/csrc/host/core.hip
@@ -110,6 +110,7 @@
   if (const char* e = getenv("LUM_SYNC_DEBUG")) ctx->sync_debug = atoi(e) != 0;
   if (const char* e = getenv("LUM_SORT_KEY")) ctx->sort.key = atoi(e);
   if (const char* e = getenv("LUM_AMBIENT_REUSE")) ctx->ambient_reuse = atoi(e) != 0 ? 1 : 0;
+  if (const char* e = getenv("LUM_SINGLE_LEVEL")) ctx->single_level = atoi(e) != 0 ? 1 : 0;
   if (const char* e = getenv("LUM_FUSED_RESOLVE")) ctx->fused_resolve = atoi(e) != 0 ? 1 : 0;
   if (const char* e = getenv("LUM_SHADE_GRID")) ctx->shade_grid_rounds = (uint32_t) atoi(e);
   if (const char* e = getenv("LUM_SOBOL_TABLE_RT")) ctx->sobol_table = atoi(e) != 0 ? 1 : 0;
@@ -205,7 +206,7 @@
   const WavefrontKernels& wf = *ctx->wf;
   {
     Launch l(ctx, stream, LUMC_KERNEL_TRACE);
-    wf.trace(grid_persistent(ctx, N), ray_kernel_lds(ctx), stream, sc, ctx->work.queue[0], nullptr, ctx->d_ctrl.get(), ctx->d_counters.get(), ctx->lds_nodes);
+    wf.trace(grid_persistent(ctx, N), ray_kernel_lds(ctx), stream, sc, ctx->work.queue[0], nullptr, ctx->d_ctrl.get(), ctx->d_counters.get(), ctx->lds_nodes, single_level_allowed(ctx));
   }
   if (sc.particles_active) trace_particles(ctx, stream, ctx->work.queue[0], ctx->d_ctrl.get(), N);
   if (sc.ocean_active) {
@@ -261,7 +262,7 @@
   if (ctx->sort.mode >= 1 && d.depth >= 1 && sort_closest_rays(ctx, stream, d.cur, d.ctrl, N, &order)) return 1;
   {
     Launch l(ctx, stream, LUMC_KERNEL_TRACE);
-    wf.trace(grid_persistent(ctx, N), ray_kernel_lds(ctx), stream, sc, d.cur, order, d.ctrl, ctx->d_counters.get(), ctx->lds_nodes);
+    wf.trace(grid_persistent(ctx, N), ray_kernel_lds(ctx), stream, sc, d.cur, order, d.ctrl, ctx->d_counters.get(), ctx->lds_nodes, single_level_allowed(ctx));
   }
   if (scheme == kResolveReuse && d.depth > 0) {
     uint32_t* prev = d.ctrl - kCtlStride;
@@ -271,7 +272,7 @@
     }
     {
       Launch l(ctx, stream, LUMC_KERNEL_SHADOW);
-      wf.shadow_rays(ctx->trace_blocks, ray_kernel_lds(ctx), stream, sc, ctx->work.shadow, nullptr, prev + kCtlVolumeShift, ctx->d_counters.get(), ctx->lds_nodes);
+      wf.shadow_rays(ctx->trace_blocks, ray_kernel_lds(ctx), stream, sc, ctx->work.shadow, nullptr, prev + kCtlVolumeShift, ctx->d_counters.get(), ctx->lds_nodes, single_level_allowed(ctx));
     }
     Launch l(ctx, stream, LUMC_KERNEL_RESOLVE);
     wf.resolve_listed(std::min<uint32_t>(grid_for(N), 1024u), stream, sc, d.prev, d.nee, ctx->work.shadow, ctx->work.results, (const uint32_t*) prev);
@@ -293,7 +294,7 @@
     }
     {
       Launch l(ctx, stream, LUMC_KERNEL_SHADOW);
-      wf.shadow_rays(grid_persistent(ctx, N), ray_kernel_lds(ctx), stream, sc, ctx->work.shadow, nullptr, d.ctrl + kCtlVolumeShift, ctx->d_counters.get(), ctx->lds_nodes);
+      wf.shadow_rays(grid_persistent(ctx, N), ray_kernel_lds(ctx), stream, sc, ctx->work.shadow, nullptr, d.ctrl + kCtlVolumeShift, ctx->d_counters.get(), ctx->lds_nodes, single_level_allowed(ctx));
     }
     Launch l(ctx, stream, LUMC_KERNEL_VOLUME);
     wf.volume_resolve(grid_for(N), stream, sc, d.cur, ctx->work.volume, ctx->work.shadow, ctx->work.results, (const uint32_t*) d.ctrl);
@@ -323,7 +324,7 @@
   if (fused && d.depth > 0) {
     {
       Launch l(ctx, stream, LUMC_KERNEL_SHADOW);
-      wf.shadow_rays(ctx->trace_blocks, ray_kernel_lds(ctx), stream, sc, ctx->fused.fallback, nullptr, d.ctrl + kCtlVolumeShift, ctx->d_counters.get(), ctx->lds_nodes);
+      wf.shadow_rays(ctx->trace_blocks, ray_kernel_lds(ctx), stream, sc, ctx->fused.fallback, nullptr, d.ctrl + kCtlVolumeShift, ctx->d_counters.get(), ctx->lds_nodes, single_level_allowed(ctx));
     }
     Launch l(ctx, stream, LUMC_KERNEL_RESOLVE);
     wf.resolve_listed(std::min<uint32_t>(grid_for(N), 1024u), stream, sc, d.prev, d.nee_before, ctx->fused.fallback, ctx->work.results, (const uint32_t*) d.ctrl);
@@ -360,7 +361,7 @@
   }
   {
     Launch l(ctx, stream, LUMC_KERNEL_SHADOW);
-    wf.shadow_rays(grid_persistent(ctx, N), ray_kernel_lds(ctx), stream, sc, ctx->work.shadow, shadow_order, d.ctrl, ctx->d_counters.get(), ctx->lds_nodes);
+    wf.shadow_rays(grid_persistent(ctx, N), ray_kernel_lds(ctx), stream, sc, ctx->work.shadow, shadow_order, d.ctrl, ctx->d_counters.get(), ctx->lds_nodes, single_level_allowed(ctx));
   }
   if (d.last || scheme == kResolvePlain) {
     Launch l(ctx, stream, LUMC_KERNEL_RESOLVE);
@@ -1064,7 +1065,7 @@
   HIP_TRY(ctx, hipMemsetAsync(cursor, 0, sizeof(uint32_t), stream));
   Launch l(ctx, stream, LUMC_KERNEL_TRACE);
   ctx->wf->trace_rays(grid_persistent(ctx, n), ray_kernel_lds(ctx), stream, ctx->scene, n, d_origins, d_dirs, d_ignore, d_out, cursor, ctx->d_counters.get(),
-                      ctx->lds_nodes);
+                      ctx->lds_nodes, single_level_allowed(ctx));
   HIP_TRY(ctx, hipGetLastError());
   return 0;
 }
@@ -1104,7 +1105,7 @@
   hipLaunchKernelGGL(k_visibility_pack, dim3(blocks), dim3(256), 0, stream, n, d_origins, d_dirs, d_dist, d_ids, sq);
   {
     Launch l(ctx, stream, LUMC_KERNEL_SHADOW);
-    ctx->wf->shadow_rays(grid_persistent(ctx, n), ray_kernel_lds(ctx), stream, ctx->scene, sq, d_order, ctrl, ctx->d_counters.get(), ctx->lds_nodes);
+    ctx->wf->shadow_rays(grid_persistent(ctx, n), ray_kernel_lds(ctx), stream, ctx->scene, sq, d_order, ctrl, ctx->d_counters.get(), ctx->lds_nodes, single_level_allowed(ctx));
   }
   hipLaunchKernelGGL(k_visibility_unpack, dim3(blocks), dim3(256), 0, stream, n, sq.vis, d_out);
   HIP_TRY(ctx, hipGetLastError());
@@ -1262,6 +1263,13 @@
   return 0;
 }
 int lumc_get_ambient_reuse(const LumContext* ctx) { return (ctx && ambient_reuse_active(ctx)) ? 1 : 0; }
+
+int lumc_set_single_level(LumContext* ctx, int mode) {
+  if (!ctx || mode < -1 || mode > 1) { if (ctx) ctx->error = "lumc_set_single_level: -1 (auto), 0 (never) or 1 (when the scene is eligible)"; return 1; }
+  ctx->single_level = mode;
+  return 0;
+}
+int lumc_get_single_level(const LumContext* ctx) { return (ctx && ctx->has_scene && single_level_allowed(ctx) && single_level_scene(ctx->scene)) ? 1 : 0; }
 int lumc_get_flavour(const LumContext* ctx) { return (ctx && ctx->wf == wavefront_kernels_exact()) ? LUMC_FLAVOUR_EXACT : LUMC_FLAVOUR_FAST; }
 
 unsigned int lumc_lds_stack_bytes(void) { return LUM_LDS_STACK_BYTES; }
diff --git a/luminary_amd/csrc/host/scene_device.hip b/luminary_amd/csrc/host/scene_device.hip
--- a/luminary_amd/csrc/host/scene_device.hip
+++ b/luminary_amd/csrc/host/scene_device.hip
@@ -443,6 +443,15 @@
   if (upload(ctx, ctx->arrays.inst.tlas_leaves, tree.tlas_leaves.data(), tree.tlas_leaves.size(), &sc.tlas_leaves)) return 1;
   sc.tlas_num_nodes = tree.tlas_num_nodes;
   sc.tlas_num_leaves = (uint32_t) (tree.tlas_leaves.size() / 4);
+  {
+    bool identity = tree.tlas_leaves.size() >= 4;
+    for (int k = 0; k < 3 && identity; k++) {
+      const float4 r = tree.tlas_leaves[k];
+      const float row[4] = {r.x, r.y, r.z, r.w};
+      for (int c = 0; c < 4; c++) identity = identity && row[c] == (c == k ? 1.0f : 0.0f);
+    }
+    ctx->first_leaf_identity = identity;
+  }
   std::memcpy(ctx->sort.world_lo, tree.world.lo, sizeof(ctx->sort.world_lo)); std::memcpy(ctx->sort.world_hi, tree.world.hi, sizeof(ctx->sort.world_hi));
   ctx->bvh_stats[0] = tree.nodes.size() - tree.tlas_num_nodes;
   ctx->bvh_stats[2] = tree.tlas_num_nodes;
@@ -547,6 +556,7 @@
   u.tlas_nodes = num_nodes;
   sc.tlas_num_nodes = num_nodes;
   sc.tlas_num_leaves = hittable + 1u;
+  ctx->first_leaf_identity = false;
   std::memcpy(ctx->sort.world_lo, world.lo, sizeof(ctx->sort.world_lo)); std::memcpy(ctx->sort.world_hi, world.hi, sizeof(ctx->sort.world_hi));
   ctx->bvh_stats[0] = u.mesh_nodes;
   ctx->bvh_stats[2] = num_nodes;
```

Measured after the change: 4061 (median of 6 runs). 6.1% higher.
